# cwitkowitz/amt-tools

Measured on AMD Instinct MI355X. Metric: audio frames/sec (OnsetsFrames+Mel-229 inference), higher is better.
Workload: dtype bf16

## Files before the change

amt_tools_amd/csrc/amtx_kernels.h:

```cpp
#pragma once
#include "amtx_common.h"

enum { AMTX_T_BF16 = 0, AMTX_T_F32 = 1, AMTX_T_SPLIT = 2 };

static inline size_t amtx_tsize(int t) { return t == AMTX_T_BF16 ? 2 : 4; }

struct GemmArgs {
    const void* A; int64_t lda; int a_type;
    const bf16_t* W; int n_pad, k_pad, planes;
    const float* bias;
    void* C; int64_t ldc; int c_type;
    int64_t M; int N, K;
    int groups; int64_t a_gs, w_gs, bias_gs, c_gs;
    const int2* pair_map = nullptr; float* pair_out = nullptr; int64_t pair_gs = 0, pair_pitch = 0;
    int pair_rows[16] = {0, 0, 0, 0, 0, 0, 0, 0, 0, 0, 0, 0, 0, 0, 0, 0};
    float* pair_max = nullptr; int pair_nh = 0;
    float* roll_out = nullptr; int roll_T = 0; float roll_thr = 0.5f; int roll_group = 0;
    bf16_t* copy16 = nullptr; int64_t copy16_ld = 0; int copy16_col0 = 0, copy16_gs = 0, copy16_pad = 0;
    int64_t a_plane = 0;
    int64_t a_valid_lo = 0, a_valid_hi = 0;
    int64_t a_split = 0, c_split = 0;
};
constexpr int AMTX_GEMM_MULTI_MAX = 10;
struct GemmMulti { GemmArgs p[AMTX_GEMM_MULTI_MAX]; int n; };

struct ConvArgs {
    const void* in; int in_type;
    const bf16_t* wfrag; int planes;
    const float* shift;
    void* out; int out_type;
    int B, T, F, c_out;
    int groups; int64_t in_gs, w_gs, shift_gs, out_gs;
    const float* feats = nullptr; int64_t f_stride_b = 0, f_stride_c = 0, f_stride_t = 0, f_stride_f = 0;
    int c_in = 0;
    const bf16_t* w1frag = nullptr; const float* shift1 = nullptr;
    int64_t w1_gs = 0;
    const float* f_clip_max = nullptr; const float* f_ref = nullptr;
    const void* feats16 = nullptr;
    int64_t out_ts = 0;
    int64_t in_split = 0, out_split = 0;
};
int amtx_launch_convx3(const ConvArgs& c, hipStream_t stream);
int amtx_launch_convx12(const ConvArgs& c, hipStream_t stream);

static inline __host__ __device__ bool amtx_conv1g_tapk(int c_in, int planes) { return (planes == 1 || planes == 2) && c_in >= 2 && c_in <= 8; }

struct Conv1Args {
    const float* in; int64_t stride_b, stride_c, stride_t, stride_f;
    const float* w;
    const float* shift;
    void* out; int out_type;
    int B, T, F, c_in, c_out;
    int groups; int64_t w_gs, shift_gs, out_gs;
    int relu = 1;
};

struct LstmArgs {
    const void* xproj; int x_type;
    const bf16_t* whh; int planes;
    void* out; int out_type;
    int B, T;
    int groups; int64_t x_gs, w_gs, out_gs;
    int hidden = 128;
    float* save = nullptr;
};

namespace amtx_bf16 {
#include "amtx_kernels_fmt.h"
}
#ifdef AMTX_WITH_F16
namespace amtx_f16 {
#include "amtx_kernels_fmt.h"
}
#endif
using namespace AMTX_FMT_NS;

size_t amtx_bce_loss_partials(int B, int T, int keys);
int amtx_launch_bce_loss(const float* logits, int64_t ld, const float* labels, const float* weight, int B, int T, int keys, float* loss,
                         float* grad, float* partial, hipStream_t stream);
int amtx_launch_loss_reduce(const float* partial, int64_t n, float inv_bt, float* loss, hipStream_t stream);
int amtx_launch_pianoroll(const float* logits, int64_t ld, int col0, int B, int T, int keys, float threshold, float* out,
                          hipStream_t stream);

int amtx_launch_cvt_pad_bf16(const float* src, int64_t ld_src, int n_src, bf16_t* dst, int ld_dst, int64_t rows, hipStream_t stream,
                             bool f16 = false );
int amtx_launch_cvt_split(const float* src, int64_t ld_src, int n_src, bf16_t* dst, int ld_dst, int64_t split, int64_t rows, hipStream_t stream);
int amtx_launch_zero_cols(void* base, int64_t pitch_bytes, int width_bytes, int64_t rows, hipStream_t stream);

constexpr int DEC_HALF = 150;
constexpr int DEC_TAPS = 2 * DEC_HALF + 1;
constexpr int DEC_KW = 352;
constexpr int DEC_NKS = DEC_KW / 32;
int amtx_launch_cqt_decimate(const float* in, int64_t n_in, int64_t in_stride, int in_pad, float* out, int64_t n_out, int64_t out_stride, int pad,
                             const void* tfrag, int zero_pads, float* maxbuf, int n_harm, int batch, hipStream_t stream);
```

amt_tools_amd/csrc/amtx_kernels_fmt.h:

```cpp

bool amtx_gemm_has_roll_epilogue(const GemmArgs& g);
int amtx_launch_gemm(const GemmArgs& g, hipStream_t stream);
int amtx_launch_gemm_multi(const GemmArgs* gs, int n, hipStream_t stream);
void amtx_gemm_pack_dims(int N, int K, int* n_pad, int* k_pad);
void amtx_gemm_pack_host(const float* W, int64_t ldw, int N, int K, int planes, bf16_t* out);

int amtx_launch_conv3x3(const ConvArgs& c, hipStream_t stream);
size_t amtx_conv1_wfrag_elems(int c_in, int planes);
void amtx_conv1_pack_host(const float* w, const float* scale, int c_in, int planes, bf16_t* out);
size_t amtx_conv3x3_wfrag_elems(int c_out, int planes);
void amtx_conv3x3_pack_host(const float* w, const float* scale, int c_out, int planes, bf16_t* out);
int amtx_launch_conv1(const Conv1Args& c, hipStream_t stream);

bool amtx_conv_stack_fused_ok(int B, int T, int F, int groups);
int amtx_launch_conv_stack(const ConvArgs& c2, const bf16_t* w3frag, int64_t w3_gs, const float* shift3, void* out, int64_t out_gs,
                           int64_t out_plane, hipStream_t stream);

int amtx_conv3x3_gen_ntc(int c_in, int c_out);
size_t amtx_conv3x3_gen_wfrag_elems(int c_in, int c_out, int planes);
void amtx_conv3x3_gen_pack_host(const float* w , const float* scale, int c_in, int c_out, int planes, bf16_t* out);
int amtx_launch_conv3x3_gen(const ConvArgs& c, int c_in, hipStream_t stream);
size_t amtx_conv1g_wfrag_elems(int c_in, int c_mid, int planes);
void amtx_conv1g_pack_host(const float* w , const float* scale, int c_in, int c_mid, int planes, bf16_t* out);
bool amtx_conv3x3_gen_can_fuse1(int c_in, int c_mid, int c_out, int planes);

int amtx_launch_bilstm(const LstmArgs& l, hipStream_t stream);
size_t amtx_bilstm_wfrag_elems(int hidden, int planes);
void amtx_bilstm_pack_host(const float* whh_fwd, const float* whh_bwd, int hidden, int planes, bf16_t* out);
int amtx_launch_bilstm_pack_dev(const float* whh_fwd, const float* whh_bwd, int hidden, int planes, bf16_t* frag_fwd, bf16_t* frag_bwd, hipStream_t stream);
int amtx_launch_bilstm_bwd(const float* dout, const float* save, const bf16_t* whh_t, int hidden, int planes, float* dxproj, int B, int T, int groups,
                           hipStream_t stream);

int amtx_pack_bn_fold_dev(const float* conv_bias, const float* gamma, const float* beta, const float* mean, const float* var, int c_out, float* scale,
                          float* shift, hipStream_t s);
int amtx_pack_conv3x3_dev(const float* w, const float* scale, int c_out, int planes, bf16_t* out, hipStream_t s);
int amtx_pack_conv1_dev(const float* w, const float* scale, int planes, bf16_t* out, hipStream_t s);
int amtx_pack_conv_gen_dev(const float* w, const float* scale, int c_in, int c_out, int ntc, int planes, bf16_t* out, hipStream_t s);
int amtx_pack_conv1g_dev(const float* w, const float* scale, int c_in, int c_mid, int planes, bf16_t* out, hipStream_t s);
int amtx_pack_scale_rows_dev(const float* w, const float* scale, int rows, int cols, float* out, hipStream_t s);
int amtx_pack_linear_dev(const float* W, int64_t ldw, int N, int K, int planes, int n_pad, int k_pad, int row0, int rows_owned, int perm_c, int perm_f,
                         bf16_t* out, hipStream_t s);
void amtx_pack_linear_host(const float* W, int64_t ldw, int N, int K, int planes, int n_pad, int k_pad, int row0, int rows_owned, int perm_c, int perm_f,
                           bf16_t* out);
int amtx_pack_head_fold_dev(const float* w_out, const float* w_fc1, const float* b_fc1, const float* b_out, int n_out, int dim_am, int kfc, int kfc_pad,
                            int nf3, int fq, float* wfold, float* bfold, hipStream_t s);
int amtx_pack_vec_add_dev(const float* a, const float* b, int n, float* out, hipStream_t s);
```

amt_tools_amd/csrc/lstm.hip:

```cpp

#include "amtx_kernels.h"
#include "amtx_pack_layouts.h"

#include <type_traits>

namespace {

constexpr int H = 128;
constexpr int UB = 1;
constexpr int LWAVES = H / (16 * UB);
constexpr int LTHREADS = 64 * LWAVES;
constexpr int HP = H + 8;
constexpr int HBUF_BYTES = 16 * HP * 2;

template <bool FAST>
__device__ __forceinline__ float sigmoid_f(float x) {
    if (FAST) return __builtin_amdgcn_rcpf(1.0f + __builtin_amdgcn_exp2f(-1.4426950408889634f * x));
    return 1.0f / (1.0f + expf(-x));
}
template <bool FAST>
__device__ __forceinline__ float tanh_f(float x) {
    if (FAST) return fmaf(2.0f, __builtin_amdgcn_rcpf(1.0f + __builtin_amdgcn_exp2f(-2.8853900817779268f * x)), -1.0f);
    return tanhf(x);
}


struct Gates { float i, f, g, o; };
template <bool FAST>
__device__ __forceinline__ Gates lstm_gates(float ai, float af, float ag, float ao) {
    return {sigmoid_f<FAST>(ai), sigmoid_f<FAST>(af), tanh_f<FAST>(ag), sigmoid_f<FAST>(ao)};
}
template <bool FAST>
__device__ __forceinline__ float lstm_cell(const Gates& z, float& c) {
    c = z.f * c + z.i * z.g;
    return z.o * tanh_f<FAST>(c);
}

template <int NS>
__device__ __forceinline__ void split16(const float (&v)[4], uint2& hi, uint2& lo) {
    lo = make_uint2(0, 0);
    if (NS == 2) {
        split_bf16x2(v[0], v[1], hi.x, lo.x);
        split_bf16x2(v[2], v[3], hi.y, lo.y);
    } else {
        hi = make_uint2(pack_bf16x2(v[0], v[1]), pack_bf16x2(v[2], v[3]));
    }
}
template <int NS>
__device__ __forceinline__ void store16(char* tile, int plane_bytes, int off, uint2 hi, uint2 lo) {
    *reinterpret_cast<uint2*>(tile + off) = hi;
    if (NS == 2) *reinterpret_cast<uint2*>(tile + plane_bytes + off) = lo;
}

__device__ __forceinline__ int step_frame(int s, const int& T, const int& reverse) {
    s = s < T ? s : T - 1;
    return reverse == 0 ? s : T - 1 - s;
}

template <int SGK, int NS>
struct FragStream {
    typedef const __attribute__((address_space(1))) char* gchar_p;
    typedef __attribute__((ext_vector_type(4))) unsigned int u32x4_t;
    typedef __attribute__((address_space(1))) u32x4_t gu4_t;
    const char* base;
    gchar_p wb;
    unsigned wlane;
    __device__ __forceinline__ FragStream(const char* base_, int lane) : base(base_), wb((gchar_p)base_), wlane(lane * 16) {}
    __device__ __forceinline__ void rewind() {
        wb = (gchar_p)base;
        asm volatile("" : "+s"(wb));
    }
    __device__ __forceinline__ uint4 load(int gi, int k, int p) const {
        return __builtin_bit_cast(uint4, *reinterpret_cast<const gu4_t*>(wb + ((gi * SGK + k) * NS + p) * 1024 + wlane));
    }
    __device__ __forceinline__ void load_group(int gi, uint4 (&dst)[SGK][NS]) const {
        static_for<0, SGK>([&](auto kc) {
            static_for<0, NS>([&](auto pc) { dst[decltype(kc)::value][decltype(pc)::value] = load(gi, decltype(kc)::value, decltype(pc)::value); });
        });
    }
};

template <int X_TYPE> struct XRaw { typedef float4 type; };
template <> struct XRaw<AMTX_T_BF16> { typedef uint2 type; };

template <int X_TYPE>
__device__ __forceinline__ void load_x(const char* xbase, int64_t row_off, typename XRaw<X_TYPE>::type (&dst)[UB][4]) {
#pragma unroll
    for (int ub = 0; ub < UB; ++ub)
#pragma unroll
        for (int q = 0; q < 4; ++q) {
            const int64_t e = row_off + q * 128 + 16 * ub;
            dst[ub][q] = *reinterpret_cast<const typename XRaw<X_TYPE>::type*>(xbase + e * (X_TYPE == AMTX_T_F32 ? 4 : 2));
        }
}
__device__ __forceinline__ f32x4_t unpack_x(float4 v) { return (f32x4_t){v.x, v.y, v.z, v.w}; }
__device__ __forceinline__ f32x4_t unpack_x(uint2 v) {
    return (f32x4_t){unpack16_lo(v.x), unpack16_hi(v.x), unpack16_lo(v.y), unpack16_hi(v.y)};
}

__device__ __forceinline__ void lds_barrier() {
    asm volatile("s_waitcnt lgkmcnt(0)\n\ts_barrier" ::: "memory");
    __builtin_amdgcn_sched_barrier(0);
}

template <int NS, int X_TYPE, int OUT_TYPE, bool FAST>
__device__ __forceinline__ void lstm_step(char* smem, int cur, const uint4 (&wf)[UB][4][4][NS], const typename XRaw<X_TYPE>::type (&xcur)[UB][4],
                                          typename XRaw<X_TYPE>::type (&xnext)[UB][4], float (&c)[UB][4], const char* xbase, char* obase, int t, int tnext,
                                          int clip, int g, int wave, bool clip_ok) {
    const char* hb = smem + cur * NS * HBUF_BYTES;
    uint4 hf[4][NS];
#pragma unroll
    for (int ks = 0; ks < 4; ++ks)
#pragma unroll
        for (int p = 0; p < NS; ++p)
            hf[ks][p] = *reinterpret_cast<const uint4*>(hb + p * HBUF_BYTES + (clip * HP + 32 * ks + 8 * g) * 2);

    load_x<X_TYPE>(xbase, (int64_t)tnext * 1024, xnext);

    f32x4_t acc[UB][4];
#pragma unroll
    for (int ub = 0; ub < UB; ++ub)
#pragma unroll
        for (int q = 0; q < 4; ++q) acc[ub][q] = unpack_x(xcur[ub][q]);
#pragma unroll
    for (int ks = 0; ks < 4; ++ks)
#pragma unroll
        for (int ub = 0; ub < UB; ++ub)
#pragma unroll
            for (int q = 0; q < 4; ++q) {
                acc[ub][q] = mfma16(wf[ub][q][ks][0], hf[ks][0], acc[ub][q]);
                if (NS == 2) {
                    acc[ub][q] = mfma16(wf[ub][q][ks][0], hf[ks][1], acc[ub][q]);
                    acc[ub][q] = mfma16(wf[ub][q][ks][1], hf[ks][0], acc[ub][q]);
                }
            }

    char* hn = smem + (cur ^ 1) * NS * HBUF_BYTES;
#pragma unroll
    for (int ub = 0; ub < UB; ++ub) {
        float h[4];
#pragma unroll
        for (int r = 0; r < 4; ++r) {
            h[r] = lstm_cell<FAST>(lstm_gates<FAST>(acc[ub][0][r], acc[ub][1][r], acc[ub][2][r], acc[ub][3][r]), c[ub][r]);
        }
        uint2 hiw, low;
        split16<NS>(h, hiw, low);
        store16<NS>(hn, HBUF_BYTES, (clip * HP + 16 * UB * wave + 16 * ub + 4 * g) * 2, hiw, low);
        if (clip_ok) {
            const int64_t e = (int64_t)t * 256 + 16 * ub;
            if (OUT_TYPE == AMTX_T_BF16) *reinterpret_cast<uint2*>(obase + e * 2) = hiw;
            else *reinterpret_cast<float4*>(obase + e * 4) = make_float4(h[0], h[1], h[2], h[3]);
        }
    }
    lds_barrier();
}

template <int NS, int X_TYPE, int OUT_TYPE>
__global__ __launch_bounds__(LTHREADS) void bilstm_kernel(LstmArgs a) {
    extern __shared__ __attribute__((aligned(16))) char smem[];
    constexpr bool FAST = true;
    const int tid = threadIdx.x, lane = tid & 63, wave = tid >> 6;
    const int clip = lane & 15, g = lane >> 4;
    const int b0 = blockIdx.x * 16, dir = blockIdx.y, grp = blockIdx.z;
    const int b = b0 + clip;
    const bool clip_ok = b < a.B;
    const int T = a.T;

    uint4 wf[UB][4][4][NS];
    {
        const uint4* w = reinterpret_cast<const uint4*>(a.whh + (int64_t)grp * a.w_gs) + lane;
#pragma unroll
        for (int ub = 0; ub < UB; ++ub)
#pragma unroll
            for (int q = 0; q < 4; ++q)
#pragma unroll
                for (int ks = 0; ks < 4; ++ks)
#pragma unroll
                    for (int p = 0; p < NS; ++p)
                        wf[ub][q][ks][p] = w[((((((dir * LWAVES + wave) * UB + ub) * 4 + q) * 4 + ks) * NS) + p) * 64];
    }

    for (int i = tid; i < 2 * NS * HBUF_BYTES / 16; i += LTHREADS) reinterpret_cast<uint4*>(smem)[i] = make_uint4(0, 0, 0, 0);

    float c[UB][4];
#pragma unroll
    for (int ub = 0; ub < UB; ++ub)
#pragma unroll
        for (int r = 0; r < 4; ++r) c[ub][r] = 0.f;

    const char* xbase = reinterpret_cast<const char*>(a.xproj) +
                        ((int64_t)grp * a.x_gs + (int64_t)(clip_ok ? b : 0) * T * 1024 + dir * 512 + 16 * UB * wave + 4 * g) * (X_TYPE == AMTX_T_BF16 ? 2 : 4);
    char* obase = reinterpret_cast<char*>(a.out) +
                  ((int64_t)grp * a.out_gs + (int64_t)(clip_ok ? b : 0) * T * 256 + dir * 128 + 16 * UB * wave + 4 * g) * (OUT_TYPE == AMTX_T_BF16 ? 2 : 4);

    typename XRaw<X_TYPE>::type x0[UB][4], x1[UB][4], x2[UB][4], x3[UB][4];
    auto tidx = [&](int s) { return (int64_t)step_frame(s, T, dir); };
    load_x<X_TYPE>(xbase, tidx(0) * 1024, x0);
    load_x<X_TYPE>(xbase, tidx(1) * 1024, x1);
    load_x<X_TYPE>(xbase, tidx(2) * 1024, x2);
    __syncthreads();

    for (int s = 0; s < T; s += 4) {
        lstm_step<NS, X_TYPE, OUT_TYPE, FAST>(smem, 0, wf, x0, x3, c, xbase, obase, (int)tidx(s), (int)tidx(s + 3), clip, g, wave, clip_ok);
        lstm_step<NS, X_TYPE, OUT_TYPE, FAST>(smem, 1, wf, x1, x0, c, xbase, obase, (int)tidx(s + 1), (int)tidx(s + 4), clip, g, wave, clip_ok && s + 1 < T);
        lstm_step<NS, X_TYPE, OUT_TYPE, FAST>(smem, 0, wf, x2, x1, c, xbase, obase, (int)tidx(s + 2), (int)tidx(s + 5), clip, g, wave, clip_ok && s + 2 < T);
        lstm_step<NS, X_TYPE, OUT_TYPE, FAST>(smem, 1, wf, x3, x2, c, xbase, obase, (int)tidx(s + 3), (int)tidx(s + 6), clip, g, wave, clip_ok && s + 3 < T);
    }
}

template <int X_TYPE> struct XScalar { typedef float type; };
template <> struct XScalar<AMTX_T_BF16> { typedef unsigned int type; };
__device__ __forceinline__ float unpack_xs(float v, bool) { return v; }
__device__ __forceinline__ float unpack_xs(unsigned int v, bool odd) { return odd ? unpack16_hi(v) : unpack16_lo(v); }

template <int X_TYPE>
__device__ __forceinline__ void load_x4(const char* xbase, int64_t row_off, typename XScalar<X_TYPE>::type (&dst)[4]) {
#pragma unroll
    for (int q = 0; q < 4; ++q)
    {
        if (X_TYPE == AMTX_T_F32) dst[q] = *reinterpret_cast<const typename XScalar<X_TYPE>::type*>(xbase + (row_off + q * 128) * 4);
        else dst[q] = *reinterpret_cast<const unsigned int*>(xbase + (row_off + q * 128) * 2);
    }
}

template <int NS, int X_TYPE, int OUT_TYPE, bool FAST, int NC>
__device__ __forceinline__ void lstm4_step(char* smem, int cur, const uint4 (&wf)[4][4][NS], const typename XScalar<X_TYPE>::type (&xcur)[NC][4],
                                           typename XScalar<X_TYPE>::type (&xnext)[NC][4], float (&c)[NC], const char* const (&xbase)[NC],
                                           char* const (&obase)[NC], int t, int tnext, int lane, const int (&hwoff)[NC], const bool (&clip_ok)[NC],
                                           float* save) {
    constexpr int RSTEP = 4 / NC;
    const char* hb = smem + cur * NS * HBUF_BYTES;
    uint4 hf[4][NS];
#pragma unroll
    for (int ks = 0; ks < 4; ++ks)
#pragma unroll
        for (int p = 0; p < NS; ++p)
            hf[ks][p] = *reinterpret_cast<const uint4*>(hb + p * HBUF_BYTES + ((lane & 15) * HP + 32 * ks + 8 * (lane >> 4)) * 2);

#pragma unroll
    for (int j = 0; j < NC; ++j) load_x4<X_TYPE>(xbase[j], (int64_t)tnext * 1024, xnext[j]);

    f32x4_t acc[4];
#pragma unroll
    for (int q = 0; q < 4; ++q) {
        acc[q] = (f32x4_t){0.f, 0.f, 0.f, 0.f};
#pragma unroll
        for (int j = 0; j < NC; ++j) acc[q][RSTEP * j] = unpack_xs(xcur[j][q], lane & 1);
    }
#pragma unroll
    for (int ks = 0; ks < 4; ++ks) {
#pragma unroll
        for (int q = 0; q < 4; ++q) acc[q] = mfma16(hf[ks][0], wf[q][ks][0], acc[q]);
        if (NS == 2) {
#pragma unroll
            for (int q = 0; q < 4; ++q) acc[q] = mfma16(hf[ks][NS - 1], wf[q][ks][0], acc[q]);
#pragma unroll
            for (int q = 0; q < 4; ++q) acc[q] = mfma16(hf[ks][0], wf[q][ks][NS - 1], acc[q]);
        }
    }

    char* hn = smem + (cur ^ 1) * NS * HBUF_BYTES;
    Gates z[NC];
    float h[NC];
    uint32_t hiw[NC], low[NC];
#pragma unroll
    for (int j = 0; j < NC; ++j) z[j] = lstm_gates<FAST>(acc[0][RSTEP * j], acc[1][RSTEP * j], acc[2][RSTEP * j], acc[3][RSTEP * j]);
#pragma unroll
    for (int j = 0; j < NC; ++j) {
        h[j] = lstm_cell<FAST>(z[j], c[j]);
        low[j] = 0;
        if (NS == 2) split_bf16x2(h[j], 0.f, hiw[j], low[j]);
        else hiw[j] = pack_bf16x2(h[j], 0.f);
    }
#pragma unroll
    for (int j = 0; j < NC; ++j) {
        *reinterpret_cast<unsigned short*>(hn + hwoff[j]) = (unsigned short)hiw[j];
        if (NS == 2) *reinterpret_cast<unsigned short*>(hn + HBUF_BYTES + hwoff[j]) = (unsigned short)low[j];
    }
#pragma unroll
    for (int j = 0; j < NC; ++j) {
        if (NC == 1 && save && clip_ok[j]) {
            float* sv = save + (int64_t)t * (2 * 5 * H);
            sv[0] = z[j].i; sv[H] = z[j].f; sv[2 * H] = z[j].g; sv[3 * H] = z[j].o; sv[4 * H] = c[j];
        }
        if (clip_ok[j]) {
            if (OUT_TYPE == AMTX_T_BF16) *reinterpret_cast<unsigned short*>(obase[j] + (int64_t)t * 256 * 2) = (unsigned short)hiw[j];
            else *reinterpret_cast<float*>(obase[j] + (int64_t)t * 256 * 4) = h[j];
        }
    }
    lds_barrier();
}

template <int NS, int X_TYPE, int OUT_TYPE, int NC = 1>
__global__ __launch_bounds__(LTHREADS) void bilstm4_kernel(LstmArgs a) {
    extern __shared__ __attribute__((aligned(16))) char smem[];
    constexpr bool FAST = true;
    const int tid = threadIdx.x, lane = tid & 63, wave = tid >> 6;
    const int unit = 16 * wave + (lane & 15), cg = lane >> 4;
    const int dir = blockIdx.y, grp = blockIdx.z;
    const int T = a.T;

    uint4 wf[4][4][NS];
    {
        const uint4* w = reinterpret_cast<const uint4*>(a.whh + (int64_t)grp * a.w_gs) + lane;
#pragma unroll
        for (int q = 0; q < 4; ++q)
#pragma unroll
            for (int ks = 0; ks < 4; ++ks)
#pragma unroll
                for (int p = 0; p < NS; ++p) wf[q][ks][p] = w[(((((dir * LWAVES + wave) * 4 + q) * 4 + ks) * NS) + p) * 64];
    }
    for (int i = tid; i < 2 * NS * HBUF_BYTES / 16; i += LTHREADS) reinterpret_cast<uint4*>(smem)[i] = make_uint4(0, 0, 0, 0);

    float c[NC];
    bool clip_ok[NC];
    const char* xbase[NC];
    char* obase[NC];
    int hwoff[NC];
    float* save = nullptr;
#pragma unroll
    for (int j = 0; j < NC; ++j) {
        const int b = (blockIdx.x * 4 + cg) * NC + j;
        clip_ok[j] = b < a.B;
        c[j] = 0.f;
        xbase[j] = reinterpret_cast<const char*>(a.xproj) +
                   ((int64_t)grp * a.x_gs + (int64_t)(clip_ok[j] ? b : 0) * T * 1024 + dir * 512 + (X_TYPE == AMTX_T_BF16 ? (unit & ~1) : unit)) *
                       (X_TYPE == AMTX_T_BF16 ? 2 : 4);
        obase[j] = reinterpret_cast<char*>(a.out) +
                   ((int64_t)grp * a.out_gs + (int64_t)(clip_ok[j] ? b : 0) * T * 256 + dir * 128 + unit) * (OUT_TYPE == AMTX_T_BF16 ? 2 : 4);
        hwoff[j] = ((4 * cg + (4 / NC) * j) * HP + unit) * 2;
        if (NC == 1) save = a.save ? a.save + (((int64_t)grp * a.B + (clip_ok[j] ? b : 0)) * T * 2 + dir) * (5 * H) + unit : nullptr;
    }

    typename XScalar<X_TYPE>::type x0[NC][4], x1[NC][4], x2[NC][4], x3[NC][4];
    auto tidx = [&](int s) { return (int64_t)step_frame(s, T, dir); };
#pragma unroll
    for (int j = 0; j < NC; ++j) {
        load_x4<X_TYPE>(xbase[j], tidx(0) * 1024, x0[j]);
        load_x4<X_TYPE>(xbase[j], tidx(1) * 1024, x1[j]);
        load_x4<X_TYPE>(xbase[j], tidx(2) * 1024, x2[j]);
    }
    __syncthreads();

    for (int s = 0; s < T; s += 4) {
        bool ok1[NC], ok2[NC], ok3[NC];
#pragma unroll
        for (int j = 0; j < NC; ++j) { ok1[j] = clip_ok[j] && s + 1 < T; ok2[j] = clip_ok[j] && s + 2 < T; ok3[j] = clip_ok[j] && s + 3 < T; }
        lstm4_step<NS, X_TYPE, OUT_TYPE, FAST, NC>(smem, 0, wf, x0, x3, c, xbase, obase, (int)tidx(s), (int)tidx(s + 3), lane, hwoff, clip_ok, save);
        lstm4_step<NS, X_TYPE, OUT_TYPE, FAST, NC>(smem, 1, wf, x1, x0, c, xbase, obase, (int)tidx(s + 1), (int)tidx(s + 4), lane, hwoff, ok1, save);
        lstm4_step<NS, X_TYPE, OUT_TYPE, FAST, NC>(smem, 0, wf, x2, x1, c, xbase, obase, (int)tidx(s + 2), (int)tidx(s + 5), lane, hwoff, ok2, save);
        lstm4_step<NS, X_TYPE, OUT_TYPE, FAST, NC>(smem, 1, wf, x3, x2, c, xbase, obase, (int)tidx(s + 3), (int)tidx(s + 6), lane, hwoff, ok3, save);
    }
}

constexpr int GP = 4 * H + 8;
constexpr int GBUF_BYTES = 16 * GP * 2;

struct LstmBwdArgs {
    const float* dout;
    const float* save;
    const bf16_t* whh_t;
    int planes;
    float* dxproj;
    int B, T;
};

#ifdef AMTX_LSTM_TIMING
__device__ unsigned long long g_lstm_prof[4];
#define LT_TICK(SLOT) do { const unsigned long long n_ = __builtin_readcyclecounter(); lt_acc[SLOT] += n_ - lt_t; lt_t = n_; } while (0)
#else
#define LT_TICK(SLOT) do {} while (0)
#endif
template <int NS>
__global__ __launch_bounds__(LTHREADS) void bilstm4_bwd_kernel(LstmBwdArgs a) {
    extern __shared__ __attribute__((aligned(16))) char smem[];
    const int tid = threadIdx.x, lane = tid & 63, wave = tid >> 6;
    const int unit = 16 * wave + (lane & 15), cg = lane >> 4;
    const int dir = blockIdx.y;
    const int b = blockIdx.x * 4 + cg;
    const bool clip_ok = b < a.B;
    const int T = a.T;

    uint4 wt[16][NS];
    {
        const uint4* w = reinterpret_cast<const uint4*>(a.whh_t) + lane;
#pragma unroll
        for (int ks = 0; ks < 16; ++ks)
#pragma unroll
            for (int p = 0; p < NS; ++p) wt[ks][p] = w[((((dir * LWAVES + wave) * 16 + ks) * NS) + p) * 64];
    }
    for (int i = tid; i < 2 * NS * GBUF_BYTES / 16; i += LTHREADS) reinterpret_cast<uint4*>(smem)[i] = make_uint4(0, 0, 0, 0);
    __syncthreads();

    const int64_t bb = clip_ok ? b : 0;
    const float* sv0 = a.save + ((bb * T) * 2 + dir) * (5 * H) + unit;
    const float* do0 = a.dout + (bb * T) * 256 + dir * H + unit;
    float* dx0 = a.dxproj + (bb * T) * 1024 + dir * 512 + unit;
    const int gwoff = (4 * cg * GP + unit) * 2;

    float dh_rec = 0.f, dc_rec = 0.f;
    auto frame = [&](int s) { return step_frame(s, T, dir == 0); };
    float n_i, n_f, n_g, n_o, n_c, n_do;
    {
        const float* sv = sv0 + (int64_t)frame(0) * (2 * 5 * H);
        n_i = sv[0]; n_f = sv[H]; n_g = sv[2 * H]; n_o = sv[3 * H]; n_c = sv[4 * H];
        n_do = do0[(int64_t)frame(0) * 256];
    }
#ifdef AMTX_LSTM_TIMING
    unsigned long long lt_acc[4] = {0, 0, 0, 0}, lt_t = __builtin_readcyclecounter();
#endif
    for (int s = 0; s < T; ++s) {
        const int t = frame(s);
        const float ig = n_i, fg = n_f, gg = n_g, og = n_o, ct = n_c, dout_t = n_do;
        {
            const int tn = frame(s + 1);
            const float* sv = sv0 + (int64_t)tn * (2 * 5 * H);
            n_i = sv[0]; n_f = sv[H]; n_g = sv[2 * H]; n_o = sv[3 * H]; n_c = sv[4 * H];
            n_do = do0[(int64_t)tn * 256];
        }
        asm volatile("" : "+v"(n_c));
        const float cp = s + 1 < T ? n_c : 0.f;
        const float dh = dout_t + dh_rec;
        const float tc = tanh_f<true>(ct);
        const float d_o = dh * tc * og * (1.f - og);
        const float dc = dc_rec + dh * og * (1.f - tc * tc);
        const float d_i = dc * gg * ig * (1.f - ig);
        const float d_g = dc * ig * (1.f - gg * gg);
        const float d_f = dc * cp * fg * (1.f - fg);
        dc_rec = dc * fg;
        const float dgv[4] = {d_i, d_f, d_g, d_o};
        char* gt = smem + (s & 1) * NS * GBUF_BYTES;
#pragma unroll
        for (int q = 0; q < 4; ++q) {
            if (clip_ok) dx0[(int64_t)t * 1024 + q * H] = dgv[q];
            uint32_t hiw, low = 0;
            if (NS == 2) split_bf16x2(dgv[q], 0.f, hiw, low);
            else hiw = pack_bf16x2(dgv[q], 0.f);
            *reinterpret_cast<unsigned short*>(gt + gwoff + q * H * 2) = (unsigned short)hiw;
            if (NS == 2) *reinterpret_cast<unsigned short*>(gt + GBUF_BYTES + gwoff + q * H * 2) = (unsigned short)low;
        }
        LT_TICK(0);
        lds_barrier();
        LT_TICK(1);
        f32x4_t acc4[4];
#pragma unroll
        for (int i = 0; i < 4; ++i) acc4[i] = (f32x4_t){0.f, 0.f, 0.f, 0.f};
#pragma unroll
        for (int k4 = 0; k4 < 16; k4 += 4) {
            uint4 gf[4][NS];
#pragma unroll
            for (int i = 0; i < 4; ++i)
#pragma unroll
                for (int p = 0; p < NS; ++p)
                    gf[i][p] = *reinterpret_cast<const uint4*>(gt + p * GBUF_BYTES + ((lane & 15) * GP + 32 * (k4 + i) + 8 * (lane >> 4)) * 2);
#pragma unroll
            for (int i = 0; i < 4; ++i) acc4[i] = mfma16(gf[i][0], wt[k4 + i][0], acc4[i]);
            if (NS == 2) {
#pragma unroll
                for (int i = 0; i < 4; ++i) acc4[i] = mfma16(gf[i][NS - 1], wt[k4 + i][0], acc4[i]);
#pragma unroll
                for (int i = 0; i < 4; ++i) acc4[i] = mfma16(gf[i][0], wt[k4 + i][NS - 1], acc4[i]);
            }
        }
        dh_rec = (acc4[0][0] + acc4[1][0]) + (acc4[2][0] + acc4[3][0]);
#ifdef AMTX_LSTM_TIMING
        asm volatile("" ::"v"(dh_rec));
        LT_TICK(2);
        lt_acc[3] += 1;
#endif
    }
#ifdef AMTX_LSTM_TIMING
    if (tid == 0 && blockIdx.x == 0 && blockIdx.y == 0)
        for (int i = 0; i < 4; ++i) atomicAdd(&g_lstm_prof[i], lt_acc[i]);
#endif
}
#if defined(AMTX_LSTM_TIMING) && !defined(AMTX_F16)
extern "C" int amtxdbg_lstm_prof(unsigned long long* out4, int reset) {
    if (hipMemcpyFromSymbol(out4, HIP_SYMBOL(g_lstm_prof), 4 * sizeof(unsigned long long)) != hipSuccess) return -1;
    if (reset) {
        unsigned long long z[4] = {0, 0, 0, 0};
        if (hipMemcpyToSymbol(HIP_SYMBOL(g_lstm_prof), z, sizeof(z)) != hipSuccess) return -1;
    }
    return 0;
}
#endif

template <int HC>
__global__ void bilstm_pack_dev_kernel(const float* __restrict__ whh_fwd, const float* __restrict__ whh_bwd, int hidden, AmtxFragPut fwd, AmtxFragPut bwd) {
    if (HC) hidden = HC;
    for (int item = blockIdx.x * blockDim.x + threadIdx.x, n = amtx_layout_bilstm_items(hidden); item < n; item += gridDim.x * blockDim.x) {
        amtx_layout_bilstm(item, whh_fwd, whh_bwd, hidden, fwd);
        amtx_layout_bilstm_transposed(item, whh_fwd, whh_bwd, hidden, bwd);
    }
}

template <int HH, int NS, int X_TYPE, int OUT_TYPE>
__global__ __launch_bounds__(512) void bilstm_stream_kernel(LstmArgs a) {
    constexpr int NU = HH / 16, UPW = NU / 8, KSN = HH / 32;
    constexpr int SGK = NS == 2 ? 2 : 4;
    constexpr int NSUB = KSN / SGK;
    constexpr int NG = UPW * 4 * NSUB;
    constexpr int HPG = HH + 8;
    constexpr int HBG = 16 * HPG * 2;
    constexpr bool FAST = true;
    constexpr int RS = 4;
    constexpr bool PIN = NS == 1 && HH == 256;
    constexpr bool PINL = NS == 1 && HH == 384;
    constexpr int PER = NG / 4;
    constexpr int NPIN = PIN ? NG / 4 : (PINL ? 4 : 0);
    constexpr int NSG = NG - (PIN ? 2 : (PINL ? 1 : 0)) * NPIN;
    static_assert(NU % 8 == 0 && KSN % SGK == 0 && NG % 4 == 0 && NSG % RS == 0, "hidden size must be a multiple of 128");
    extern __shared__ __attribute__((aligned(16))) char smem[];
    const int tid = threadIdx.x, lane = tid & 63, wave = tid >> 6;
    const int clip = lane & 15, g = lane >> 4;
    const int b0 = blockIdx.x * 16, dir = blockIdx.y, grp = blockIdx.z;
    const int b = b0 + clip;
    const bool clip_ok = b < a.B;
    const int T = a.T;
    constexpr int XES = X_TYPE == AMTX_T_BF16 ? 2 : 4, OES = OUT_TYPE == AMTX_T_BF16 ? 2 : 4;

    for (int i = tid; i < 2 * NS * HBG / 16; i += 512) reinterpret_cast<uint4*>(smem)[i] = make_uint4(0, 0, 0, 0);

    const int wave_u = __builtin_amdgcn_readfirstlane(wave);
    const char* wbase = reinterpret_cast<const char*>(a.whh + (int64_t)grp * a.w_gs) + ((int64_t)(dir * NU + wave_u * UPW) * 4 * KSN * NS) * 1024;
    FragStream<SGK, NS> ws(wbase, lane);
    const char* xbase = reinterpret_cast<const char*>(a.xproj) +
                        ((int64_t)grp * a.x_gs + (int64_t)(clip_ok ? b : 0) * T * 8 * HH + dir * 4 * HH + 16 * UPW * wave + 4 * g) * XES;
    char* obase = reinterpret_cast<char*>(a.out) +
                  ((int64_t)grp * a.out_gs + (int64_t)(clip_ok ? b : 0) * T * 2 * HH + dir * HH + 16 * UPW * wave + 4 * g) * OES;

    float c[UPW][4];
#pragma unroll
    for (int ub = 0; ub < UPW; ++ub)
#pragma unroll
        for (int r = 0; r < 4; ++r) c[ub][r] = 0.f;

    typedef typename XRaw<X_TYPE>::type xraw_t;
    auto tidx = [&](int s) { return (int64_t)step_frame(s, T, dir); };
    auto load_xrow = [&](int64_t t, xraw_t (&dst)[UPW][4]) {
#pragma unroll
        for (int ub = 0; ub < UPW; ++ub)
#pragma unroll
            for (int q = 0; q < 4; ++q)
                dst[ub][q] = *reinterpret_cast<const xraw_t*>(xbase + (t * 8 * HH + q * HH + 16 * ub) * XES);
    };
    uint4 w[RS][SGK][NS];
    uint4 wpin[PIN ? NPIN : 1][SGK][NS];
    char* wlds = smem + 2 * NS * HBG + wave * (NPIN * SGK * NS * 1024);
    if constexpr (PIN || PINL) {
        static_for<0, NG>([&](auto ic) {
            constexpr int gi = decltype(ic)::value;
            constexpr int kind = PIN ? ((gi & 3) == 0 ? 0 : ((gi & 3) == 1 ? 1 : 2)) : (gi % PER == 0 ? 1 : 2);
            constexpr int pidx = PIN ? gi >> 2 : gi / PER;
            if constexpr (kind < 2) {
                static_for<0, SGK>([&](auto kc) {
                    constexpr int k = decltype(kc)::value;
                    static_for<0, NS>([&](auto pc) {
                        constexpr int p = decltype(pc)::value;
                        const uint4 v = ws.load(gi, k, p);
                        if constexpr (kind == 0) wpin[pidx][k][p] = v;
                        else *reinterpret_cast<uint4*>(wlds + ((pidx * SGK + k) * NS + p) * 1024 + ws.wlane) = v;
                    });
                });
            }
        });
    }

    xraw_t xn[UPW][4];
    load_xrow(tidx(0), xn);
    static_for<0, RS - 1>([&](auto sc) {
        constexpr int si = decltype(sc)::value;
        constexpr int gi = PIN ? (si >> 1) * 4 + 2 + (si & 1) : (PINL ? si + si / (PER - 1) + 1 : si);
        ws.load_group(gi, w[si % RS]);
    });
    __syncthreads();

    int cur = 0;
    for (int s = 0; s < T; ++s) {
        ws.rewind();
        const char* hb = smem + cur * NS * HBG;
        constexpr bool HF_REG = KSN * NS <= 16;
        uint4 hf[HF_REG ? KSN : 1][NS];
        if constexpr (HF_REG) {
#pragma unroll
            for (int ks = 0; ks < KSN; ++ks)
#pragma unroll
                for (int p = 0; p < NS; ++p) hf[ks][p] = *reinterpret_cast<const uint4*>(hb + p * HBG + (clip * HPG + 32 * ks + 8 * g) * 2);
        }

        f32x4_t acc[UPW][4];
#pragma unroll
        for (int ub = 0; ub < UPW; ++ub)
#pragma unroll
            for (int q = 0; q < 4; ++q) acc[ub][q] = unpack_x(xn[ub][q]);
        load_xrow(tidx(s + 1), xn);
        __builtin_amdgcn_sched_barrier(0);

        static_for<0, NG>([&](auto ic) {
            constexpr int gi = decltype(ic)::value;
            constexpr int ub = gi / (4 * NSUB), q = (gi / NSUB) & 3, sub = gi % NSUB;
            constexpr int kind = PIN ? ((gi & 3) == 0 ? 0 : ((gi & 3) == 1 ? 1 : 2)) : (PINL ? (gi % PER == 0 ? 1 : 2) : 2);
            constexpr int pidx = PIN ? gi >> 2 : gi / PER;
            constexpr int si = PIN ? (gi >> 2) * 2 + (gi & 3) - 2 : (PINL ? gi - gi / PER - 1 : gi);
            if constexpr (kind == 2) {
                constexpr int sn = (si + RS - 1) % NSG;
                constexpr int gn = PIN ? (sn >> 1) * 4 + 2 + (sn & 1) : (PINL ? sn + sn / (PER - 1) + 1 : sn);
                ws.load_group(gn, w[sn % RS]);
            }
            f32x4_t d = acc[ub][q];
            static_for<0, SGK>([&](auto kc) {
                constexpr int k = decltype(kc)::value;
                constexpr int ks = sub * SGK + k;
                uint4 w0, w1;
                if constexpr (kind == 0) {
                    w0 = wpin[pidx][k][0]; w1 = wpin[pidx][k][NS - 1];
                } else if constexpr (kind == 1) {
                    w0 = *reinterpret_cast<const uint4*>(wlds + ((pidx * SGK + k) * NS + 0) * 1024 + ws.wlane);
                    w1 = w0;
                } else {
                    w0 = w[si % RS][k][0]; w1 = w[si % RS][k][NS - 1];
                }
                uint4 h0, h1;
                if constexpr (HF_REG) {
                    h0 = hf[ks][0]; h1 = hf[ks][NS - 1];
                } else {
                    h0 = *reinterpret_cast<const uint4*>(hb + (clip * HPG + 32 * ks + 8 * g) * 2);
                    h1 = *reinterpret_cast<const uint4*>(hb + (NS - 1) * HBG + (clip * HPG + 32 * ks + 8 * g) * 2);
                }
                d = mfma16(w0, h0, d);
                if constexpr (NS == 2) {
                    d = mfma16(w0, h1, d);
                    d = mfma16(w1, h0, d);
                }
            });
            acc[ub][q] = d;
            __builtin_amdgcn_sched_barrier(0);
        });

        char* hn = smem + (cur ^ 1) * NS * HBG;
        const int64_t t = tidx(s);
#pragma unroll
        for (int ub = 0; ub < UPW; ++ub) {
            float h[4], sv[4][4];
#pragma unroll
            for (int r = 0; r < 4; ++r) {
                const Gates z = lstm_gates<FAST>(acc[ub][0][r], acc[ub][1][r], acc[ub][2][r], acc[ub][3][r]);
                h[r] = lstm_cell<FAST>(z, c[ub][r]);
                sv[0][r] = z.i; sv[1][r] = z.f; sv[2][r] = z.g; sv[3][r] = z.o;
            }
            if (a.save && clip_ok) {
                float* sp = a.save + ((((int64_t)grp * a.B + b) * T + t) * 2 + dir) * (5 * HH) + 16 * UPW * wave + 16 * ub + 4 * g;
#pragma unroll
                for (int q = 0; q < 4; ++q) *reinterpret_cast<float4*>(sp + q * HH) = make_float4(sv[q][0], sv[q][1], sv[q][2], sv[q][3]);
                *reinterpret_cast<float4*>(sp + 4 * HH) = make_float4(c[ub][0], c[ub][1], c[ub][2], c[ub][3]);
            }
            uint2 hiw, low;
            split16<NS>(h, hiw, low);
            store16<NS>(hn, HBG, (clip * HPG + 16 * UPW * wave + 16 * ub + 4 * g) * 2, hiw, low);
            if (clip_ok) {
                const int64_t e = t * 2 * HH + 16 * ub;
                if (OUT_TYPE == AMTX_T_BF16) *reinterpret_cast<uint2*>(obase + e * 2) = hiw;
                else *reinterpret_cast<float4*>(obase + e * 4) = make_float4(h[0], h[1], h[2], h[3]);
            }
        }
        cur ^= 1;
        lds_barrier();
    }
}

struct LstmBwdHArgs {
    const float* dout; const float* save; const bf16_t* whh_t; float* dxproj; int B, T;
    int64_t w_gs;
};

template <int HH, int NS>
__global__ __launch_bounds__(512) void bilstm_stream_bwd_kernel(LstmBwdHArgs a) {
    constexpr int UT = HH / 128;
    constexpr int KSN = 4 * HH / 32;
    constexpr int SGK = NS == 2 ? 2 : 4;
    constexpr int NG = UT * KSN / SGK;
    constexpr int RS = 4;
    constexpr bool PINB = HH == 256;
    constexpr int NPINB = PINB ? NG / 4 : 0, NSGB = NG - NPINB;
    constexpr int GPH = 4 * HH + 8;
    constexpr int GBH = 5 * GPH * 2;
    static_assert(NG % 4 == 0 && NSGB % RS == 0, "hidden size must be a multiple of 128");
    extern __shared__ __attribute__((aligned(16))) char smem[];
    const int tid = threadIdx.x, lane = tid & 63, wave = tid >> 6;
    const int cg = lane >> 4;
    const int dir = blockIdx.y;
    const int b = blockIdx.x * 4 + cg;
    const bool clip_ok = b < a.B;
    const int T = a.T;
    const int unit0 = 16 * UT * wave + (lane & 15);

    for (int i = tid; i < 2 * NS * GBH / 16; i += 512) reinterpret_cast<uint4*>(smem)[i] = make_uint4(0, 0, 0, 0);

    const int wave_u = __builtin_amdgcn_readfirstlane(wave);
    const int grp = blockIdx.z;
    const char* wbase = reinterpret_cast<const char*>(a.whh_t + (int64_t)grp * a.w_gs) + ((int64_t)(dir * 8 + wave_u) * UT * KSN * NS) * 1024;
    FragStream<SGK, NS> ws(wbase, lane);
    uint4 w[RS][SGK][NS];

    const int64_t bb = (int64_t)grp * a.B + (clip_ok ? b : 0);
    const float* sv0 = a.save + ((bb * T) * 2 + dir) * (5 * HH) + unit0;
    const float* do0 = a.dout + (bb * T) * (2 * HH) + dir * HH + unit0;
    float* dx0 = a.dxproj + (bb * T) * (8 * HH) + dir * 4 * HH + unit0;
    const int gwoff = (cg * GPH + unit0) * 2;
    const int groff = ((((lane & 15) & 3) == 0 ? (lane & 15) >> 2 : 4) * GPH + 8 * (lane >> 4)) * 2;

    float dh_rec[UT], dc_rec[UT];
#pragma unroll
    for (int ut = 0; ut < UT; ++ut) { dh_rec[ut] = 0.f; dc_rec[ut] = 0.f; }
    auto frame = [&](int s) { return step_frame(s, T, dir == 0); };
    float nv[UT][6];
    auto load_next = [&](int tn) {
#pragma unroll
        for (int ut = 0; ut < UT; ++ut) {
            const float* sv = sv0 + (int64_t)tn * (2 * 5 * HH) + 16 * ut;
#pragma unroll
            for (int q = 0; q < 5; ++q) nv[ut][q] = sv[q * HH];
            nv[ut][5] = do0[(int64_t)tn * (2 * HH) + 16 * ut];
        }
    };
    load_next(frame(0));
    uint4 wpin[PINB ? NPINB : 1][SGK][NS];
    static_for<0, NPINB>([&](auto gc) { ws.load_group(4 * decltype(gc)::value, wpin[decltype(gc)::value]); });
    static_for<0, RS - 1>([&](auto sc) {
        constexpr int si = decltype(sc)::value;
        constexpr int gi = PINB ? (si / 3) * 4 + 1 + si % 3 : si;
        ws.load_group(gi, w[si % RS]);
    });
    __syncthreads();

    for (int s = 0; s < T; ++s) {
        ws.rewind();
        const int t = frame(s);
        float cur[UT][6];
#pragma unroll
        for (int ut = 0; ut < UT; ++ut)
#pragma unroll
            for (int q = 0; q < 6; ++q) cur[ut][q] = nv[ut][q];
        load_next(frame(s + 1));
        char* gt = smem + (s & 1) * NS * GBH;
#pragma unroll
        for (int ut = 0; ut < UT; ++ut) {
            asm volatile("" : "+v"(nv[ut][4]));
            const float cp = s + 1 < T ? nv[ut][4] : 0.f;
            const float ig = cur[ut][0], fg = cur[ut][1], gg = cur[ut][2], og = cur[ut][3], ct = cur[ut][4];
            const float dh = cur[ut][5] + dh_rec[ut];
            const float tc = tanh_f<true>(ct);
            const float d_o = dh * tc * og * (1.f - og);
            const float dc = dc_rec[ut] + dh * og * (1.f - tc * tc);
            const float d_i = dc * gg * ig * (1.f - ig);
            const float d_g = dc * ig * (1.f - gg * gg);
            const float d_f = dc * cp * fg * (1.f - fg);
            dc_rec[ut] = dc * fg;
            const float dgv[4] = {d_i, d_f, d_g, d_o};
#pragma unroll
            for (int q = 0; q < 4; ++q) {
                if (clip_ok) dx0[(int64_t)t * (8 * HH) + q * HH + 16 * ut] = dgv[q];
                uint32_t hiw, low = 0;
                if (NS == 2) split_bf16x2(dgv[q], 0.f, hiw, low);
                else hiw = pack_bf16x2(dgv[q], 0.f);
                *reinterpret_cast<unsigned short*>(gt + gwoff + (q * HH + 16 * ut) * 2) = (unsigned short)hiw;
                if (NS == 2) *reinterpret_cast<unsigned short*>(gt + GBH + gwoff + (q * HH + 16 * ut) * 2) = (unsigned short)low;
            }
        }
        lds_barrier();
        f32x4_t acc[UT];
#pragma unroll
        for (int ut = 0; ut < UT; ++ut) acc[ut] = (f32x4_t){0.f, 0.f, 0.f, 0.f};
        static_for<0, NG>([&](auto ic) {
            constexpr int gi = decltype(ic)::value;
            constexpr int ut = gi / (KSN / SGK), sub = gi % (KSN / SGK);
            constexpr bool pinned = PINB && (gi & 3) == 0;
            constexpr int si = PINB ? (gi >> 2) * 3 + (gi & 3) - 1 : gi;
            if constexpr (!pinned) {
                constexpr int sn = (si + RS - 1) % NSGB;
                constexpr int gn = PINB ? (sn / 3) * 4 + 1 + sn % 3 : sn;
                ws.load_group(gn, w[sn % RS]);
            }
            static_for<0, SGK>([&](auto kc) {
                constexpr int k = decltype(kc)::value;
                constexpr int ks = sub * SGK + k;
                uint4 gf[NS];
#pragma unroll
                for (int p = 0; p < NS; ++p)
                    gf[p] = *reinterpret_cast<const uint4*>(gt + p * GBH + groff + 32 * ks * 2);
                uint4 w0, w1;
                if constexpr (pinned) { w0 = wpin[gi >> 2][k][0]; w1 = wpin[gi >> 2][k][NS - 1]; }
                else { w0 = w[si % RS][k][0]; w1 = w[si % RS][k][NS - 1]; }
                acc[ut] = mfma16(gf[0], w0, acc[ut]);
                if constexpr (NS == 2) {
                    acc[ut] = mfma16(gf[NS - 1], w0, acc[ut]);
                    acc[ut] = mfma16(gf[0], w1, acc[ut]);
                }
            });
            __builtin_amdgcn_sched_barrier(0);
        });
#pragma unroll
        for (int ut = 0; ut < UT; ++ut) dh_rec[ut] = acc[ut][0];
    }
}


struct LstmSwitches { bool no8; };
const LstmSwitches& lstm_switches() {
    static const LstmSwitches sw = {getenv("AMTX_LSTM_NO8") != nullptr};
    return sw;
}

enum LstmFamily { LSTM_CLIPS4, LSTM_CLIPS8, LSTM_CLIPS16, LSTM_STREAM, LSTM_ERROR };
enum LstmInst { LSTM_BF16, LSTM_BF16_F32IO, LSTM_X3, LSTM_NO_INST };
struct LstmRouted { LstmFamily family; LstmInst inst; dim3 grid; size_t lds; int code; const char* error; };

LstmRouted lstm_route(const LstmArgs& a, const LstmSwitches& sw) {
    const bool io16 = a.x_type == AMTX_T_BF16 && a.out_type == AMTX_T_BF16, io32 = a.x_type == AMTX_T_F32 && a.out_type == AMTX_T_F32;
    const LstmInst inst = a.planes == 1 && io16 ? LSTM_BF16 : (a.planes == 1 && io32 ? LSTM_BF16_F32IO : (a.planes == 2 && io32 ? LSTM_X3 : LSTM_NO_INST));
    auto error = [](int code, const char* msg) { return LstmRouted{LSTM_ERROR, LSTM_NO_INST, dim3(), 0, code, msg}; };
    auto on = [&](LstmFamily family, int clips, size_t lds) {
        return LstmRouted{family, inst, dim3((unsigned)((a.B + clips - 1) / clips), 2, (unsigned)a.groups), lds, AMTX_OK, nullptr};
    };
    if (a.hidden != H) {
        if (a.save && a.planes != 2) return error(AMTX_ERR_ARG, "bilstm: the training forward (save) is built for the two-plane precision");
        if (a.hidden != 256 && a.hidden != 384 && a.hidden != 512) return error(AMTX_ERR_UNSUPPORTED, "bilstm: unsupported hidden size (128, 256, 384 and 512 are built)");
        if (inst != LSTM_BF16 && inst != LSTM_X3) return error(AMTX_ERR_UNSUPPORTED, "bilstm: unsupported precision/type combination");
        return on(LSTM_STREAM, 16, 2 * (size_t)a.planes * 16 * (a.hidden + 8) * 2 + (a.planes == 1 && a.hidden <= 384 ? (size_t)8 * 4 * 4096 : 0));
    }
    if (inst == LSTM_NO_INST) return error(AMTX_ERR_UNSUPPORTED, "bilstm: unsupported precision/type combination");
    const size_t lds = 2 * (size_t)a.planes * HBUF_BYTES;
    const int64_t blocks4 = (int64_t)((a.B + 3) / 4) * 2 * a.groups;
    if (a.save) return on(LSTM_CLIPS4, 4, lds);
    if (blocks4 > 1024) return on(LSTM_CLIPS16, 16, lds);
    if (!sw.no8 && a.planes == 1 && blocks4 > 256) return on(LSTM_CLIPS8, 8, lds);
    return on(LSTM_CLIPS4, 4, lds);
}

template <typename F>
int with_hidden(int hidden, F&& f) {
    switch (hidden) {
        case 256: return f(std::integral_constant<int, 256>{});
        case 384: return f(std::integral_constant<int, 384>{});
        case 512: return f(std::integral_constant<int, 512>{});
    }
    amtx_set_error("bilstm: unsupported hidden size %d (128, 256, 384 and 512 are built)", hidden);
    return AMTX_ERR_UNSUPPORTED;
}

template <typename K, typename A>
int launch_kernel(K kern, dim3 grid, size_t lds, hipStream_t stream, const A& a) {
    AMTX_GRANT_LDS(kern, lds);
    hipLaunchKernelGGL(kern, grid, dim3(LTHREADS), lds, stream, a);
    AMTX_CHECK_LAUNCH();
    return AMTX_OK;
}

template <int NS, int XT>
int launch_routed(const LstmRouted& r, const LstmArgs& a, hipStream_t stream) {
    switch (r.family) {
        case LSTM_CLIPS4: return launch_kernel(bilstm4_kernel<NS, XT, XT>, r.grid, r.lds, stream, a);
        case LSTM_CLIPS8: return launch_kernel(bilstm4_kernel<NS, XT, XT, 2>, r.grid, r.lds, stream, a);
        case LSTM_CLIPS16: return launch_kernel(bilstm_kernel<NS, XT, XT>, r.grid, r.lds, stream, a);
        case LSTM_STREAM:
            if constexpr (NS == 2 || XT == AMTX_T_BF16)
                return with_hidden(a.hidden, [&](auto hh) { return launch_kernel(bilstm_stream_kernel<decltype(hh)::value, NS, XT, XT>, r.grid, r.lds, stream, a); });
            break;
        case LSTM_ERROR: break;
    }
    amtx_set_error("bilstm: route without a kernel");
    return AMTX_ERR_UNSUPPORTED;
}

}

namespace AMTX_FMT_NS {

size_t amtx_bilstm_wfrag_elems(int hidden, int planes) { return (size_t)2 * 4 * hidden * hidden * planes; }

static_assert(16 * UB * LWAVES == H && LWAVES == AMTX_LSTM_BWD_WAVES, "W_hh fragment layouts");

void amtx_bilstm_pack_host(const float* whh_fwd, const float* whh_bwd, int hidden, int planes, bf16_t* out) {
    const AmtxFragPut put{out, planes};
    for (int item = 0, n = amtx_layout_bilstm_items(hidden); item < n; ++item) amtx_layout_bilstm(item, whh_fwd, whh_bwd, hidden, put);
}

int amtx_launch_bilstm(const LstmArgs& a, hipStream_t stream) {
    AMTX_REQUIRE(a.xproj && a.whh && a.out, "bilstm: null pointer");
    AMTX_REQUIRE(a.B > 0 && a.T > 0 && a.groups > 0, "bilstm: bad sizes");
    AMTX_REQUIRE(a.planes == 1 || a.planes == 2, "bilstm: planes must be 1 or 2");
    const LstmRouted r = lstm_route(a, lstm_switches());
    switch (r.inst) {
        case LSTM_BF16: return launch_routed<1, AMTX_T_BF16>(r, a, stream);
        case LSTM_BF16_F32IO: return launch_routed<1, AMTX_T_F32>(r, a, stream);
        case LSTM_X3: return launch_routed<2, AMTX_T_F32>(r, a, stream);
        case LSTM_NO_INST: break;
    }
    amtx_set_error("%s (hidden %d)", r.error, a.hidden);
    return r.code;
}

int amtx_launch_bilstm_pack_dev(const float* whh_fwd, const float* whh_bwd, int hidden, int planes, bf16_t* frag_fwd, bf16_t* frag_bwd, hipStream_t stream) {
    AMTX_REQUIRE(whh_fwd && whh_bwd && frag_fwd && frag_bwd && (planes == 1 || planes == 2), "bilstm pack: bad argument");
    AMTX_REQUIRE(hidden == H || hidden == 256 || hidden == 384 || hidden == 512, "bilstm pack: hidden size %d is not built (128, 256, 384, 512)", hidden);
    const AmtxFragPut fwd{frag_fwd, planes}, bwd{frag_bwd, planes};
    if (hidden == H) hipLaunchKernelGGL(bilstm_pack_dev_kernel<H>, dim3(64), dim3(256), 0, stream, whh_fwd, whh_bwd, H, fwd, bwd);
    else hipLaunchKernelGGL(bilstm_pack_dev_kernel<0>, dim3(256), dim3(256), 0, stream, whh_fwd, whh_bwd, hidden, fwd, bwd);
    AMTX_CHECK_LAUNCH();
    return AMTX_OK;
}

int amtx_launch_bilstm_bwd(const float* dout, const float* save, const bf16_t* whh_t, int hidden, int planes, float* dxproj, int B, int T, int groups,
                           hipStream_t stream) {
    AMTX_REQUIRE(groups >= 1, "bilstm backward: bad group count");
    AMTX_REQUIRE(dout && save && whh_t && dxproj, "bilstm backward: null pointer");
    AMTX_REQUIRE(B > 0 && T > 0 && (planes == 1 || planes == 2), "bilstm backward: bad sizes");
    const int64_t w_gs = (int64_t)amtx_bilstm_wfrag_elems(hidden, planes), bt = (int64_t)B * T;
    const dim3 grid((unsigned)((B + 3) / 4), 2);
    if (hidden == H) {
        for (int g = 0; g < groups; ++g) {
            const LstmBwdArgs a{dout + g * bt * 2 * H, save + g * bt * 2 * 5 * H, whh_t + g * w_gs, planes, dxproj + g * bt * 8 * H, B, T};
            const size_t lds = 2 * (size_t)planes * GBUF_BYTES;
            const int rc = planes == 2 ? launch_kernel(bilstm4_bwd_kernel<2>, grid, lds, stream, a) : launch_kernel(bilstm4_bwd_kernel<1>, grid, lds, stream, a);
            if (rc != AMTX_OK) return rc;
        }
        return AMTX_OK;
    }
    AMTX_REQUIRE(planes == 2 && (hidden == 256 || hidden == 384 || hidden == 512),
                 "bilstm backward: hidden 256 / 384 / 512 are built for the two-plane precision only (got hidden %d, planes %d)", hidden, planes);
    const LstmBwdHArgs a{dout, save, whh_t, dxproj, B, T, w_gs};
    return with_hidden(hidden, [&](auto hh) {
        return launch_kernel(bilstm_stream_bwd_kernel<decltype(hh)::value, 2>, dim3(grid.x, 2, (unsigned)groups), 2 * (size_t)planes * 5 * (4 * hidden + 8) * 2, stream, a);
    });
}

}
```

amt_tools_amd/csrc/ofmodel.hip:

```cpp

#include "amtx_kernels.h"
#include "amtx_model_common.h"
#include "amtx_pack_layouts.h"

#include <cmath>
#include <cstdlib>
#include <thread>

namespace {

struct LinearPack { DevBuf w, b; int N = 0, K = 0, n_pad = 0, k_pad = 0, groups = 0; };

#define AMTX_FMT_KERNELS(X, ns)                                                                                                    \
    X(ns, pack_linear_host) X(ns, bilstm_pack_host) X(ns, conv1_pack_host) X(ns, conv1g_pack_host) X(ns, conv3x3_pack_host)     \
    X(ns, conv3x3_gen_pack_host) X(ns, pack_conv1_dev) X(ns, pack_conv1g_dev) X(ns, pack_conv3x3_dev) X(ns, pack_conv_gen_dev)    \
    X(ns, pack_linear_dev) X(ns, launch_bilstm_pack_dev) X(ns, launch_conv1) X(ns, launch_conv3x3) X(ns, launch_conv3x3_gen)    \
    X(ns, launch_conv_stack) X(ns, launch_gemm) X(ns, launch_bilstm)
#define AMTX_KERNEL_FIELD(ns, name) decltype(&ns::amtx_##name) name;
#define AMTX_KERNEL_ENTRY(ns, name) &ns::amtx_##name,
struct KernelSet { AMTX_FMT_KERNELS(AMTX_KERNEL_FIELD, amtx_bf16) };
const KernelSet kKernelsBf16 = {AMTX_FMT_KERNELS(AMTX_KERNEL_ENTRY, amtx_bf16)};
#ifdef AMTX_WITH_F16
const KernelSet kKernelsF16 = {AMTX_FMT_KERNELS(AMTX_KERNEL_ENTRY, amtx_f16)};
#endif

enum ConvFamily { K_CONV1,
                  K_CONV,
                  K_CONVG };
struct ConvLayer { const char* name; int c_in, c_out; ConvFamily fam; size_t frag_per; };

struct ConvSwitches { bool no_convg_mc2, no_conv_fuse, x3_no_split, no_convx12m, rowmajor_a3, no_roll_epilogue; };
ConvSwitches switches_from_env() {
    auto on = [](const char* name) { return getenv(name) != nullptr; };
    return {on("AMTX_NO_CONVG_MC2"), on("AMTX_NO_CONV_FUSE"), on("AMTX_X3_NO_SPLIT"), on("AMTX_NO_CONVX12M"), on("AMTX_OF_ROWMAJOR_A3"), on("AMTX_OF_NO_ROLL_EPILOGUE")};
}

struct ConvPlan {
    ConvLayer layer[3];
    bool conv1_fused;
    bool stack;
    bool two_plane_acts;
    bool convx12; size_t c2x_per;
    bool rowmajor_a3, no_roll_epilogue;
    bool device_resync;
    int fuses_db_scale, takes_feats16;
};

ConvPlan make_conv_plan(int in_channels, int model_complexity, int precision, const ConvSwitches& sw) {
    const int ic = in_channels, nf1 = 16 * model_complexity, nf3 = 2 * nf1, pl = precision == AMTX_PREC_X3 ? 2 : 1;
    ConvPlan p{};
    const ConvFamily f3 = nf1 != 32 ? K_CONVG : K_CONV;
    const bool g_fuse1 = amtx_conv3x3_gen_can_fuse1(ic, nf1, nf1, pl);
    const ConvFamily f2 = f3 == K_CONVG || (ic > 1 && !sw.no_convg_mc2 && g_fuse1) ? K_CONVG : K_CONV;
    p.conv1_fused = f2 == K_CONVG ? g_fuse1 : 9 * ic <= 64;
    auto frag3x3 = [pl](ConvFamily f, int c_in, int c_out) { return f == K_CONVG ? amtx_conv3x3_gen_wfrag_elems(c_in, c_out, pl) : amtx_conv3x3_wfrag_elems(c_out, pl); };
    p.layer[0] = {"layer1", ic, nf1, p.conv1_fused ? f2 : K_CONV1,
                  !p.conv1_fused ? 0 : f2 == K_CONVG ? amtx_conv1g_wfrag_elems(ic, nf1, pl) : amtx_conv1_wfrag_elems(ic, pl)};
    p.layer[1] = {"layer2", nf1, nf1, f2, frag3x3(f2, nf1, nf1)};
    p.layer[2] = {"layer3", nf1, nf3, f3, frag3x3(f3, nf1, nf3)};
    p.stack = f2 == K_CONV && p.conv1_fused && ic == 1 && pl == 1 && !sw.no_conv_fuse;
    p.two_plane_acts = pl == 2 && f3 == K_CONV && p.conv1_fused && !sw.x3_no_split && (f2 == K_CONV ? ic == 1 : ic > 1 && (9 * ic + 31) / 32 <= 2);
    p.convx12 = p.two_plane_acts && f2 == K_CONVG && ic >= 2 && ic <= 8 && amtx_conv1g_tapk(ic, 2) && !sw.no_convx12m;
    p.c2x_per = frag3x3(K_CONV, nf1, nf1);
    p.rowmajor_a3 = sw.rowmajor_a3; p.no_roll_epilogue = sw.no_roll_epilogue;
    p.device_resync = f2 == K_CONVG || ic == 1;
    p.fuses_db_scale = p.conv1_fused && f2 == K_CONV && ic == 1;
    p.takes_feats16 = !(p.conv1_fused && f2 == K_CONVG && precision != AMTX_PREC_F16) ? 0 : p.convx12 ? 2 : pl == 1 && nf1 == 32 && amtx_conv1g_tapk(ic, pl);
    return p;
}

}

struct amtx_of_model {
    int dim_in, in_channels, mc, n_out, has_offsets, precision;
    int planes, act_type;
    bool f16 = false;
    const KernelSet* k = &kKernelsBf16;
    int nf1, nf2, nf3, dim_am, dim_lm, fq, kfc;
    int kfc_pad;
    int hid, xw;
    size_t hh_elems;
    ConvPlan plan;
    int n_heads;
    int n_rec;
    std::vector<std::string> head_names;
    TensorStore store{"of_model", "was not provided"};
    DevBuf pack_scratch;
    bool finalized = false;
    bool packed_once = false;
    DevBuf conv_w[3], conv_s[3];
    DevBuf conv1_w;
    DevBuf conv2_wx;
    LinearPack fc1;
    LinearPack rec_ih;
    DevBuf rec_hh;
    LinearPack rec_out;
    LinearPack pitch_out;
    LinearPack adj_ih;
    DevBuf adj_hh;
    LinearPack adj_out;
    int dim_aj;
    mutable bool prof = false;
    mutable std::vector<std::vector<hipEvent_t>> prof_events;
};

enum { ST_CONV1 = 0, ST_CONV2, ST_CONV3, ST_FC1, ST_REC_XPROJ, ST_REC_LSTM, ST_REC_HEAD, ST_PITCH_HEAD, ST_ADJ_XPROJ, ST_ADJ_LSTM,
       ST_ADJ_HEAD, ST_PIANOROLL, ST_COUNT };
static const char* kStageNames[ST_COUNT] = {"conv1", "conv2_pool", "conv3_pool", "fc1_gemm", "rec_xproj_gemm", "rec_bilstm", "rec_head_gemm",
                                            "pitch_head_gemm", "adj_xproj_gemm", "adj_bilstm", "adj_head_gemm", "pianoroll"};

namespace {

struct Workspace {
    char *a1, *a2, *a3, *e, *xp, *l1, *joint, *joint16, *xp2, *l2, *mp;
    size_t total;
};

enum ConvPath { PATH_STACK,
                PATH_CONVX12,
                PATH_CONV12, PATH_CONVG12,
                PATH_CONV1 };
struct ConvCall { ConvPath path; bool a2_in_hbm; int64_t a3_plane; };

ConvCall resolve_conv(const amtx_of_model* m, int B, int T, bool feats16) {
    const ConvPlan& p = m->plan;
    if (p.stack && amtx_conv_stack_fused_ok(B, T, m->dim_in, m->n_heads))
        return {PATH_STACK, false, p.rowmajor_a3 ? 0 : (int64_t)B * T * 64};
    return {feats16 && p.convx12 ? PATH_CONVX12 : !p.conv1_fused ? PATH_CONV1 : p.layer[1].fam == K_CONVG ? PATH_CONVG12 : PATH_CONV12, true, 0};
}

Workspace carve(const amtx_of_model* m, int B, int T, char* base) {
    Workspace w;
    const size_t es = amtx_tsize(m->act_type);
    const size_t BT = (size_t)B * T;
    const int F = m->dim_in, F2 = F / 2;
    WorkspaceCarver ws{base};
    w.a1 = ws.take(m->plan.conv1_fused ? 256 : BT * F * m->nf1 * es * m->n_heads);
    w.a2 = ws.take(resolve_conv(m, B, T, false).a2_in_hbm ? BT * F2 * m->nf2 * es * m->n_heads : 256);
    w.a3 = ws.take(BT * m->kfc_pad * es * m->n_heads);
    w.e = ws.take(BT * m->dim_am * es * m->n_heads);
    w.xp = ws.take(BT * m->xw * es * m->n_rec);
    w.l1 = ws.take(BT * m->dim_lm * es * m->n_rec);
    w.joint = ws.take(BT * m->dim_aj * sizeof(float));
    w.joint16 = ws.take(BT * (size_t)((m->dim_aj + 63) / 64 * 64) * 2 * (m->plan.two_plane_acts ? 2 : 1));
    w.xp2 = ws.take(BT * m->xw * es);
    w.l2 = ws.take(BT * m->dim_lm * es);
    w.mp = ws.take(BT * m->n_out * sizeof(float));
    w.total = ws.off;
    return w;
}

}

extern "C" int amtx_has_f16(void) {
#ifdef AMTX_WITH_F16
    return 1;
#else
    return 0;
#endif
}

extern "C" int amtx_of_model_create(amtx_of_model** out, int dim_in, int in_channels, int model_complexity, int n_out,
                                    int has_offsets, int precision) {
    AMTX_REQUIRE(out, "amtx_of_model_create: null model pointer");
    *out = nullptr;
    AMTX_REQUIRE(precision == AMTX_PREC_BF16 || precision == AMTX_PREC_X3 || precision == AMTX_PREC_F16, "amtx_of_model_create: bad precision");
    AMTX_REQUIRE(dim_in >= 4 && in_channels >= 1 && n_out > 0 && n_out % 4 == 0, "amtx_of_model_create: bad dims");
    if (precision == AMTX_PREC_F16 && !amtx_has_f16()) {
        amtx_set_error("amtx_of_model_create: precision f16 needs a library built with the half-operand kernel twins (AMTX_BUILD_F16=1 python -m amt_tools_amd.build)");
        return AMTX_ERR_UNSUPPORTED;
    }
    if (model_complexity < 2 || model_complexity > 5) {
        amtx_set_error("amtx_of_model_create: model_complexity 2 (32/32/64-channel convolutions, LSTM hidden 128), 3 (48/48/96, hidden 256) and "
                       "4 (64/64/128, hidden 384), 5 (80/80/160, hidden 512) are implemented, with or without the OnsetsFrames2 offset head (got model_complexity=%d)", model_complexity);
        return AMTX_ERR_UNSUPPORTED;
    }
    amtx_of_model* m = new amtx_of_model();
    m->dim_in = dim_in; m->in_channels = in_channels; m->mc = model_complexity; m->n_out = n_out;
    m->has_offsets = has_offsets; m->precision = precision;
    m->planes = precision == AMTX_PREC_X3 ? 2 : 1;
    m->act_type = precision == AMTX_PREC_X3 ? AMTX_T_F32 : AMTX_T_BF16;
    m->f16 = precision == AMTX_PREC_F16;
#ifdef AMTX_WITH_F16
    if (m->f16) m->k = &kKernelsF16;
#endif
    m->nf1 = 16 * model_complexity; m->nf2 = m->nf1; m->nf3 = 32 * model_complexity;
    m->dim_am = 256 * model_complexity; m->dim_lm = 256 * (model_complexity - 1);
    m->fq = dim_in / 4;
    m->kfc = m->nf3 * m->fq;
    m->kfc_pad = (m->kfc + 63) / 64 * 64;
    m->hid = m->dim_lm / 2; m->xw = 8 * m->hid;
    m->hh_elems = amtx_bilstm_wfrag_elems(m->hid, m->planes);
    m->plan = make_conv_plan(in_channels, model_complexity, precision, switches_from_env());
    m->head_names = {"onset_head"};
    if (has_offsets) m->head_names.push_back("offset_head");
    m->n_rec = (int)m->head_names.size();
    m->head_names.push_back("pitch_head");
    m->n_heads = (int)m->head_names.size();
    m->dim_aj = (m->n_rec + 1) * n_out;
    *out = m;
    return AMTX_OK;
}

extern "C" int amtx_of_model_destroy(amtx_of_model* m) {
    if (!m) return AMTX_OK;
    DevBuf* bufs[] = {&m->conv1_w, &m->conv_w[0], &m->conv_w[1], &m->conv_w[2], &m->conv_s[0], &m->conv_s[1], &m->conv_s[2], &m->conv2_wx, &m->fc1.w, &m->fc1.b,
                      &m->rec_ih.w, &m->rec_ih.b, &m->rec_hh, &m->rec_out.w, &m->rec_out.b, &m->pitch_out.w, &m->pitch_out.b,
                      &m->adj_ih.w, &m->adj_ih.b, &m->adj_hh, &m->adj_out.w, &m->adj_out.b, &m->pack_scratch};
    for (DevBuf* b : bufs) b->release();
    delete m;
    return AMTX_OK;
}

extern "C" int amtx_of_model_set_tensor(amtx_of_model* m, const char* name, const float* host_data, int64_t numel) {
    AMTX_REQUIRE(m && name && host_data && numel > 0, "amtx_of_model_set_tensor: bad argument");
    m->store.set(name, host_data, numel);
    m->finalized = false;
    return AMTX_OK;
}

namespace {

struct HostPack {
    amtx_of_model* m;
    std::map<DevBuf*, std::vector<char>> image;
    std::vector<float> scratch_;

    int need(const std::string& name, size_t numel, const float** p) { return m->store.need(name, numel, p); }
    template <class T> T* dst(DevBuf& b, size_t elems) {
        std::vector<char>& v = image[&b];
        v.resize(elems * sizeof(T));
        return (T*)v.data();
    }
    int scratch(size_t floats, float** p) { scratch_.resize(floats); *p = scratch_.data(); return AMTX_OK; }
    int bn_fold(const float* cb, const float* g, const float* be, const float* mu, const float* var, int c_out, float* scale, float* shift) {
        for (int c = 0; c < c_out; ++c) amtx_bn_fold(cb, g, be, mu, var, c, scale, shift);
        return AMTX_OK;
    }
    int scale_rows(const float* w, const float* scale, int rows, int cols, float* out) {
        for (int item = 0; item < rows * cols; ++item) amtx_layout_scale_rows(item, w, scale, cols, out);
        return AMTX_OK;
    }
    int conv1(const float* w, const float* scale, int c_in, bf16_t* out) { m->k->conv1_pack_host(w, scale, c_in, m->planes, out); return AMTX_OK; }
    int conv1g(const float* w, const float* scale, int c_in, int c_mid, bf16_t* out) { m->k->conv1g_pack_host(w, scale, c_in, c_mid, m->planes, out); return AMTX_OK; }
    int conv3x3(const float* w, const float* scale, int c_out, bf16_t* out) { m->k->conv3x3_pack_host(w, scale, c_out, m->planes, out); return AMTX_OK; }
    int conv_gen(const float* w, const float* scale, int c_in, int c_out, bf16_t* out) { m->k->conv3x3_gen_pack_host(w, scale, c_in, c_out, m->planes, out); return AMTX_OK; }
    int linear(const float* W, int64_t ldw, int N, int K, const LinearPack& lp, int row0, int rows, int perm_c, int perm_f, bf16_t* out) {
        m->k->pack_linear_host(W, ldw, N, K, m->planes, lp.n_pad, lp.k_pad, row0, rows, perm_c, perm_f, out);
        return AMTX_OK;
    }
    int vec_add(const float* a, const float* b, int n, float* out) { for (int i = 0; i < n; ++i) out[i] = a[i] + b[i]; return AMTX_OK; }
    int copy(float* out, const float* src, size_t n) { memcpy(out, src, n * sizeof(float)); return AMTX_OK; }
    int bilstm(const float* whh_fwd, const float* whh_bwd, bf16_t* out) { m->k->bilstm_pack_host(whh_fwd, whh_bwd, m->hid, m->planes, out); return AMTX_OK; }
    int head_fold(const float* w_out, const float* w_fc1, const float* b_fc1, const float* b_out, float* wfold, float* bfold) {
        const int n_out = m->n_out, dim_am = m->dim_am, kfc = m->kfc, kfc_pad = m->kfc_pad, nf3 = m->nf3, fq = m->fq;
        auto fold_rows = [=](int o0, int o1) {
            std::vector<double> rowacc(kfc);
            for (int o = o0; o < o1; ++o) {
                std::fill(rowacc.begin(), rowacc.end(), 0.0);
                double bacc = b_out[o];
                for (int j = 0; j < dim_am; ++j) {
                    const double wo = w_out[(size_t)o * dim_am + j];
                    const float* frow = w_fc1 + (size_t)j * kfc;
                    for (int ks = 0; ks < kfc; ++ks) rowacc[ks] += wo * frow[ks];
                    bacc += wo * b_fc1[j];
                }
                for (int k = 0; k < kfc_pad; ++k) wfold[(size_t)o * kfc_pad + k] = k < kfc ? (float)rowacc[amtx_fc1_col(k, nf3, fq)] : 0.0f;
                bfold[o] = (float)bacc;
            }
        };
        const int nthreads = (int)std::max(1u, std::min(8u, std::thread::hardware_concurrency()));
        std::vector<std::thread> pool;
        const int per = (n_out + nthreads - 1) / nthreads;
        for (int t = 1; t < nthreads; ++t)
            if (t * per < n_out) pool.emplace_back(fold_rows, t * per, std::min(n_out, (t + 1) * per));
        fold_rows(0, std::min(n_out, per));
        for (auto& th : pool) th.join();
        return AMTX_OK;
    }
};

struct DevicePack {
    amtx_of_model* m;
    hipStream_t s;
    bool dry;

    int need(const std::string& name, size_t numel, const float** p) { return m->store.need_device(name, numel, p); }
    template <class T> T* dst(DevBuf& b, size_t) { return (T*)b.p; }
    bf16_t* hh_bwd = nullptr;
    int scratch(size_t floats, float** p) {
        const size_t bytes = floats * sizeof(float) + m->hh_elems * sizeof(bf16_t) + 256;
        if (!m->pack_scratch.p || m->pack_scratch.bytes < bytes) {
            m->pack_scratch.release();
            AMTX_CHECK_HIP(hipMalloc(&m->pack_scratch.p, bytes));
            m->pack_scratch.bytes = bytes;
        }
        *p = (float*)m->pack_scratch.p;
        hh_bwd = (bf16_t*)(((uintptr_t)(*p + floats) + 255) & ~(uintptr_t)255);
        return AMTX_OK;
    }
    int bn_fold(const float* cb, const float* g, const float* be, const float* mu, const float* var, int c_out, float* scale, float* shift) {
        return dry ? AMTX_OK : amtx_pack_bn_fold_dev(cb, g, be, mu, var, c_out, scale, shift, s);
    }
    int scale_rows(const float* w, const float* scale, int rows, int cols, float* out) { return dry ? AMTX_OK : amtx_pack_scale_rows_dev(w, scale, rows, cols, out, s); }
    int conv1(const float* w, const float* scale, int c_in, bf16_t* out) {
        AMTX_REQUIRE(c_in == 1, "amtx_of_model_finalize_device: internal: no device packer for a multi-channel first conv on conv.hip");
        return dry ? AMTX_OK : m->k->pack_conv1_dev(w, scale, m->planes, out, s);
    }
    int conv1g(const float* w, const float* scale, int c_in, int c_mid, bf16_t* out) { return dry ? AMTX_OK : m->k->pack_conv1g_dev(w, scale, c_in, c_mid, m->planes, out, s); }
    int conv3x3(const float* w, const float* scale, int c_out, bf16_t* out) { return dry ? AMTX_OK : m->k->pack_conv3x3_dev(w, scale, c_out, m->planes, out, s); }
    int conv_gen(const float* w, const float* scale, int c_in, int c_out, bf16_t* out) {
        return dry ? AMTX_OK : m->k->pack_conv_gen_dev(w, scale, c_in, c_out, amtx_conv3x3_gen_ntc(c_in, c_out), m->planes, out, s);
    }
    int linear(const float* W, int64_t ldw, int N, int K, const LinearPack& lp, int row0, int rows, int perm_c, int perm_f, bf16_t* out) {
        return dry ? AMTX_OK : m->k->pack_linear_dev(W, ldw, N, K, m->planes, lp.n_pad, lp.k_pad, row0, rows, perm_c, perm_f, out, s);
    }
    int vec_add(const float* a, const float* b, int n, float* out) { return dry ? AMTX_OK : amtx_pack_vec_add_dev(a, b, n, out, s); }
    int copy(float* out, const float* src, size_t n) {
        if (!dry) AMTX_CHECK_HIP(hipMemcpyAsync(out, src, n * sizeof(float), hipMemcpyDeviceToDevice, s));
        return AMTX_OK;
    }
    int bilstm(const float* whh_fwd, const float* whh_bwd, bf16_t* out) {
        return dry ? AMTX_OK : m->k->launch_bilstm_pack_dev(whh_fwd, whh_bwd, m->hid, m->planes, out, hh_bwd, s);
    }
    int head_fold(const float* w_out, const float* w_fc1, const float* b_fc1, const float* b_out, float* wfold, float* bfold) {
        return dry ? AMTX_OK : amtx_pack_head_fold_dev(w_out, w_fc1, b_fc1, b_out, m->n_out, m->dim_am, m->kfc, m->kfc_pad, m->nf3, m->fq, wfold, bfold, s);
    }
};

#define NEED(name, numel, ptr)                                         \
    do {                                                               \
        int _rc = x.need(name, numel, &(ptr));                         \
        if (_rc != AMTX_OK) return _rc;                                \
    } while (0)
#define STEP(expr)                                                     \
    do {                                                               \
        int _rc = (expr);                                              \
        if (_rc != AMTX_OK) return _rc;                                \
    } while (0)

template <class X>
int pack_model(amtx_of_model* m, X& x) {
    const int nh = m->n_heads, pl = m->planes, G = 4 * m->hid, ic = m->in_channels;
    const ConvPlan& p = m->plan;
    auto size_linear = [](LinearPack& lp, int N, int K, int groups) {
        lp.N = N; lp.K = K; lp.groups = groups;
        amtx_gemm_pack_dims(N, K, &lp.n_pad, &lp.k_pad);
    };
    size_linear(m->fc1, m->dim_am, m->kfc_pad, m->n_rec);
    size_linear(m->rec_ih, m->xw, m->dim_am, m->n_rec);
    size_linear(m->rec_out, m->n_out, m->dim_lm, m->n_rec);
    size_linear(m->pitch_out, m->n_out, m->kfc_pad, 1);
    size_linear(m->adj_ih, m->xw, m->dim_aj, 1);
    size_linear(m->adj_out, m->n_out, m->dim_lm, 1);
    auto linear = [&](LinearPack& lp, int grp, const float* W, int N, int K, int row0, int rows, int perm_c, int perm_f) {
        const size_t per = (size_t)lp.n_pad * lp.k_pad * pl;
        return x.linear(W, K, N, K, lp, row0, rows, perm_c, perm_f, x.template dst<bf16_t>(lp.w, per * lp.groups) + per * grp);
    };
    auto bias = [&](LinearPack& lp, int grp) { return x.template dst<float>(lp.b, (size_t)lp.N * lp.groups) + (size_t)lp.N * grp; };
    auto need_fc1 = [&](int h, const float*& w, const float*& b) {
        NEED(m->head_names[h] + ".0.fc1.0.weight", (size_t)m->dim_am * m->kfc, w);
        NEED(m->head_names[h] + ".0.fc1.0.bias", (size_t)m->dim_am, b);
        return (int)AMTX_OK;
    };
    auto need_bank = [&](const std::string& bank, int K, const float*& w, const float*& b) {
        NEED(bank + ".output_layer.weight", (size_t)m->n_out * K, w);
        NEED(bank + ".output_layer.bias", (size_t)m->n_out, b);
        return (int)AMTX_OK;
    };
    AMTX_REQUIRE(m->nf3 <= 256, "of_model: internal: scale scratch");
    float* scale;
    STEP(x.scratch(256 + (size_t)m->n_out * m->kfc_pad + m->n_out, &scale));
    float* wfold = scale + 256;
    float* bfold = wfold + (size_t)m->n_out * m->kfc_pad;

    for (int h = 0; h < nh; ++h) {
        const std::string am = m->head_names[h] + ".0";
        const float *w, *cb, *g, *be, *mu, *var;
        for (int l = 0; l < 3; ++l) {
            const ConvLayer& y = p.layer[l];
            const std::string conv = am + "." + y.name + ".0", bn = am + "." + y.name + ".1";
            NEED(conv + ".weight", (size_t)y.c_out * y.c_in * 9, w);
            NEED(conv + ".bias", (size_t)y.c_out, cb); NEED(bn + ".weight", (size_t)y.c_out, g); NEED(bn + ".bias", (size_t)y.c_out, be);
            NEED(bn + ".running_mean", (size_t)y.c_out, mu); NEED(bn + ".running_var", (size_t)y.c_out, var);
            STEP(x.bn_fold(cb, g, be, mu, var, y.c_out, scale, x.template dst<float>(m->conv_s[l], (size_t)nh * y.c_out) + (size_t)h * y.c_out));
            bf16_t* frag = x.template dst<bf16_t>(m->conv_w[l], y.frag_per * nh) + y.frag_per * h;
            if (l == 0) {
                const size_t per = (size_t)y.c_out * ic * 9;
                STEP(x.scale_rows(w, scale, y.c_out, ic * 9, x.template dst<float>(m->conv1_w, per * nh) + per * h));
                if (y.fam == K_CONVG) STEP(x.conv1g(w, scale, ic, y.c_out, frag));
                else if (y.fam == K_CONV) STEP(x.conv1(w, scale, ic, frag));
            } else if (y.fam == K_CONVG) STEP(x.conv_gen(w, scale, y.c_in, y.c_out, frag));
            else STEP(x.conv3x3(w, scale, y.c_out, frag));
            if (l == 1 && p.convx12) STEP(x.conv3x3(w, scale, y.c_out, x.template dst<bf16_t>(m->conv2_wx, p.c2x_per * nh) + p.c2x_per * h));
        }
        if (h < m->n_rec) {
            const float* fb;
            STEP(need_fc1(h, w, fb));
            STEP(linear(m->fc1, h, w, m->dim_am, m->kfc, 0, m->fc1.n_pad, m->nf3, m->fq));
            STEP(x.copy(bias(m->fc1, h), fb, m->dim_am));
        }
    }
    auto pack_rec = [&](const std::string& lstm, const std::string& bank, int dim_in, LinearPack& ih, DevBuf& hh, LinearPack& outp, int grp) {
        const float *wif, *wib, *whf, *whb, *bif, *bib, *bhf, *bhb, *wo, *bo;
        const std::string q = lstm + ".mlm.";
        NEED(q + "weight_ih_l0", (size_t)G * dim_in, wif); NEED(q + "weight_ih_l0_reverse", (size_t)G * dim_in, wib);
        NEED(q + "weight_hh_l0", (size_t)G * m->hid, whf); NEED(q + "weight_hh_l0_reverse", (size_t)G * m->hid, whb);
        NEED(q + "bias_ih_l0", (size_t)G, bif); NEED(q + "bias_ih_l0_reverse", (size_t)G, bib);
        NEED(q + "bias_hh_l0", (size_t)G, bhf); NEED(q + "bias_hh_l0_reverse", (size_t)G, bhb);
        STEP(linear(ih, grp, wif, G, dim_in, 0, G, 0, 0));
        STEP(linear(ih, grp, wib, G, dim_in, G, ih.n_pad - G, 0, 0));
        STEP(x.vec_add(bif, bhf, G, bias(ih, grp)));
        STEP(x.vec_add(bib, bhb, G, bias(ih, grp) + G));
        STEP(x.bilstm(whf, whb, x.template dst<bf16_t>(hh, m->hh_elems * ih.groups) + m->hh_elems * grp));
        STEP(need_bank(bank, m->dim_lm, wo, bo));
        STEP(linear(outp, grp, wo, m->n_out, m->dim_lm, 0, outp.n_pad, 0, 0));
        STEP(x.copy(bias(outp, grp), bo, m->n_out));
        return (int)AMTX_OK;
    };
    for (int r = 0; r < m->n_rec; ++r) STEP(pack_rec(m->head_names[r] + ".1", m->head_names[r] + ".2", m->dim_am, m->rec_ih, m->rec_hh, m->rec_out, r));
    {
        const float *wo, *bo, *w1, *b1;
        STEP(need_bank("pitch_head.1", m->dim_am, wo, bo));
        STEP(need_fc1(nh - 1, w1, b1));
        STEP(x.head_fold(wo, w1, b1, bo, wfold, bfold));
        STEP(linear(m->pitch_out, 0, wfold, m->n_out, m->kfc_pad, 0, m->pitch_out.n_pad, 0, 0));
        STEP(x.copy(bias(m->pitch_out, 0), bfold, m->n_out));
    }
    return pack_rec("adjoin.0", "adjoin.1", m->dim_aj, m->adj_ih, m->adj_hh, m->adj_out, 0);
}

}

extern "C" int amtx_of_model_finalize(amtx_of_model* m) {
    AMTX_REQUIRE(m, "amtx_of_model_finalize: null model");
    STEP(amtx_quiesce_before_resync(m->packed_once));
    if (m->plan.layer[2].fam == K_CONVG && (!amtx_conv3x3_gen_ntc(m->nf1, m->nf2) || !amtx_conv3x3_gen_ntc(m->nf2, m->nf3))) {
        amtx_set_error("of_model: no convolution kernel for %d -> %d -> %d channels", m->nf1, m->nf2, m->nf3);
        return AMTX_ERR_UNSUPPORTED;
    }
    HostPack x{m};
    STEP(pack_model(m, x));
    DevBuf* order[] = {&m->conv1_w, &m->conv_s[0], &m->conv_w[0], &m->conv_w[1], &m->conv2_wx, &m->conv_s[1], &m->conv_w[2], &m->conv_s[2],
                       &m->fc1.w, &m->fc1.b, &m->rec_ih.w, &m->rec_ih.b, &m->rec_hh, &m->rec_out.w, &m->rec_out.b, &m->pitch_out.w, &m->pitch_out.b,
                       &m->adj_ih.w, &m->adj_ih.b, &m->adj_hh, &m->adj_out.w, &m->adj_out.b};
    for (DevBuf* b : order) {
        const std::vector<char>& v = x.image[b];
        if (!v.empty()) STEP(b->upload(v.data(), v.size()));
    }
    m->store.host.clear();
    m->finalized = true;
    m->packed_once = true;
    return AMTX_OK;
}

extern "C" int amtx_of_model_set_tensor_device(amtx_of_model* m, const char* name, const float* device_data, int64_t numel) {
    AMTX_REQUIRE(m && name && device_data && numel > 0, "amtx_of_model_set_tensor_device: bad argument");
    m->store.set_device(name, device_data, numel);
    return AMTX_OK;
}

extern "C" int amtx_of_model_finalize_device(amtx_of_model* m, void* stream_) {
    AMTX_REQUIRE(m, "amtx_of_model_finalize_device: null model");
    struct Clear {
        amtx_of_model* m;
        ~Clear() { m->store.device.clear(); }
    } clear{m};
    AMTX_REQUIRE(m->finalized, "amtx_of_model_finalize_device: the first sync goes through amtx_of_model_finalize (it allocates the packed buffers)");
    if (!m->plan.device_resync) {
        amtx_set_error("amtx_of_model_finalize_device: no device packer for conv.hip's multi-channel first conv; use amtx_of_model_finalize");
        return AMTX_ERR_UNSUPPORTED;
    }
    DevicePack x{m, (hipStream_t)stream_, true};
    STEP(pack_model(m, x));
    STEP(amtx_quiesce_before_resync(m->packed_once));
    x.dry = false;
    const int rc = pack_model(m, x);
    if (rc != AMTX_OK) m->finalized = false;
    return rc;
}

extern "C" size_t amtx_of_workspace_bytes(const amtx_of_model* m, int batch, int num_frames) {
    if (!m || batch <= 0 || num_frames <= 0) return 0;
    return carve(m, batch, num_frames, nullptr).total;
}

static GemmArgs gemm_args(const void* A, int64_t lda, int a_type, const LinearPack& lp, int planes, void* C, int64_t ldc, int c_type,
                          int64_t M, int groups, int64_t a_gs, int64_t c_gs) {
    GemmArgs g;
    g.A = A; g.lda = lda; g.a_type = a_type;
    g.W = (const bf16_t*)lp.w.p; g.n_pad = lp.n_pad; g.k_pad = lp.k_pad; g.planes = planes;
    g.bias = (const float*)lp.b.p;
    g.C = C; g.ldc = ldc; g.c_type = c_type;
    g.M = M; g.N = lp.N; g.K = lp.K;
    g.groups = groups; g.a_gs = a_gs; g.w_gs = (int64_t)lp.n_pad * lp.k_pad * planes; g.bias_gs = lp.N; g.c_gs = c_gs;
    return g;
}

struct FeatsIn { const float* feats; const void* feats16; int64_t stride_b, stride_c, stride_t, stride_f; const float *clip_max, *ref; };

template <class Mark>
static int run_convs(const amtx_of_model* m, const ConvCall& call, const FeatsIn& in, const Workspace& w, int B, int T, hipStream_t s, Mark&& mark) {
    const ConvPlan& p = m->plan;
    const KernelSet* k = m->k;
    const int64_t BT = (int64_t)B * T;
    const int F = m->dim_in, F2 = F / 2, at = m->act_type, pl = m->planes, nh = m->n_heads;
    int rc;
    if (call.path == PATH_CONV1) {
        Conv1Args c1;
        c1.in = in.feats; c1.stride_b = in.stride_b; c1.stride_c = in.stride_c; c1.stride_t = in.stride_t; c1.stride_f = in.stride_f;
        c1.w = (const float*)m->conv1_w.p; c1.shift = (const float*)m->conv_s[0].p; c1.out = w.a1; c1.out_type = at;
        c1.B = B; c1.T = T; c1.F = F; c1.c_in = m->in_channels; c1.c_out = m->nf1;
        c1.groups = nh; c1.w_gs = (int64_t)m->nf1 * m->in_channels * 9; c1.shift_gs = m->nf1; c1.out_gs = BT * F * m->nf1;
        if ((rc = k->launch_conv1(c1, s)) != AMTX_OK) return rc;
    }
    mark();
    ConvArgs c2;
    c2.in = w.a1; c2.in_type = at; c2.wfrag = (const bf16_t*)m->conv_w[1].p; c2.planes = pl; c2.shift = (const float*)m->conv_s[1].p;
    c2.out = w.a2; c2.out_type = at; c2.B = B; c2.T = T; c2.F = F; c2.c_out = m->nf2;
    c2.groups = nh; c2.in_gs = BT * F * m->nf1; c2.shift_gs = m->nf2; c2.w_gs = (int64_t)p.layer[1].frag_per; c2.out_gs = BT * F2 * m->nf2;
    const int64_t a2_split = BT * F2 * m->nf2 * nh, a3_split = BT * m->kfc_pad * nh;
    if (p.two_plane_acts) { c2.out_type = AMTX_T_SPLIT; c2.out_split = a2_split; }
    if (p.conv1_fused) {
        c2.in = nullptr;
        c2.feats = in.feats; c2.f_stride_b = in.stride_b; c2.f_stride_c = in.stride_c; c2.f_stride_t = in.stride_t; c2.f_stride_f = in.stride_f;
        c2.c_in = m->in_channels; c2.w1frag = (const bf16_t*)m->conv_w[0].p; c2.shift1 = (const float*)m->conv_s[0].p; c2.w1_gs = (int64_t)p.layer[0].frag_per;
        c2.f_clip_max = in.clip_max; c2.f_ref = in.ref;
        if (in.feats16) { c2.feats = nullptr; c2.feats16 = in.feats16; }
    }
    if (call.path == PATH_CONVX12) { c2.in_split = BT * F * 8; c2.wfrag = (const bf16_t*)m->conv2_wx.p; c2.w_gs = (int64_t)p.c2x_per; }
    if (call.path == PATH_STACK)
        rc = k->launch_conv_stack(c2, (const bf16_t*)m->conv_w[2].p, (int64_t)p.layer[2].frag_per, (const float*)m->conv_s[2].p, w.a3, BT * m->kfc_pad, call.a3_plane, s);
    else if (call.path == PATH_CONVX12) rc = amtx_launch_convx12(c2, s);
    else rc = p.layer[1].fam == K_CONVG ? k->launch_conv3x3_gen(c2, m->nf1, s) : k->launch_conv3x3(c2, s);
    if (rc != AMTX_OK) return rc;
    mark();
    ConvArgs c3 = c2;
    c3.feats = nullptr; c3.feats16 = nullptr; c3.w1frag = nullptr; c3.shift1 = nullptr; c3.c_in = 0;
    c3.in = w.a2; c3.wfrag = (const bf16_t*)m->conv_w[2].p; c3.shift = (const float*)m->conv_s[2].p; c3.out = w.a3;
    c3.F = F2; c3.c_out = m->nf3; c3.in_gs = BT * F2 * m->nf2; c3.w_gs = (int64_t)p.layer[2].frag_per; c3.shift_gs = m->nf3; c3.out_gs = BT * m->kfc_pad;
    if (p.two_plane_acts) { c3.in_type = AMTX_T_SPLIT; c3.in_split = a2_split; c3.out_type = AMTX_T_SPLIT; c3.out_split = a3_split; }
    if (m->kfc_pad != m->kfc) {
        AMTX_REQUIRE(p.layer[2].fam == K_CONVG, "amtx_of_forward: internal: padded fc1 rows need the general conv kernel");
        c3.out_ts = m->kfc_pad;
        const size_t es = amtx_tsize(at);
        if ((rc = amtx_launch_zero_cols(w.a3 + (size_t)m->kfc * es, (int64_t)m->kfc_pad * es, (int)((m->kfc_pad - m->kfc) * es), BT * nh, s)) != AMTX_OK) return rc;
    }
    if (call.path != PATH_STACK && (rc = p.layer[2].fam == K_CONVG ? k->launch_conv3x3_gen(c3, m->nf2, s) : k->launch_conv3x3(c3, s)) != AMTX_OK) return rc;
    mark();
    return AMTX_OK;
}

static int of_forward_impl(const amtx_of_model* m, const FeatsIn& in, int B, int T, void* workspace, size_t workspace_bytes, float* out_onsets,
                           float* out_multi_pitch, float* logits_onsets, float* logits_multi_pitch, float* logits_pitch_head, void* stream_) {
    AMTX_REQUIRE(m && m->finalized, "amtx_of_forward: model not finalized");
    AMTX_REQUIRE(!in.clip_max || m->plan.fuses_db_scale, "amtx_of_forward_power: this model does not stage its features in the conv kernel");
    AMTX_REQUIRE(!in.feats16 || m->plan.takes_feats16, "amtx_of_forward_feats16: this model does not stage 16-bit channels-last features");
    AMTX_REQUIRE((in.feats || in.feats16) && workspace, "amtx_of_forward: null pointer");
    AMTX_REQUIRE(B > 0 && T > 0, "amtx_of_forward: bad batch/num_frames");
    Workspace w = carve(m, B, T, (char*)workspace);
    AMTX_REQUIRE(workspace_bytes >= w.total, "amtx_of_forward: workspace too small (%zu < %zu)", workspace_bytes, w.total);
    AMTX_REQUIRE(((uintptr_t)workspace % 256) == 0, "amtx_of_forward: workspace must be 256-byte aligned");
    hipStream_t s = (hipStream_t)stream_;
    const int64_t BT = (int64_t)B * T;
    const int at = m->act_type, pl = m->planes;
    const KernelSet* k = m->k;
    int rc;
    std::vector<hipEvent_t>* evs = nullptr;
    if (m->prof) {
        m->prof_events.emplace_back();
        evs = &m->prof_events.back();
    }
    auto mark = [&]() {
        if (!evs) return;
        hipEvent_t e;
        if (hipEventCreate(&e) == hipSuccess) { (void)hipEventRecord(e, s); evs->push_back(e); }
    };
    mark();

    const ConvCall call = resolve_conv(m, B, T, in.feats16 != nullptr);
    if ((rc = run_convs(m, call, in, w, B, T, s, mark)) != AMTX_OK) return rc;
    const bool sp = m->plan.two_plane_acts, no_roll_epi = m->plan.no_roll_epilogue;
    const int64_t a3_plane = call.a3_plane, a3_split = BT * m->kfc_pad * m->n_heads, e_split = BT * m->dim_am * m->n_heads;

    const int at_d = sp ? AMTX_T_SPLIT : at;
    GemmArgs g = gemm_args(w.a3, m->kfc_pad, at_d, m->fc1, pl, w.e, m->dim_am, at_d, BT, m->n_rec, BT * m->kfc_pad, BT * m->dim_am);
    g.a_plane = a3_plane; g.a_split = a3_split; g.c_split = e_split;
    if ((rc = k->launch_gemm(g, s)) != AMTX_OK) return rc;
    mark();

    g = gemm_args(w.e, m->dim_am, at_d, m->rec_ih, pl, w.xp, m->xw, at, BT, m->n_rec, BT * m->dim_am, BT * m->xw);
    g.a_split = e_split;
    if ((rc = k->launch_gemm(g, s)) != AMTX_OK) return rc;
    mark();
    LstmArgs l;
    l.xproj = w.xp; l.x_type = at; l.whh = (const bf16_t*)m->rec_hh.p; l.planes = pl; l.out = w.l1; l.out_type = at;
    l.B = B; l.T = T; l.groups = m->n_rec; l.x_gs = BT * m->xw; l.w_gs = (int64_t)m->hh_elems; l.out_gs = BT * m->dim_lm;
    l.hidden = m->hid;
    if ((rc = k->launch_bilstm(l, s)) != AMTX_OK) return rc;
    mark();
    g = gemm_args(w.l1, m->dim_lm, at, m->rec_out, pl, w.joint, m->dim_aj, AMTX_T_F32, BT, m->n_rec, BT * m->dim_lm, m->n_out);
    const bool roll_on = out_onsets && !no_roll_epi && amtx_gemm_has_roll_epilogue(g);
    if (roll_on) { g.roll_out = out_onsets; g.roll_T = T; g.roll_thr = 0.5f; g.roll_group = 0; }
    const int kp = (m->dim_aj + 63) / 64 * 64;
    GemmArgs gp = gemm_args(w.a3 + (size_t)(m->n_heads - 1) * BT * m->kfc_pad * (sp ? 2 : amtx_tsize(at)), m->kfc_pad, at_d, m->pitch_out, pl,
                            w.joint + (size_t)m->n_rec * m->n_out * sizeof(float), m->dim_aj, AMTX_T_F32, BT, 1, 0, 0);
    gp.a_plane = a3_plane; gp.a_split = a3_split;
    const bool copy_on = pl == 1 && !no_roll_epi && amtx_gemm_has_roll_epilogue(g) && amtx_gemm_has_roll_epilogue(gp) && m->n_out % 4 == 0 &&
                         (kp - m->dim_aj) % 4 == 0 && gp.N + (kp - m->dim_aj) <= gp.n_pad;
    if (copy_on) {
        g.copy16 = (bf16_t*)w.joint16; g.copy16_ld = kp; g.copy16_col0 = 0; g.copy16_gs = m->n_out; g.copy16_pad = 0;
        gp.copy16 = (bf16_t*)w.joint16; gp.copy16_ld = kp; gp.copy16_col0 = m->n_rec * m->n_out; gp.copy16_gs = 0; gp.copy16_pad = kp - m->dim_aj;
        if (roll_on && !logits_onsets && !logits_pitch_head && !m->has_offsets) { g.C = nullptr; gp.C = nullptr; }
    }
    if ((rc = k->launch_gemm(g, s)) != AMTX_OK) return rc;
    mark();
    if ((rc = k->launch_gemm(gp, s)) != AMTX_OK) return rc;
    mark();

    if (pl == 1) {
        if (!copy_on && (rc = amtx_launch_cvt_pad_bf16((const float*)w.joint, m->dim_aj, m->dim_aj, (bf16_t*)w.joint16, kp, BT, s, m->f16)) != AMTX_OK) return rc;
        g = gemm_args(w.joint16, kp, AMTX_T_BF16, m->adj_ih, pl, w.xp2, m->xw, at, BT, 1, 0, 0);
        g.K = kp;
    } else if (sp) {
        if ((rc = amtx_launch_cvt_split((const float*)w.joint, m->dim_aj, m->dim_aj, (bf16_t*)w.joint16, kp, BT * kp, BT, s)) != AMTX_OK) return rc;
        g = gemm_args(w.joint16, kp, AMTX_T_SPLIT, m->adj_ih, pl, w.xp2, m->xw, at, BT, 1, 0, 0);
        g.K = kp; g.a_split = BT * kp;
    } else {
        g = gemm_args(w.joint, m->dim_aj, AMTX_T_F32, m->adj_ih, pl, w.xp2, m->xw, at, BT, 1, 0, 0);
    }
    if ((rc = k->launch_gemm(g, s)) != AMTX_OK) return rc;
    mark();
    l.xproj = w.xp2; l.whh = (const bf16_t*)m->adj_hh.p; l.out = w.l2; l.groups = 1;
    if ((rc = k->launch_bilstm(l, s)) != AMTX_OK) return rc;
    mark();
    g = gemm_args(w.l2, m->dim_lm, at, m->adj_out, pl, w.mp, m->n_out, AMTX_T_F32, BT, 1, 0, 0);
    const bool roll_mp = out_multi_pitch && !no_roll_epi && amtx_gemm_has_roll_epilogue(g);
    if (roll_mp) {
        g.roll_out = out_multi_pitch; g.roll_T = T; g.roll_thr = 0.5f; g.roll_group = 0;
        if (!logits_multi_pitch) g.C = nullptr;
    }
    if ((rc = k->launch_gemm(g, s)) != AMTX_OK) return rc;
    mark();

    if (out_onsets && !roll_on && (rc = amtx_launch_pianoroll((const float*)w.joint, m->dim_aj, 0, B, T, m->n_out, 0.5f, out_onsets, s)) != AMTX_OK) return rc;
    if (out_multi_pitch && !roll_mp && (rc = amtx_launch_pianoroll((const float*)w.mp, m->n_out, 0, B, T, m->n_out, 0.5f, out_multi_pitch, s)) != AMTX_OK) return rc;

    mark();
    const size_t row = (size_t)m->n_out * sizeof(float);
    if (logits_onsets)
        AMTX_CHECK_HIP(hipMemcpy2DAsync(logits_onsets, row, w.joint, (size_t)m->dim_aj * 4, row, BT, hipMemcpyDeviceToDevice, s));
    if (logits_pitch_head)
        AMTX_CHECK_HIP(hipMemcpy2DAsync(logits_pitch_head, row, w.joint + (size_t)m->n_rec * row, (size_t)m->dim_aj * 4, row, BT,
                                        hipMemcpyDeviceToDevice, s));
    if (logits_multi_pitch)
        AMTX_CHECK_HIP(hipMemcpyAsync(logits_multi_pitch, w.mp, row * BT, hipMemcpyDeviceToDevice, s));
    return AMTX_OK;
}

extern "C" int amtx_of_fuses_db_scale(const amtx_of_model* m) { return m && m->finalized && m->plan.fuses_db_scale; }
extern "C" int amtx_of_conv_stack_fused(const amtx_of_model* m, int batch, int num_frames) { return m && resolve_conv(m, batch, num_frames, false).path == PATH_STACK; }

extern "C" int amtx_of_forward(const amtx_of_model* m, const float* feats, int64_t stride_b, int64_t stride_c, int64_t stride_t,
                               int64_t stride_f, int batch, int num_frames, void* workspace, size_t workspace_bytes,
                               float* out_onsets, float* out_multi_pitch, float* logits_onsets, float* logits_multi_pitch,
                               float* logits_pitch_head, void* stream_) {
    return of_forward_impl(m, {feats, nullptr, stride_b, stride_c, stride_t, stride_f, nullptr, nullptr}, batch, num_frames, workspace, workspace_bytes,
                           out_onsets, out_multi_pitch, logits_onsets, logits_multi_pitch, logits_pitch_head, stream_);
}

extern "C" int amtx_of_forward_power(const amtx_of_model* m, const float* power, int64_t stride_b, int64_t stride_t, int64_t stride_f,
                                     const float* clip_max, const float* ref, int batch, int num_frames, void* workspace,
                                     size_t workspace_bytes, float* out_onsets, float* out_multi_pitch, float* logits_onsets,
                                     float* logits_multi_pitch, float* logits_pitch_head, void* stream_) {
    AMTX_REQUIRE(clip_max, "amtx_of_forward_power: clip_max is null");
    return of_forward_impl(m, {power, nullptr, stride_b, 0, stride_t, stride_f, clip_max, ref}, batch, num_frames, workspace, workspace_bytes,
                           out_onsets, out_multi_pitch, logits_onsets, logits_multi_pitch, logits_pitch_head, stream_);
}

extern "C" int amtx_of_takes_feats16(const amtx_of_model* m) { return m && m->finalized ? m->plan.takes_feats16 : 0; }

extern "C" int amtx_of_forward_feats16(const amtx_of_model* m, const void* feats16, int batch, int num_frames, void* workspace, size_t workspace_bytes,
                                       float* out_onsets, float* out_multi_pitch, float* logits_onsets, float* logits_multi_pitch,
                                       float* logits_pitch_head, void* stream_) {
    AMTX_REQUIRE(feats16, "amtx_of_forward_feats16: feats16 is null");
    return of_forward_impl(m, {nullptr, feats16, 0, 0, 0, 0, nullptr, nullptr}, batch, num_frames, workspace, workspace_bytes, out_onsets, out_multi_pitch,
                           logits_onsets, logits_multi_pitch, logits_pitch_head, stream_);
}

extern "C" int amtx_of_offsets(const amtx_of_model* m, void* workspace, size_t workspace_bytes, int batch, int num_frames, float* out_offsets,
                               float* logits_offsets, void* stream_) {
    AMTX_REQUIRE(m && m->finalized, "amtx_of_offsets: model not finalized");
    AMTX_REQUIRE(m->has_offsets, "amtx_of_offsets: the model has no offset head");
    AMTX_REQUIRE(workspace && batch > 0 && num_frames > 0, "amtx_of_offsets: bad argument");
    Workspace w = carve(m, batch, num_frames, (char*)workspace);
    AMTX_REQUIRE(workspace_bytes >= w.total, "amtx_of_offsets: workspace too small");
    hipStream_t s = (hipStream_t)stream_;
    const int64_t BT = (int64_t)batch * num_frames;
    int rc;
    if (out_offsets && (rc = amtx_launch_pianoroll((const float*)w.joint, m->dim_aj, m->n_out, batch, num_frames, m->n_out, -1.0f, out_offsets, s)) != AMTX_OK)
        return rc;
    const size_t row = (size_t)m->n_out * sizeof(float);
    if (logits_offsets)
        AMTX_CHECK_HIP(hipMemcpy2DAsync(logits_offsets, row, w.joint + row, (size_t)m->dim_aj * 4, row, BT, hipMemcpyDeviceToDevice, s));
    return AMTX_OK;
}

extern "C" int amtx_of_num_stages(void) { return ST_COUNT; }
extern "C" const char* amtx_of_stage_name(int i) { return (i >= 0 && i < ST_COUNT) ? kStageNames[i] : ""; }

extern "C" int amtx_of_profile_enable(amtx_of_model* m, int enable) {
    AMTX_REQUIRE(m, "amtx_of_profile_enable: null model");
    for (auto& v : m->prof_events)
        for (hipEvent_t e : v) (void)hipEventDestroy(e);
    m->prof_events.clear();
    m->prof = enable != 0;
    return AMTX_OK;
}

extern "C" int amtx_of_profile_read(amtx_of_model* m, double* stage_ms, int* num_forwards) {
    AMTX_REQUIRE(m && stage_ms && num_forwards, "amtx_of_profile_read: null argument");
    for (int i = 0; i < ST_COUNT; ++i) stage_ms[i] = 0.0;
    *num_forwards = 0;
    for (auto& v : m->prof_events) {
        if ((int)v.size() != ST_COUNT + 1) continue;
        AMTX_CHECK_HIP(hipEventSynchronize(v.back()));
        for (int i = 0; i < ST_COUNT; ++i) {
            float ms = 0.f;
            AMTX_CHECK_HIP(hipEventElapsedTime(&ms, v[i], v[i + 1]));
            stage_ms[i] += ms;
        }
        ++*num_forwards;
    }
    return AMTX_OK;
}
```

amt_tools_amd/models.py:

```python

import ctypes as C

import numpy as np
import os

import torch
import torch.nn.functional as F
from torch import nn

from . import _lib, tools

__all__ = ['TranscriptionModel', 'OutputLayer', 'LogisticBank', 'AcousticModel', 'LanguageModel', 'OnsetsFrames',
           'SpectralFrontend']


class TranscriptionModel(nn.Module):

    def __init__(self, dim_in, profile, in_channels=1, model_complexity=1, frame_width=1, device='cpu'):
        nn.Module.__init__(self)
        self.dim_in = dim_in
        self.profile = profile
        self.in_channels = in_channels
        self.model_complexity = model_complexity
        self.frame_width = frame_width
        self.device = device
        self.iter = 0
        self.frontend = nn.Sequential()

    _engine_class = None
    _transient = ('_engine',)

    def __getstate__(self):
        state = dict(self.__dict__)
        for key in self._transient:
            state.pop(key, None)
        return state

    def _get_engine(self, device):
        eng = self.__dict__.get('_engine')
        if eng is None or eng.device != device:
            eng = self._engine_class(self, device)
            self.__dict__['_engine'] = eng
        eng.sync_weights(self)
        return eng

    def change_device(self, device=None):
        if device is None:
            device = self.device
        if isinstance(device, int):
            device = torch.device(f'cuda:{device}' if torch.cuda.is_available() else 'cpu')
        self.device = device
        self.to(self.device)
        if torch.device(self.device).type == 'cuda':
            self.to(memory_format=torch.channels_last)
        for m in self.frontend:
            mod = getattr(m, 'module', None)
            if mod is not None and hasattr(mod, 'change_device'):
                mod.change_device(self.device)

    def pre_proc(self, batch):
        batch = tools.dict_to_device(batch, self.device)
        audio = tools.unpack_dict(batch, tools.KEY_AUDIO)
        feats = tools.unpack_dict(batch, tools.KEY_FEATS)
        from .tracks import TrackClips
        if isinstance(audio, TrackClips):
            frontend_feats = self._clips_module(audio).process_clips(audio, model_layout=True).transpose(-1, -2)
            feats = frontend_feats if feats is None else torch.cat((feats, frontend_feats), dim=1)
        elif audio is not None and len(self.frontend):
            frontend_feats = self.frontend(audio.unsqueeze(-2))
            feats = frontend_feats if feats is None else torch.cat((feats, frontend_feats), dim=1)
        batch[tools.KEY_FEATS] = feats
        return batch

    def _clips_module(self, clips):
        from .features import _SpecPlanOwner, _index_of
        module = self.frontend[0].module if len(self.frontend) == 1 and isinstance(self.frontend[0], SpectralFrontend) else None
        if not isinstance(module, _SpecPlanOwner):
            raise TypeError('a TrackClips batch needs a model whose frontend is exactly one SpectralFrontend over an STFT / MelSpec module')
        if torch.device(self.device).type != 'cuda' or _index_of(self.device) != clips.device.index:
            raise ValueError(f'the clips live on {clips.device}, the model on {self.device}')
        return module

    def forward(self, feats):
        raise NotImplementedError

    def post_proc(self, batch):
        raise NotImplementedError

    def run_on_batch(self, batch):
        batch = self.pre_proc(batch)
        batch[tools.KEY_OUTPUT] = self(batch[tools.KEY_FEATS])
        output = self.post_proc(batch)
        if tools.query_dict(batch, tools.KEY_TIMES):
            output[tools.KEY_TIMES] = batch[tools.KEY_TIMES]
        return output

    @classmethod
    def model_name(cls):
        return cls.__name__


class OutputLayer(nn.Module):
    def __init__(self, dim_in, dim_out, weights=None):
        super().__init__()
        self.dim_in = dim_in
        self.dim_out = dim_out
        self.weights = None
        if weights is not None:
            self.set_weights(np.asarray(weights).flatten())

    def set_weights(self, weights, device='cpu'):
        if isinstance(device, int):
            device = torch.device(f'cuda:{device}' if torch.cuda.is_available() else 'cpu')
        self.weights = torch.Tensor(weights).to(device)


class LogisticBank(OutputLayer):

    def __init__(self, dim_in, dim_out, weights=None):
        super().__init__(dim_in, dim_out, weights)
        self.output_layer = nn.Linear(self.dim_in, self.dim_out)

    def forward(self, feats):
        if feats.is_cuda and torch.is_grad_enabled():
            from .autograd import linear, linear_supported, note_fallback
            if linear_supported(feats, self.output_layer.weight):
                return linear(feats, self.output_layer.weight, self.output_layer.bias)
            note_fallback('LogisticBank.output_layer', f'Linear {self.dim_in} -> {self.dim_out}, {feats.dtype}')
        return self.output_layer(feats)

    def get_loss(self, estimated, reference):
        if (estimated.is_cuda and estimated.dtype == torch.float32 and estimated.dim() == 3 and reference.dim() == 3
                and reference.shape == (estimated.shape[0], estimated.shape[2], estimated.shape[1])):
            from .autograd import bce_logits_loss
            return bce_logits_loss(estimated, reference, self.weights)
        if estimated.is_cuda and torch.is_grad_enabled() and estimated.requires_grad:
            from .autograd import note_fallback
            note_fallback('LogisticBank.get_loss', f'logits {tuple(estimated.shape)} {estimated.dtype} vs labels {tuple(reference.shape)}')
        est = estimated.transpose(-2, -1)
        weight = self.weights.unsqueeze(-1) if self.weights is not None else None
        loss = F.binary_cross_entropy_with_logits(est.float(), reference.float(), weight=weight, reduction='none')
        return loss.mean(dim=-1).sum(dim=-1).mean()

    def finalize_output(self, raw_output, threshold=None):
        final = torch.sigmoid(raw_output.clone().detach()).transpose(-2, -1)
        if threshold is not None:
            final = tools.threshold_activations(final.contiguous(), threshold)
        return final


class AcousticModel(nn.Module):

    def __init__(self, dim_in, dim_out, in_channels=1, model_complexity=2):
        super().__init__()
        nf1 = nf2 = 16 * model_complexity
        nf3 = 32 * model_complexity
        self.layer1 = nn.Sequential(nn.Conv2d(in_channels, nf1, (3, 3), padding=1), nn.BatchNorm2d(nf1), nn.ReLU())
        self.layer2 = nn.Sequential(nn.Conv2d(nf1, nf2, (3, 3), padding=1), nn.BatchNorm2d(nf2), nn.ReLU(),
                                    nn.MaxPool2d((1, 2)), nn.Dropout(0.25))
        self.layer3 = nn.Sequential(nn.Conv2d(nf2, nf3, (3, 3), padding=1), nn.BatchNorm2d(nf3), nn.ReLU(),
                                    nn.MaxPool2d((1, 2)), nn.Dropout(0.25))
        self.fc1 = nn.Sequential(nn.Linear(nf3 * (dim_in // 4), dim_out), nn.Dropout(0.50))

    use_hip_bn = True

    def _stage(self, layer, x):
        mods = list(layer)
        if self.training and self.use_hip_bn and x.is_cuda and not isinstance(mods[1], nn.SyncBatchNorm):
            from .autograd import bn_relu_pool, bn_relu_pool_supported, conv3x3, conv3x3_supported, note_fallback
            if conv3x3_supported(x, mods[0]):
                y = conv3x3(x, mods[0])
            else:
                note_fallback('AcousticModel conv', f'Conv2d {mods[0].in_channels} -> {mods[0].out_channels} on {x.dtype}')
                y = mods[0](x)
            if bn_relu_pool_supported(y, mods[1]):
                pool = len(mods) > 3 and isinstance(mods[3], nn.MaxPool2d)
                y = bn_relu_pool(y, mods[1], pool)
                for m in mods[(4 if pool else 3):]:
                    y = m(y)
                return y
            note_fallback('AcousticModel BatchNorm+ReLU+MaxPool', f'{y.shape[1]} channels, {y.dtype}, channels_last={y.is_contiguous(memory_format=torch.channels_last)}')
            for m in mods[1:]:
                y = m(y)
            return y
        if self.training and x.is_cuda:
            from .autograd import note_fallback
            note_fallback('AcousticModel stage', 'use_hip_bn off' if not self.use_hip_bn else 'SyncBatchNorm (stock modules by design: its statistics are a collective)')
        return layer(x)

    def forward(self, in_feats):
        x = self._stage(self.layer3, self._stage(self.layer2, self._stage(self.layer1, in_feats)))
        if (self.training and x.is_cuda and x.dim() == 4 and x.is_contiguous(memory_format=torch.channels_last)
                and not x.is_contiguous()):
            lin = self.fc1[0]
            B, C, T, F = x.shape
            w = lin.weight.view(lin.out_features, C, F).transpose(1, 2).reshape(lin.out_features, F * C)
            from .autograd import linear, linear_supported, note_fallback
            xin = x.permute(0, 2, 3, 1).reshape(B, T, F * C)
            if linear_supported(xin, w):
                y = linear(xin, w, lin.bias)
            else:
                note_fallback('AcousticModel.fc1', f'Linear {w.shape[1]} -> {w.shape[0]}, {xin.dtype}')
                y = torch.nn.functional.linear(xin, w, lin.bias)
            for m in list(self.fc1)[1:]:
                y = m(y)
            return y
        if self.training and x.is_cuda:
            from .autograd import note_fallback
            note_fallback('AcousticModel.fc1', 'conv map not in channels-last layout')
        x = x.transpose(-3, -2).flatten(-2)
        return self.fc1(x)


class LanguageModel(nn.Module):

    def __init__(self, dim_in, dim_out, chunk_len=512, bidirectional=True):
        super().__init__()
        self.dim_in = dim_in
        self.dim_out = dim_out
        self.chunk_len = chunk_len
        self.num_directions = int(bidirectional) + 1
        self.hidden_size = self.dim_out // self.num_directions
        self.mlm = nn.LSTM(input_size=self.dim_in, hidden_size=self.hidden_size, batch_first=True, bidirectional=bidirectional)
        self.use_hip_autograd = True

    def forward(self, in_feats):
        from .autograd import HIDDEN_SIZES
        if (in_feats.is_cuda and in_feats.dtype == torch.float32 and self.num_directions == 2 and self.hidden_size in HIDDEN_SIZES
                and self.mlm.num_layers == 1 and self.use_hip_autograd):
            from .autograd import bilstm
            return bilstm(in_feats, self.mlm)
        if in_feats.is_cuda and torch.is_grad_enabled():
            from .autograd import note_fallback
            note_fallback('LanguageModel', f'nn.LSTM hidden {self.hidden_size} x {self.num_directions} directions, {in_feats.dtype}, '
                                           f'use_hip_autograd={self.use_hip_autograd}')
        return self.mlm(in_feats)[0]


class SpectralFrontend(nn.Module):

    def __init__(self, module):
        super().__init__()
        self.module = module

    def forward(self, audio):
        assert audio.dim() == 3 and audio.shape[1] == 1
        from .features import _SpecPlanOwner
        if isinstance(self.module, _SpecPlanOwner):
            feats = self.module.process_batch(audio[:, 0].float(), model_layout=True)
            return feats.transpose(-1, -2)
        return self.module.process_batch(audio[:, 0].float())


def _pick_side_stream(device, candidates=6, spins=20, spin_cycles=20000):
    import time
    sleep = getattr(torch.cuda, '_sleep', None)
    main = torch.cuda.current_stream(device)
    first = None
    try:
        with torch.cuda.device(device):
            def chains(streams):
                torch.cuda.synchronize(device)
                t0 = time.perf_counter()
                for st in streams:
                    with torch.cuda.stream(st):
                        for _ in range(spins):
                            sleep(spin_cycles)
                for st in streams:
                    st.synchronize()
                return time.perf_counter() - t0
            for _ in range(candidates):
                s = torch.cuda.Stream(device=device)
                first = first or s
                if sleep is None:
                    return s
                chains((main, s))
                one = min(chains((main,)) for _ in range(2))
                if min(chains((main, s)) for _ in range(2)) < 1.7 * one:
                    return s
    except Exception:
        pass
    return first or torch.cuda.Stream(device=device)


class PendingFeatures(object):

    def __init__(self, module, power, clip_max, ref=None):
        self.module, self.power, self.clip_max, self.ref = module, power, clip_max, ref

    @property
    def device(self):
        return self.power.device

    def materialize(self):
        return self.module.scale_batch(self.power, self.clip_max, self.ref, model_layout=True)


class PendingFeatures16(PendingFeatures):

    def __init__(self, module, feats16, audio):
        self.module, self.feats16, self.audio = module, feats16, audio

    @property
    def device(self):
        return self.feats16.device

    def materialize(self):
        return self.module.process_batch(self.audio).transpose(-1, -2)


class _EngineBase(object):

    ABI = None

    def __init__(self, device, *create_args):
        self.device = device
        self.handle = C.c_void_p()
        _lib.call(self.ABI + '_create', C.byref(self.handle), *create_args, device=device)
        self.version = None
        self.workspace = None

    def sync_weights(self, model):
        items = [(k, v) for k, v in model.state_dict().items() if v.dtype.is_floating_point and not k.startswith('frontend.') and v.numel() > 0]
        version = tuple((k, v._version, v.data_ptr()) for k, v in items)
        if version == self.version:
            return
        if self.version is None or not self._resync_on_device(items):
            flat = torch.cat([v.detach().reshape(-1).to(torch.float32) for _, v in items]).cpu().numpy()
            off = 0
            for k, v in items:
                n = v.numel()
                _lib.call(self.ABI + '_set_tensor', self.handle, k.encode(), flat[off:off + n], n)
                off += n
            _lib.call(self.ABI + '_finalize', self.handle, device=self.device)
        self.version = version

    def _resync_on_device(self, items):
        return False

    def _grow_workspace(self, need, device):
        if self.workspace is None or self.workspace.numel() < need:
            self.workspace = None
            self.workspace = _lib.alloc_workspace(need, device)

    def __del__(self):
        try:
            _lib.call(self.ABI + '_destroy', self.handle)
        except Exception:
            pass


class _OFEngine(_EngineBase):

    ABI = 'amtx_of_model'

    def __init__(self, model, device):
        self.n_out = model.profile.get_range_len()
        super().__init__(device, int(model.dim_in), int(model.in_channels), int(model.model_complexity), int(self.n_out),
                         int(model.has_offsets), {'bf16': 0, 'x3': 1, 'f16': 2}[model.precision])
        self.device_sync = os.environ.get('AMTX_HOST_WEIGHT_SYNC') is None
        self.device_syncs = 0

    def _resync_on_device(self, items):
        if not (self.device_sync and all(v.is_cuda and v.device == torch.device(self.device) and v.dtype == torch.float32 for _, v in items)):
            return False
        keep = []
        for k, v in items:
            t = v.detach()
            t = t if t.is_contiguous() else t.contiguous()
            keep.append(t)
            _lib.call('amtx_of_model_set_tensor_device', self.handle, k.encode(), t, t.numel())
        with torch.cuda.device(self.device):
            rc = _lib.lib().amtx_of_model_finalize_device(self.handle, _lib.current_stream(self.device))
            if keep and rc == 0:
                torch.cuda.current_stream(self.device).synchronize()
        del keep
        if rc == 0:
            self.device_syncs += 1
            return True
        if rc != _lib.ERR_UNSUPPORTED:
            _lib.check(rc, 'amtx_of_model_finalize_device')
        self.device_sync = False
        return False

    def fuses_db_scale(self):
        return bool(_lib.call('amtx_of_fuses_db_scale', self.handle))

    def takes_feats16(self):
        return int(_lib.call('amtx_of_takes_feats16', self.handle))

    def conv_stack_fused(self, batch, num_frames):
        return bool(_lib.call('amtx_of_conv_stack_fused', self.handle, int(batch), int(num_frames)))

    def forward(self, feats, want_logits=True):
        pending = feats if isinstance(feats, PendingFeatures) else None
        pending16 = isinstance(pending, PendingFeatures16)
        if pending16:
            feats = pending.feats16
            B, T = feats.shape[-4], feats.shape[-3]
        elif pending is not None:
            feats = pending.power.unsqueeze(1)
        if not pending16:
            B, Cc, T, Fd = feats.shape
        self._grow_workspace(_lib.call('amtx_of_workspace_bytes', self.handle, B, T), feats.device)
        n_out = self.n_out
        opts = dict(dtype=torch.float32, device=feats.device)
        onsets = torch.empty((B, n_out, T), **opts)
        multi_pitch = torch.empty((B, n_out, T), **opts)
        lo = torch.empty((B, T, n_out), **opts) if want_logits else None
        lm = torch.empty((B, T, n_out), **opts) if want_logits else None
        lp = torch.empty((B, T, n_out), **opts) if want_logits else None
        sb, sc, st, sf = (0, 0, 0, 0) if pending16 else feats.stride()
        ws, outs = self.workspace, (onsets, multi_pitch, lo, lm, lp)
        if pending16:
            _lib.call('amtx_of_forward_feats16', self.handle, feats, B, T, ws, ws.numel(), *outs, device=feats.device)
        elif pending is not None:
            _lib.call('amtx_of_forward_power', self.handle, feats, sb, st, sf, pending.clip_max, pending.ref, B, T, ws, ws.numel(), *outs,
                      device=feats.device)
        else:
            _lib.call('amtx_of_forward', self.handle, feats, sb, sc, st, sf, B, T, ws, ws.numel(), *outs, device=feats.device)
        self._last = (B, T)
        return onsets, multi_pitch, lo, lm, lp

    def offsets(self, device, want_logits=True):
        B, T = self._last
        opts = dict(dtype=torch.float32, device=device)
        prob = torch.empty((B, self.n_out, T), **opts)
        logits = torch.empty((B, T, self.n_out), **opts) if want_logits else None
        _lib.call('amtx_of_offsets', self.handle, self.workspace, self.workspace.numel(), B, T, prob, logits, device=device)
        return prob, logits


class OnsetsFrames(TranscriptionModel):

    has_offsets = False

    def __init__(self, dim_in, profile, in_channels=1, model_complexity=2, detach_heads=False, device='cpu',
                 precision='x3'):
        super().__init__(dim_in, profile, in_channels, model_complexity, 1, device)
        assert precision in ('bf16', 'x3', 'f16')
        self.detach_heads = detach_heads
        self.precision = precision
        self.dim_am = 256 * self.model_complexity
        self.dim_lm = 256 * (self.model_complexity - 1)
        dim_out = self.profile.get_range_len()
        self.onset_head = nn.Sequential(AcousticModel(self.dim_in, self.dim_am, self.in_channels, self.model_complexity),
                                        LanguageModel(self.dim_am, self.dim_lm), LogisticBank(self.dim_lm, dim_out))
        self.pitch_head = nn.Sequential(AcousticModel(self.dim_in, self.dim_am, self.in_channels, self.model_complexity),
                                        LogisticBank(self.dim_am, dim_out))
        self.dim_aj = 2 * dim_out
        self.adjoin = nn.Sequential(LanguageModel(self.dim_aj, self.dim_lm), LogisticBank(self.dim_lm, dim_out))

    _engine_class = _OFEngine
    _transient = TranscriptionModel._transient + ('_engine_out', '_engine_offsets', '_side_stream', '_overlap_armed', '_fb_last_forward',
                                                  '_overlap_latched_off')

    def pre_proc(self, batch):
        pending = self._deferred_scale(batch) if self.__dict__.get('_in_run_on_batch') else None
        if pending is not None:
            return pending
        batch = super().pre_proc(batch)
        batch[tools.KEY_FEATS] = batch[tools.KEY_FEATS].transpose(-1, -2)
        return batch

    def _deferred_scale(self, batch):
        if self.training or len(self.frontend) != 1 or not isinstance(self.frontend[0], SpectralFrontend):
            return None
        if os.environ.get('AMTX_DEFER_DB_SCALE', '1') == '0':
            return None
        from .features import _SpecPlanOwner, _CqtPlanOwner
        module = self.frontend[0].module
        cqt = isinstance(module, _CqtPlanOwner)
        if cqt:
            if os.environ.get('AMTX_CQT_FEATS16', '1') == '0':
                return None
        elif not isinstance(module, _SpecPlanOwner) or not getattr(module, 'decibels', False):
            return None
        if tools.query_dict(batch, tools.KEY_FEATS) or not tools.query_dict(batch, tools.KEY_AUDIO):
            return None
        if torch.device(self.device).type != 'cuda':
            return None
        batch = tools.dict_to_device(batch, self.device)
        audio = batch[tools.KEY_AUDIO]
        from .tracks import TrackClips
        if isinstance(audio, TrackClips):
            if cqt or not self._get_engine(audio.device).fuses_db_scale():
                return None
            power, track_max = self._clips_module(audio).power_clips(audio)
            batch[tools.KEY_FEATS] = PendingFeatures(module, power, clip_max=track_max)
            return batch
        if not (torch.is_tensor(audio) and audio.is_cuda and audio.dim() == 2):
            return None
        if cqt:
            form = self._get_engine(audio.device).takes_feats16()
            if not form:
                return None
            if int(getattr(module, 'n_bins', -1)) != int(self.dim_in) or int(module.get_num_channels()) != int(self.in_channels):
                return None
            audio = audio.float()
            batch[tools.KEY_FEATS] = PendingFeatures16(module, module.process_batch16(audio, split=(form == 2)), audio)
            return batch
        if not self._get_engine(audio.device).fuses_db_scale():
            return None
        power, clip_max = module.power_batch(audio.float())
        batch[tools.KEY_FEATS] = PendingFeatures(module, power, clip_max)
        return batch

    def run_on_batch(self, batch):
        labelled = any(tools.query_dict(batch, k) for k in (tools.KEY_MULTIPITCH, tools.KEY_ONSETS, tools.KEY_OFFSETS))
        self.__dict__['_logits_wanted'] = labelled
        self.__dict__['_in_run_on_batch'] = True
        try:
            return super().run_on_batch(batch)
        finally:
            self.__dict__.pop('_logits_wanted', None)
            self.__dict__.pop('_in_run_on_batch', None)

    def forward(self, feats):
        pending = isinstance(feats, PendingFeatures)
        if pending and self.training:
            feats, pending = feats.materialize(), False
        if pending or (feats.is_cuda and not self.training):
            eng = self._get_engine(feats.device)
            if not pending and feats.dtype != torch.float32:
                feats = feats.float()
            want = self.__dict__.get('_logits_wanted', True)
            onsets_bin, mp_bin, lo, lm, lp = eng.forward(feats if pending else feats.detach(), want_logits=want)
            if not want:
                lo, lm = onsets_bin, mp_bin
            output = {tools.KEY_ONSETS: lo, tools.KEY_MULTIPITCH: lm}
            self.__dict__['_engine_out'] = (lo, lm, onsets_bin, mp_bin, lp)
            if self.has_offsets:
                prob, logits = eng.offsets(feats.device, want_logits=want)
                output[tools.KEY_OFFSETS] = logits if want else prob
                self.__dict__['_engine_offsets'] = (output[tools.KEY_OFFSETS], prob)
            return output
        self.__dict__.pop('_engine_out', None)
        self.__dict__.pop('_engine_offsets', None)
        output = dict()
        fb0 = None
        if feats.is_cuda and self.training and torch.is_grad_enabled():
            from . import autograd as _ag
            fb0 = _ag.fallback_total()
        if self._overlap_heads(feats):
            main = torch.cuda.current_stream(feats.device)
            side = self.__dict__.get('_side_stream')
            if side is None or side.device != feats.device:
                side = _pick_side_stream(feats.device)
                self.__dict__['_side_stream'] = side
            side.wait_stream(main)
            feats.record_stream(side)
            with torch.cuda.stream(side):
                multi_pitch = self.pitch_head(feats)
            onsets, offsets = self._recurrent_heads(feats)
            main.wait_stream(side)
            multi_pitch.record_stream(main)
        else:
            multi_pitch = self.pitch_head(feats)
            onsets, offsets = self._recurrent_heads(feats)
        output[tools.KEY_ONSETS] = onsets
        heads = [onsets]
        if self.has_offsets:
            output[tools.KEY_OFFSETS] = offsets
            heads.append(offsets)
        if self.detach_heads:
            heads = [h.clone().detach() for h in heads]
        joint = torch.cat(heads + [multi_pitch], -1)
        output[tools.KEY_MULTIPITCH] = self.adjoin(joint)
        if fb0 is not None:
            self.__dict__['_fb_last_forward'] = _ag.fallback_total() - fb0
            if self.__dict__['_fb_last_forward']:
                self.__dict__['_overlap_latched_off'] = True
        return output

    def _overlap_heads(self, feats):
        if not (feats.is_cuda and self.training and torch.is_grad_enabled()):
            return False
        if os.environ.get('AMTX_TRAIN_OVERLAP', '1') == '0' or not self.__dict__.get('overlap_heads', True):
            return False
        from . import autograd as ag
        if not ag.USE_HIP_DENSE:
            return False
        if self.__dict__.get('_overlap_latched_off', False):
            return False
        if self.__dict__.get('_fb_last_forward', None) != 0:
            return False
        return True

    def _recurrent_heads(self, feats):
        if self._grouped_recurrences(feats):
            from .autograd import bilstm_multi
            (am_on, lm_on, lb_on), (am_off, lm_off, lb_off) = self.onset_head, self.offset_head
            l_on, l_off = bilstm_multi([am_on(feats), am_off(feats)], [lm_on.mlm, lm_off.mlm])
            return lb_on(l_on), lb_off(l_off)
        onsets = self.onset_head(feats)
        offsets = self.offset_head(feats) if self.has_offsets else None
        return onsets, offsets

    def _grouped_recurrences(self, feats):
        if not (self.has_offsets and feats.is_cuda and self.training and feats.dtype == torch.float32):
            return False
        from .autograd import HIDDEN_SIZES
        lms = (self.onset_head[1], self.offset_head[1])
        return all(isinstance(lm, LanguageModel) and lm.use_hip_autograd and lm.num_directions == 2 and lm.mlm.num_layers == 1
                   and lm.hidden_size in HIDDEN_SIZES for lm in lms) and lms[0].hidden_size == lms[1].hidden_size

    def post_proc(self, batch):
        output = batch[tools.KEY_OUTPUT]
        onset_layer, pitch_layer = self.onset_head[-1], self.adjoin[-1]
        onsets_est, multi_pitch_est = output[tools.KEY_ONSETS], output[tools.KEY_MULTIPITCH]
        if tools.KEY_MULTIPITCH in batch.keys():
            loss = dict()
            multi_pitch_ref = batch[tools.KEY_MULTIPITCH]
            loss[tools.KEY_LOSS_PITCH] = pitch_layer.get_loss(multi_pitch_est, multi_pitch_ref)
            if tools.KEY_ONSETS in batch.keys():
                onsets_ref = batch[tools.KEY_ONSETS]
            else:
                onsets_ref = tools.multi_pitch_to_onsets(multi_pitch_ref)
            loss[tools.KEY_LOSS_ONSETS] = onset_layer.get_loss(onsets_est, onsets_ref)
            loss[tools.KEY_LOSS_TOTAL] = loss[tools.KEY_LOSS_PITCH] + loss[tools.KEY_LOSS_ONSETS]
            output[tools.KEY_LOSS] = loss
        cached = self.__dict__.pop('_engine_out', None)
        if cached is not None and cached[0] is onsets_est and cached[1] is multi_pitch_est:
            output[tools.KEY_ONSETS], output[tools.KEY_MULTIPITCH] = cached[2], cached[3]
        else:
            output[tools.KEY_ONSETS] = onset_layer.finalize_output(onsets_est, 0.5)
            output[tools.KEY_MULTIPITCH] = pitch_layer.finalize_output(multi_pitch_est, 0.5)
        return output

    def engine_logits(self, feats_bcft):
        feats = feats_bcft.transpose(-1, -2)
        eng = self._get_engine(feats.device)
        onsets_bin, mp_bin, lo, lm, lp = eng.forward(feats.float())
        return {'onsets': lo, 'multi_pitch': lm, 'pitch_head': lp, 'onsets_bin': onsets_bin, 'multi_pitch_bin': mp_bin}


class OnsetsFrames2(OnsetsFrames):

    has_offsets = True

    def __init__(self, dim_in, profile, in_channels=1, model_complexity=3, detach_heads=True, device='cpu', precision='x3'):
        super().__init__(dim_in, profile, in_channels, model_complexity, detach_heads, device, precision)
        dim_out = self.profile.get_range_len()
        self.offset_head = nn.Sequential(AcousticModel(self.dim_in, self.dim_am, self.in_channels, self.model_complexity),
                                         LanguageModel(self.dim_am, self.dim_lm), LogisticBank(self.dim_lm, dim_out))
        self.dim_aj += dim_out
        self.adjoin[0] = LanguageModel(self.dim_aj, self.dim_lm)

    def post_proc(self, batch):
        output = super().post_proc(batch)
        offset_layer = self.offset_head[-1]
        offsets_est = output[tools.KEY_OFFSETS]
        if tools.KEY_LOSS in output.keys():
            if tools.KEY_OFFSETS in batch.keys():
                offsets_ref = batch[tools.KEY_OFFSETS]
            else:
                offsets_ref = tools.multi_pitch_to_offsets(batch[tools.KEY_MULTIPITCH])
            loss = output[tools.KEY_LOSS]
            offsets_loss = offset_layer.get_loss(offsets_est, offsets_ref)
            loss[tools.KEY_LOSS_OFFSETS] = offsets_loss
            loss[tools.KEY_LOSS_TOTAL] += offsets_loss
            output[tools.KEY_LOSS] = loss
        cached = self.__dict__.pop('_engine_offsets', None)
        if cached is not None and cached[0] is offsets_est:
            output[tools.KEY_OFFSETS] = cached[1]
        else:
            output[tools.KEY_OFFSETS] = offset_layer.finalize_output(offsets_est)
        return output

    def engine_logits(self, feats_bcft):
        out = super().engine_logits(feats_bcft)
        prob, logits = self._get_engine(feats_bcft.device).offsets(feats_bcft.device)
        out['offsets'], out['offsets_prob'] = logits, prob
        return out


class SoftmaxGroups(OutputLayer):

    def __init__(self, dim_in, num_groups, num_classes, weights=None):
        self.num_groups = num_groups
        self.num_classes = num_classes
        super().__init__(dim_in, num_groups * num_classes, weights)
        self.output_layer = nn.Linear(self.dim_in, self.dim_out)

    def forward(self, feats):
        return self.output_layer(feats)

    def _grouped(self, logits):
        return logits.reshape(logits.shape[0], -1, self.num_groups, self.num_classes)

    def get_loss(self, estimated, reference):
        log_prob = torch.log_softmax(self._grouped(estimated).float(), dim=-1)
        target = reference.transpose(-2, -1).long()
        target = torch.where(target < 0, torch.full_like(target, self.num_classes - 1), target)
        nll = -log_prob.gather(-1, target.unsqueeze(-1)).squeeze(-1)
        if self.weights is not None:
            per_class = self.weights.to(nll.device).reshape(self.num_groups, self.num_classes)
            group_idx = torch.arange(self.num_groups, device=nll.device).expand_as(target)
            nll = nll * per_class[group_idx, target]
        return nll.sum(dim=-1).mean(dim=-1).mean()

    def finalize_output(self, raw_output, last_negative=True):
        winners = torch.softmax(self._grouped(raw_output.detach()), dim=-1).argmax(dim=-1)
        if last_negative:
            winners = torch.where(winners == self.num_classes - 1, torch.full_like(winners, -1), winners)
        return winners.transpose(-2, -1)


def tab_window_view(feats, frame_width=9):
    if not torch.is_tensor(feats) or feats.dim() != 5 or feats.shape[-1] != frame_width or feats.dtype != torch.float32:
        return None
    B, T, Cc, Fd, W = feats.shape
    sb, st, sc, sf, sw = feats.stride()
    if st != sw or st <= 0 or min(sb, sc, sf) < 0 or min(B, T, Cc, Fd) <= 0:
        return None
    ncols = T + W - 1
    off = feats.storage_offset()
    last = off + (B - 1) * sb + (Cc - 1) * sc + (Fd - 1) * sf + (ncols - 1) * st
    if off < 0 or (last + 1) * feats.element_size() > feats.untyped_storage().nbytes():
        return None
    return dict(offset=off, num_windows=T, num_cols=ncols, strides=(sb, sc, sf, st))


class _TabEngine(_EngineBase):

    ABI = 'amtx_tab_model'
    WORKSPACE_CAP = 1 << 30

    def __init__(self, model, device):
        self.G = int(model.profile.get_num_dofs())
        self.C = int(model.profile.num_pitches + 1)
        super().__init__(device, int(model.dim_in), int(model.in_channels), int(model.model_complexity), self.G, self.C,
                         {'bf16': 0, 'x3': 1}[model.precision])
        self.forwards = 0

    def workspace_bytes(self, batch, num_windows):
        return int(_lib.call('amtx_tab_workspace_bytes', self.handle, int(batch), int(num_windows)))

    def _chunks(self, B, T):
        cap = self.WORKSPACE_CAP
        if self.workspace_bytes(B, T) <= cap:
            return [(0, B, 0, T)]
        bc = B
        while bc > 1 and self.workspace_bytes(bc, 1) > cap:
            bc = (bc + 1) // 2
        lo, hi = 1, T
        while lo < hi:
            mid = (lo + hi + 1) // 2
            if self.workspace_bytes(bc, mid) <= cap:
                lo = mid
            else:
                hi = mid - 1
        return [(b0, min(B, b0 + bc), t0, min(T, t0 + lo)) for b0 in range(0, B, bc) for t0 in range(0, T, lo)]

    def forward(self, feats, view):
        B, T = feats.shape[:2]
        sb, sc, sf, st = view['strides']
        G, Cn = self.G, self.C
        logits = torch.empty((B, T, G * Cn), dtype=torch.float32, device=feats.device)
        tab = torch.empty((B, G, T), dtype=torch.int64, device=feats.device)
        chunks = self._chunks(B, T)
        self._grow_workspace(max(self.workspace_bytes(b1 - b0, t1 - t0) for b0, b1, t0, t1 in chunks), feats.device)
        base = feats.data_ptr()
        esz = feats.element_size()
        for b0, b1, t0, t1 in chunks:
            whole = len(chunks) == 1
            lg = logits if whole else torch.empty((b1 - b0, t1 - t0, G * Cn), dtype=torch.float32, device=feats.device)
            tb = tab if whole else torch.empty((b1 - b0, G, t1 - t0), dtype=torch.int64, device=feats.device)
            ptr = base + (b0 * sb + t0 * st) * esz
            _lib.call('amtx_tab_forward', self.handle, ptr, sb, sc, sf, st, b1 - b0, t1 - t0, self.workspace, self.workspace.numel(), lg, tb,
                      device=feats.device)
            if not whole:
                logits[b0:b1, t0:t1] = lg
                tab[b0:b1, :, t0:t1] = tb
        self.forwards += 1
        return logits, tab


class TabCNN(TranscriptionModel):

    CONTEXT = 9
    use_hip_train = True

    def __init__(self, dim_in, profile, in_channels=1, model_complexity=1, device='cpu', precision='x3'):
        super().__init__(dim_in, profile, in_channels, model_complexity, self.CONTEXT, device)
        assert precision in ('bf16', 'x3')
        self.precision = precision
        self.online = False
        widths = (32 * model_complexity, 64 * model_complexity, 64 * model_complexity)
        layers, c_prev = [], self.in_channels
        for c in widths:
            layers += [nn.Conv2d(c_prev, c, (3, 3)), nn.ReLU()]
            c_prev = c
        self.conv = nn.Sequential(*layers, nn.MaxPool2d((2, 2)), nn.Dropout(0.25))
        self.conv_embedding_size = widths[-1] * ((self.dim_in - 6) // 2) * ((self.frame_width - 6) // 2)
        self.fc_embedding_size = 128 * model_complexity
        self.dense = nn.Sequential(nn.Linear(self.conv_embedding_size, self.fc_embedding_size), nn.ReLU(), nn.Dropout(0.50),
                                   SoftmaxGroups(self.fc_embedding_size, self.profile.get_num_dofs(), self.profile.num_pitches + 1))

    _engine_class = _TabEngine
    _transient = TranscriptionModel._transient + ('_engine_tab',)

    def engine_unsupported(self):
        C_ = self.profile.num_pitches + 1
        G = self.profile.get_num_dofs()
        if self.model_complexity != 1:
            return f'model_complexity={self.model_complexity} (1 is built)'
        if not 1 <= self.in_channels <= 8:
            return f'in_channels={self.in_channels} (1 to 8 are built)'
        if not 9 <= self.dim_in <= 2048:
            return f'dim_in={self.dim_in} (9 to 2048 are built)'
        if C_ > 32 or G * C_ > 256:
            return f'num_classes={C_}, num_groups={G} (num_classes <= 32 and num_groups x num_classes <= 256 are built)'
        return None

    def _engine_view(self, feats):
        if not (torch.is_tensor(feats) and feats.is_cuda and feats.dtype == torch.float32 and not self.training):
            return None
        if torch.is_grad_enabled() and (feats.requires_grad or any(p.requires_grad for p in self.parameters())):
            return None
        view = tab_window_view(feats, self.frame_width)
        if view is None or tuple(feats.shape[2:4]) != (self.in_channels, self.dim_in):
            return None
        why = self.engine_unsupported()
        if why is not None:
            from . import autograd
            autograd.note_fallback('TabCNN.forward', f'no HIP engine for {why}')
            return None
        return view

    def toggle_online(self):
        self.online = not self.online

    def pre_proc(self, batch):
        batch = super().pre_proc(batch)
        feats = batch[tools.KEY_FEATS]
        W = self.frame_width
        if not self.online:
            feats = F.pad(feats, (W // 2, W // 2))
        elif feats.shape[-1] < W:
            feats = F.pad(feats, ((W - feats.shape[-1]) // 2, W - feats.shape[-1] - (W - feats.shape[-1]) // 2))
        windows = feats.unfold(-1, W, 1)
        batch[tools.KEY_FEATS] = windows.permute(0, 3, 1, 2, 4)
        return batch

    def train_unsupported(self, feats):
        from . import autograd
        if not self.use_hip_train:
            return 'TabCNN.use_hip_train is off'
        if not autograd.USE_HIP_DENSE:
            return 'autograd.USE_HIP_DENSE is off'
        if feats.dtype != torch.float32:
            return f'{feats.dtype} features'
        if tab_window_view(feats, self.frame_width) is None:
            return 'the windows are not a shared-window view (a contiguous copy?)'
        if tuple(feats.shape[2:4]) != (self.in_channels, self.dim_in):
            return f'feature shape {tuple(feats.shape[2:4])} is not ({self.in_channels}, {self.dim_in})'
        if self.dim_in < 8:
            return f'dim_in={self.dim_in}'
        for i, idx in enumerate((0, 2, 4)):
            if not autograd.tab_conv_supported(self.conv[idx], i > 0 or feats.requires_grad):
                return f'conv.{idx} ({self.conv[idx]})'
        if not isinstance(self.conv[6], nn.MaxPool2d) or self.conv[6].kernel_size not in (2, (2, 2)):
            return 'conv.6 is not MaxPool2d((2, 2))'
        fc, out = self.dense[0], self.dense[-1].output_layer
        if fc.weight.dtype != torch.float32 or fc.in_features % 4 or fc.out_features % 4 or out.in_features % 4:
            return f'dense layers {fc.in_features} -> {fc.out_features} -> {out.out_features}'
        return None

    def _forward_hip_train(self, feats):
        from . import autograd
        view = tab_window_view(feats, self.frame_width)
        B, T = feats.shape[:2]
        sb, sc, sf, st = view['strides']
        seq = feats.as_strided((B, self.in_channels, view['num_cols'], self.dim_in), (sb, sc, st, sf), view['offset'])
        y = torch.relu(autograd.tab_conv3x3(seq, self.conv[0]))
        y = torch.relu(autograd.tab_conv3x3(y, self.conv[2]))
        y = autograd.tab_conv3x3(y, self.conv[4])
        x = self.conv[-1](autograd.tab_window_pool(y, T))
        fc = self.dense[0]
        x = self.dense[2](torch.relu(autograd.linear(x, fc.weight, fc.bias)))
        head = self.dense[-1].output_layer
        n = head.out_features
        pad = (-n) % 4
        w = F.pad(head.weight, (0, 0, 0, pad)) if pad else head.weight
        b = F.pad(head.bias, (0, pad)) if pad else head.bias
        logits = autograd.linear(x, w, b)[:, :n]
        return logits.reshape(B, T, n)

    def forward(self, feats):
        self.__dict__.pop('_engine_tab', None)
        if self.training and torch.is_tensor(feats) and feats.is_cuda:
            from . import autograd
            why = self.train_unsupported(feats)
            if why is None:
                return {tools.KEY_TABLATURE: self._forward_hip_train(feats)}
            autograd.note_fallback('TabCNN.train', why)
        view = self._engine_view(feats)
        if view is not None:
            logits, tab = self._get_engine(feats.device).forward(feats.detach(), view)
            self.__dict__['_engine_tab'] = (logits, tab)
            return {tools.KEY_TABLATURE: logits}
        B, T = feats.shape[:2]
        embeddings = self.conv(feats.reshape(B * T, self.in_channels, self.dim_in, self.frame_width))
        return {tools.KEY_TABLATURE: self.dense(embeddings.reshape(B, T, -1))}

    def post_proc(self, batch):
        output = batch[tools.KEY_OUTPUT]
        head = self.dense[-1]
        logits = output[tools.KEY_TABLATURE]
        if tools.KEY_TABLATURE in batch:
            labels = batch[tools.KEY_TABLATURE]
            if (self.training and self.use_hip_train and logits.is_cuda and logits.dtype == torch.float32 and logits.dim() == 3
                    and tuple(labels.shape) == (logits.shape[0], head.num_groups, logits.shape[1])):
                from .autograd import softmax_groups_loss
                loss = softmax_groups_loss(logits, labels, head.num_groups, head.num_classes, head.weights)
            else:
                loss = head.get_loss(logits, labels)
            output[tools.KEY_LOSS] = {tools.KEY_LOSS_TOTAL: loss}
        engine = self.__dict__.pop('_engine_tab', None)
        if engine is not None and engine[0] is logits:
            output[tools.KEY_TABLATURE] = engine[1]
        else:
            output[tools.KEY_TABLATURE] = head.finalize_output(logits)
        return output
```

include/amtx.h:

```cpp
#ifndef AMTX_H
#define AMTX_H

#include <stddef.h>
#include <stdint.h>

#ifdef __cplusplus
extern "C" {
#endif

#define AMTX_OK 0
#define AMTX_ERR_ARG (-1)
#define AMTX_ERR_HIP (-2)
#define AMTX_ERR_UNSUPPORTED (-3)

#define AMTX_PREC_BF16 0
#define AMTX_PREC_X3 1
#define AMTX_PREC_F16 2

const char* amtx_last_error(void);
int amtx_version(void);

typedef struct amtx_spec_plan amtx_spec_plan;

#define AMTX_PAD_CONSTANT 0
#define AMTX_PAD_REFLECT 1

int amtx_spec_plan_create(amtx_spec_plan** plan, int sample_rate, int n_fft, int hop_length, int win_length,
                          int n_mels, int htk, int center, int pad_mode);
int amtx_spec_mel_layout(int sample_rate, int n_fft, int n_mels, int htk, int32_t* slot_row, int32_t* slot_start, int32_t* round_max);
int amtx_spec_plan_destroy(amtx_spec_plan* plan);
int amtx_spec_num_bins(const amtx_spec_plan* plan);
int64_t amtx_spec_num_frames(const amtx_spec_plan* plan, int64_t num_samples);
int amtx_spec_filterbank(const amtx_spec_plan* plan, float* host_out);

int amtx_spec_power(const amtx_spec_plan* plan, const float* audio, int64_t num_samples, int64_t audio_stride,
                    int batch, float* power, float* clip_max, void* stream);

#define AMTX_LAYOUT_BFT_F32 0
#define AMTX_LAYOUT_BTF_F32 1
#define AMTX_SCALE_DB 0
#define AMTX_SCALE_POWER 1
#define AMTX_SCALE_MAGNITUDE 2
int amtx_spec_scale(const amtx_spec_plan* plan, const float* power, const float* clip_max, const float* ref,
                    int batch, int64_t num_frames, int transform, int layout, float* out, void* stream);

typedef struct amtx_of_model amtx_of_model;

int amtx_of_model_create(amtx_of_model** model, int dim_in, int in_channels, int model_complexity, int n_out,
                         int has_offsets, int precision );
int amtx_has_f16(void);
int amtx_of_model_destroy(amtx_of_model* model);
int amtx_of_model_set_tensor(amtx_of_model* model, const char* name, const float* host_data, int64_t numel);
int amtx_of_model_finalize(amtx_of_model* model);
size_t amtx_of_workspace_bytes(const amtx_of_model* model, int batch, int num_frames);
int amtx_of_forward(const amtx_of_model* model, const float* feats, int64_t stride_b, int64_t stride_c, int64_t stride_t,
                    int64_t stride_f, int batch, int num_frames, void* workspace, size_t workspace_bytes,
                    float* out_onsets, float* out_multi_pitch, float* logits_onsets, float* logits_multi_pitch,
                    float* logits_pitch_head, void* stream);

int amtx_of_fuses_db_scale(const amtx_of_model* model);
int amtx_of_forward_power(const amtx_of_model* model, const float* power, int64_t stride_b, int64_t stride_t, int64_t stride_f,
                          const float* clip_max, const float* ref, int batch, int num_frames, void* workspace, size_t workspace_bytes,
                          float* out_onsets, float* out_multi_pitch, float* logits_onsets, float* logits_multi_pitch,
                          float* logits_pitch_head, void* stream);

int amtx_of_takes_feats16(const amtx_of_model* model);
int amtx_of_forward_feats16(const amtx_of_model* model, const void* feats16, int batch, int num_frames, void* workspace, size_t workspace_bytes,
                            float* out_onsets, float* out_multi_pitch, float* logits_onsets, float* logits_multi_pitch,
                            float* logits_pitch_head, void* stream);

int amtx_of_model_set_tensor_device(amtx_of_model* model, const char* name, const float* device_data, int64_t numel);
int amtx_of_model_finalize_device(amtx_of_model* model, void* stream);

int amtx_of_conv_stack_fused(const amtx_of_model* model, int batch, int num_frames);

int amtx_of_offsets(const amtx_of_model* model, void* workspace, size_t workspace_bytes, int batch, int num_frames, float* out_offsets,
                    float* logits_offsets, void* stream);

int amtx_of_num_stages(void);
const char* amtx_of_stage_name(int stage);
int amtx_of_profile_enable(amtx_of_model* model, int enable);
int amtx_of_profile_read(amtx_of_model* model, double* stage_ms , int* num_forwards);

int64_t amtx_linear_packed_elems(int n, int k, int planes);
int amtx_linear_pack(const float* host_w, int n, int k, int planes, uint16_t* host_out);
int amtx_linear_fwd(const void* a, int64_t lda, int a_type, const uint16_t* w_packed, int planes, const float* bias, void* c,
                    int64_t ldc, int c_type, int64_t m, int n, int k, void* stream);
int amtx_split_planes(const float* src, int64_t ld_src, int n, uint16_t* dst, int ld_dst, int64_t split, int64_t rows, void* stream);
int amtx_linear_fwd_split(const void* a, int64_t lda, int64_t a_split, const uint16_t* w_packed, const float* bias, void* c, int64_t ldc,
                          int c_type, int64_t c_split, int64_t m, int n, int k, void* stream);
int64_t amtx_conv3x3_packed_elems(int c_out, int planes);
int amtx_conv3x3_pack(const float* host_w , const float* host_scale , int c_out, int planes,
                      uint16_t* host_out);
int amtx_conv3x3_fwd(const void* in, int elem_type, const uint16_t* w_packed, int planes, const float* shift, void* out, int batch,
                     int num_frames, int num_bins, int c_out, void* stream);
int64_t amtx_conv3x3g_packed_elems(int c_in, int c_out, int planes);
int amtx_conv3x3g_pack(const float* host_w , const float* host_scale , int c_in, int c_out, int planes,
                       uint16_t* host_out);
int amtx_conv3x3g_fwd(const void* in, int elem_type, const uint16_t* w_packed, int planes, const float* shift, void* out, int batch,
                      int num_frames, int num_bins, int c_in, int c_out, void* stream);
int amtx_conv1_fwd(const float* feats, int64_t stride_b, int64_t stride_c, int64_t stride_t, int64_t stride_f, const float* w,
                   const float* shift, void* out, int out_type, int batch, int num_frames, int num_bins, int c_in, int c_out,
                   void* stream);
int64_t amtx_bilstm_packed_elems(int planes);
int amtx_bilstm_pack(const float* host_whh_fwd, const float* host_whh_bwd , int planes, uint16_t* host_out);
int amtx_bilstm_fwd(const void* xproj , const uint16_t* whh_packed, int planes, int elem_type, void* out ,
                    int batch, int num_frames, void* stream);
int64_t amtx_bilstm_h_packed_elems(int hidden, int planes);
int amtx_bilstm_h_pack(const float* host_whh_fwd, const float* host_whh_bwd, int hidden, int planes, uint16_t* host_out);
int amtx_bilstm_h_fwd(const void* xproj, const uint16_t* whh_packed, int hidden, int planes, int elem_type, void* out, int batch,
                      int num_frames, void* stream);
int amtx_bilstm_pack_device(const float* whh_fwd, const float* whh_bwd, int planes, uint16_t* frag_fwd, uint16_t* frag_bwd, void* stream);
int amtx_bilstm_train_fwd(const float* xproj, const uint16_t* whh_packed, int planes, float* out, float* save, int batch, int num_frames,
                          void* stream);
int amtx_bilstm_train_bwd(const float* dout, const float* save, const uint16_t* whh_t_packed, int planes, float* dxproj, int batch,
                          int num_frames, void* stream);
int amtx_bilstm_h_pack_device(const float* whh_fwd, const float* whh_bwd, int hidden, int planes, uint16_t* frag_fwd, uint16_t* frag_bwd,
                              void* stream);
int amtx_bilstm_h_train_fwd(const float* xproj, const uint16_t* whh_packed, int hidden, int planes, float* out, float* save, int batch,
                            int num_frames, int groups, void* stream);
int amtx_bilstm_h_train_bwd(const float* dout, const float* save, const uint16_t* whh_t_packed, int hidden, int planes, float* dxproj,
                            int batch, int num_frames, int groups, void* stream);
size_t amtx_bn_train_workspace_bytes(int channels);
int amtx_bn_relu_pool_train_fwd(const float* x, int64_t rows, int num_bins, int channels, int pool, const float* gamma, const float* beta,
                                float eps, float momentum, float* running_mean, float* running_var, float* y, float* stats,
                                void* workspace, size_t workspace_bytes, void* stream);
int amtx_bn_relu_pool_train_bwd(const float* x, int64_t rows, int num_bins, int channels, int pool, const float* stats, const float* dy,
                                float* dx, float* dgamma, float* dbeta, void* workspace, size_t workspace_bytes, void* stream);
size_t amtx_bce_logits_loss_workspace_bytes(int batch, int num_frames, int keys);
int amtx_bce_logits_loss(const float* logits, int64_t ld, const float* labels, const float* weight, int batch, int num_frames, int keys,
                         float* loss, float* grad, void* workspace, size_t workspace_bytes, void* stream);
size_t amtx_matmul_workspace_bytes(int64_t m, int64_t n, int64_t k);
int amtx_matmul_f32(const float* a, int64_t lda, int a_trans, const float* b, int64_t ldb, int b_trans, const float* bias, float* c, int64_t ldc,
                    int64_t m, int64_t n, int64_t k, void* workspace, size_t workspace_bytes, void* stream);
int amtx_linear_train_fwd(const float* x, int64_t ldx, const float* w, int64_t ldw, const float* bias, float* y, int64_t ldy, int64_t m, int n,
                          int k, void* stream);
size_t amtx_linear_bwd_workspace_bytes(int64_t m, int n, int k);
int amtx_linear_bwd(const float* dy, int64_t lddy, const float* x, int64_t ldx, const float* w, int64_t ldw, float* dx, int64_t lddx, float* dw,
                    float* db, int64_t m, int n, int k, void* workspace, size_t workspace_bytes, void* stream);
size_t amtx_conv3x3_train_workspace_bytes(int64_t rows, int num_bins, int c_in, int c_out);
int amtx_conv3x3_train_fwd(const float* x, const float* w, const float* bias, float* y, int64_t rows, int frames_per_clip, int num_bins, int c_in,
                           int c_out, void* workspace, size_t workspace_bytes, void* stream);
int amtx_conv3x3_bwd(const float* dy, const float* x, const float* w, float* dx, float* dw, float* db, int64_t rows, int frames_per_clip,
                     int num_bins, int c_in, int c_out, void* workspace, size_t workspace_bytes, void* stream);
int amtx_pianoroll_fwd(const float* logits, int64_t ld, int col0, int batch, int num_frames, int keys, float threshold, float* out,
                       void* stream);

typedef struct amtx_cqt_plan amtx_cqt_plan;
int amtx_cqt_plan_create(amtx_cqt_plan** plan, int sample_rate, int hop_length, double fmin, int n_bins, int bins_per_octave,
                         double gamma, const double* harmonics, int n_harmonics, int truncate_to_expected, int librosa09);
int amtx_cqt_plan_destroy(amtx_cqt_plan* plan);
int amtx_cqt_num_harmonics(const amtx_cqt_plan* plan);
int64_t amtx_cqt_num_frames(const amtx_cqt_plan* plan, int64_t num_samples);
size_t amtx_cqt_workspace_bytes(const amtx_cqt_plan* plan, int batch, int64_t num_samples);
int amtx_cqt_forward(const amtx_cqt_plan* plan, const float* audio, int64_t num_samples, int64_t audio_stride, int batch, int decibels,
                     void* workspace, size_t workspace_bytes, float* out, void* stream);
int amtx_cqt_forward16(const amtx_cqt_plan* plan, const float* audio, int64_t num_samples, int64_t audio_stride, int batch, int decibels,
                       void* workspace, size_t workspace_bytes, void* out16, void* stream);
int amtx_cqt_forward16_split(const amtx_cqt_plan* plan, const float* audio, int64_t num_samples, int64_t audio_stride, int batch, int decibels,
                             void* workspace, size_t workspace_bytes, void* out16, int64_t plane_elems, void* stream);

size_t amtx_rms_norm_workspace_bytes(int batch, int64_t num_samples);
int amtx_rms_norm(const float* audio, int64_t num_samples, int64_t audio_stride, int batch, float* out, int64_t out_stride,
                  void* workspace, size_t workspace_bytes, void* stream);

int amtx_notes_decode(const float* onsets, const float* multi_pitch, int batch, int keys, int num_frames, int capacity,
                      int32_t* pairs, int32_t* counts, void* stream);

int amtx_notes_rows(const int32_t* pairs, const int32_t* counts, int batch, int keys, int capacity, const double* times_ext,
                    int64_t times_stride, int low_pitch, double* rows, double* onset_col, int64_t rows_capacity, int32_t* clip_offsets,
                    void* stream);

int amtx_tab_expand(const int64_t* tablature, int batch, int strings, int num_frames, const int32_t* dof_start, int num_classes,
                    int num_pitches, float* stacked, float* collapsed, void* stream);

int amtx_tab_notes(const int64_t* tablature, int batch, int strings, int num_frames, const int32_t* tuning, int num_classes,
                   const double* times_ext, int64_t times_stride, const int32_t* release, int64_t release_stride, int has_minimum_duration,
                   double minimum_duration, double* rows, int64_t rows_capacity, int32_t* row_offsets, void* stream);

int amtx_eval_multipitch_counts(const float* est, const float* ref, int batch, int slices, int keys, int num_frames, int64_t* counts,
                                void* stream);

int amtx_eval_tab_counts(const int64_t* est, const int64_t* ref, int batch, int strings, int num_frames, const int32_t* tuning, int num_classes,
                         int64_t* counts, void* stream);

#define AMTX_EVAL_MATCH_MAX_WINDOW 128
size_t amtx_eval_notes_match_workspace_bytes(int64_t est_rows, int64_t ref_rows);
int amtx_eval_notes_match(const double* est, const int32_t* est_offsets, int64_t est_rows, const double* ref, const int32_t* ref_offsets,
                          int64_t ref_rows, int groups, double onset_tolerance, double offset_ratio, double offset_min_tolerance, int decimals,
                          void* workspace, size_t workspace_bytes, int32_t* matched, int32_t* status, int wait, void* stream);

typedef struct amtx_tab_model amtx_tab_model;
int amtx_tab_model_create(amtx_tab_model** model, int dim_in, int in_channels, int model_complexity, int num_groups, int num_classes,
                          int precision );
int amtx_tab_model_destroy(amtx_tab_model* model);
int amtx_tab_model_set_tensor(amtx_tab_model* model, const char* name, const float* host, int64_t numel);
int amtx_tab_model_finalize(amtx_tab_model* model);
size_t amtx_tab_workspace_bytes(const amtx_tab_model* model, int batch, int num_windows);
int amtx_tab_forward(const amtx_tab_model* model, const float* feats, int64_t stride_b, int64_t stride_c, int64_t stride_f, int64_t stride_t,
                     int batch, int num_windows, void* workspace, size_t workspace_bytes, float* logits, int64_t* tablature, void* stream);

int amtx_tab_pool_train_fwd(const float* map, int64_t stride_b, int64_t stride_c, int64_t stride_col, int64_t stride_f, int batch,
                            int channels, int num_bins, int num_windows, float* x, uint8_t* record, void* stream);
int amtx_tab_pool_train_bwd(const float* dx, const uint8_t* record, int batch, int channels, int num_bins, int num_windows, float* dmap,
                            void* stream);
size_t amtx_softmax_groups_loss_workspace_bytes(int batch, int num_frames, int num_groups, int num_classes);
int amtx_softmax_groups_loss(const float* logits, int64_t ld, const int64_t* targets, const float* weight, int batch, int num_frames,
                             int num_groups, int num_classes, float* loss, float* grad, void* workspace, size_t workspace_bytes, void* stream);

#ifdef __cplusplus
}
#endif
#endif
```

Baseline: 41.46 million.

## Fuse adjacency LSTM input projection into the bidirectional recurrence kernel

```diff
diff --git a/amt_tools_amd/csrc/amtx_kernels.h b/amt_tools_amd/csrc/amtx_kernels.h
--- a/amt_tools_amd/csrc/amtx_kernels.h
+++ b/amt_tools_amd/csrc/amtx_kernels.h
@@ -63,6 +63,8 @@
     int groups; int64_t x_gs, w_gs, out_gs;
     int hidden = 128;
     float* save = nullptr;
+    const bf16_t* x = nullptr; int64_t ldx = 0; int kx = 0;
+    const bf16_t* wih = nullptr; int64_t ldw = 0; const float* bias = nullptr;
 };
 
 namespace amtx_bf16 {
diff --git a/amt_tools_amd/csrc/amtx_kernels_fmt.h b/amt_tools_amd/csrc/amtx_kernels_fmt.h
--- a/amt_tools_amd/csrc/amtx_kernels_fmt.h
+++ b/amt_tools_amd/csrc/amtx_kernels_fmt.h
@@ -25,6 +25,7 @@
 bool amtx_conv3x3_gen_can_fuse1(int c_in, int c_mid, int c_out, int planes);
 
 int amtx_launch_bilstm(const LstmArgs& l, hipStream_t stream);
+bool amtx_bilstm_takes_input(int hidden, int B, int kx, int64_t ldx, int64_t ldw);
 size_t amtx_bilstm_wfrag_elems(int hidden, int planes);
 void amtx_bilstm_pack_host(const float* whh_fwd, const float* whh_bwd, int hidden, int planes, bf16_t* out);
 int amtx_launch_bilstm_pack_dev(const float* whh_fwd, const float* whh_bwd, int hidden, int planes, bf16_t* frag_fwd, bf16_t* frag_bwd, hipStream_t stream);
diff --git a/amt_tools_amd/csrc/lstm.hip b/amt_tools_amd/csrc/lstm.hip
--- a/amt_tools_amd/csrc/lstm.hip
+++ b/amt_tools_amd/csrc/lstm.hip
@@ -30,9 +30,9 @@
 __device__ __forceinline__ Gates lstm_gates(float ai, float af, float ag, float ao) {
     return {sigmoid_f<FAST>(ai), sigmoid_f<FAST>(af), tanh_f<FAST>(ag), sigmoid_f<FAST>(ao)};
 }
-template <bool FAST>
+template <bool FAST, bool PIN = false>
 __device__ __forceinline__ float lstm_cell(const Gates& z, float& c) {
-    c = z.f * c + z.i * z.g;
+    c = PIN ? fmaf(c, z.f, z.i * z.g) : z.f * c + z.i * z.g;
     return z.o * tanh_f<FAST>(c);
 }
 
@@ -141,7 +141,7 @@
         float h[4];
 #pragma unroll
         for (int r = 0; r < 4; ++r) {
-            h[r] = lstm_cell<FAST>(lstm_gates<FAST>(acc[ub][0][r], acc[ub][1][r], acc[ub][2][r], acc[ub][3][r]), c[ub][r]);
+            h[r] = lstm_cell<FAST, NS == 1 && X_TYPE == AMTX_T_BF16 && OUT_TYPE == AMTX_T_BF16>(lstm_gates<FAST>(acc[ub][0][r], acc[ub][1][r], acc[ub][2][r], acc[ub][3][r]), c[ub][r]);
         }
         uint2 hiw, low;
         split16<NS>(h, hiw, low);
@@ -208,6 +208,21 @@
     }
 }
 
+#ifdef AMTX_LSTM_FWD_TIMING
+__device__ unsigned long long g_lstm_fwd_prof[5];
+#define LF_PARAM , unsigned long long (&lf_acc)[5], unsigned long long& lf_t
+#define LF_ARG , lf_acc, lf_t
+#define LF_TICK(SLOT) do { const unsigned long long n_ = __builtin_readcyclecounter(); lf_acc[SLOT] += n_ - lf_t; lf_t = n_; } while (0)
+#define LF_BEGIN unsigned long long lf_acc[5] = {0, 0, 0, 0, 0}, lf_t = __builtin_readcyclecounter()
+#define LF_END do { if (threadIdx.x == 0 && blockIdx.x == 0 && blockIdx.y == 0 && blockIdx.z == 0) for (int i_ = 0; i_ < 5; ++i_) atomicAdd(&g_lstm_fwd_prof[i_], lf_acc[i_]); } while (0)
+#else
+#define LF_PARAM
+#define LF_ARG
+#define LF_TICK(SLOT) do {} while (0)
+#define LF_BEGIN do {} while (0)
+#define LF_END do {} while (0)
+#endif
+
 template <int X_TYPE> struct XScalar { typedef float type; };
 template <> struct XScalar<AMTX_T_BF16> { typedef unsigned int type; };
 __device__ __forceinline__ float unpack_xs(float v, bool) { return v; }
@@ -227,7 +242,7 @@
 __device__ __forceinline__ void lstm4_step(char* smem, int cur, const uint4 (&wf)[4][4][NS], const typename XScalar<X_TYPE>::type (&xcur)[NC][4],
                                            typename XScalar<X_TYPE>::type (&xnext)[NC][4], float (&c)[NC], const char* const (&xbase)[NC],
                                            char* const (&obase)[NC], int t, int tnext, int lane, const int (&hwoff)[NC], const bool (&clip_ok)[NC],
-                                           float* save) {
+                                           float* save LF_PARAM) {
     constexpr int RSTEP = 4 / NC;
     const char* hb = smem + cur * NS * HBUF_BYTES;
     uint4 hf[4][NS];
@@ -259,6 +274,7 @@
         }
     }
 
+    LF_TICK(0);
     char* hn = smem + (cur ^ 1) * NS * HBUF_BYTES;
     Gates z[NC];
     float h[NC];
@@ -267,7 +283,7 @@
     for (int j = 0; j < NC; ++j) z[j] = lstm_gates<FAST>(acc[0][RSTEP * j], acc[1][RSTEP * j], acc[2][RSTEP * j], acc[3][RSTEP * j]);
 #pragma unroll
     for (int j = 0; j < NC; ++j) {
-        h[j] = lstm_cell<FAST>(z[j], c[j]);
+        h[j] = lstm_cell<FAST, NS == 1 && X_TYPE == AMTX_T_BF16 && OUT_TYPE == AMTX_T_BF16>(z[j], c[j]);
         low[j] = 0;
         if (NS == 2) split_bf16x2(h[j], 0.f, hiw[j], low[j]);
         else hiw[j] = pack_bf16x2(h[j], 0.f);
@@ -288,7 +304,12 @@
             else *reinterpret_cast<float*>(obase[j] + (int64_t)t * 256 * 4) = h[j];
         }
     }
+    LF_TICK(2);
     lds_barrier();
+    LF_TICK(3);
+#ifdef AMTX_LSTM_FWD_TIMING
+    lf_acc[4] += 1;
+#endif
 }
 
 template <int NS, int X_TYPE, int OUT_TYPE, int NC = 1>
@@ -342,15 +363,161 @@
     }
     __syncthreads();
 
+    LF_BEGIN;
     for (int s = 0; s < T; s += 4) {
         bool ok1[NC], ok2[NC], ok3[NC];
 #pragma unroll
         for (int j = 0; j < NC; ++j) { ok1[j] = clip_ok[j] && s + 1 < T; ok2[j] = clip_ok[j] && s + 2 < T; ok3[j] = clip_ok[j] && s + 3 < T; }
-        lstm4_step<NS, X_TYPE, OUT_TYPE, FAST, NC>(smem, 0, wf, x0, x3, c, xbase, obase, (int)tidx(s), (int)tidx(s + 3), lane, hwoff, clip_ok, save);
-        lstm4_step<NS, X_TYPE, OUT_TYPE, FAST, NC>(smem, 1, wf, x1, x0, c, xbase, obase, (int)tidx(s + 1), (int)tidx(s + 4), lane, hwoff, ok1, save);
-        lstm4_step<NS, X_TYPE, OUT_TYPE, FAST, NC>(smem, 0, wf, x2, x1, c, xbase, obase, (int)tidx(s + 2), (int)tidx(s + 5), lane, hwoff, ok2, save);
-        lstm4_step<NS, X_TYPE, OUT_TYPE, FAST, NC>(smem, 1, wf, x3, x2, c, xbase, obase, (int)tidx(s + 3), (int)tidx(s + 6), lane, hwoff, ok3, save);
-    }
+        lstm4_step<NS, X_TYPE, OUT_TYPE, FAST, NC>(smem, 0, wf, x0, x3, c, xbase, obase, (int)tidx(s), (int)tidx(s + 3), lane, hwoff, clip_ok, save LF_ARG);
+        lstm4_step<NS, X_TYPE, OUT_TYPE, FAST, NC>(smem, 1, wf, x1, x0, c, xbase, obase, (int)tidx(s + 1), (int)tidx(s + 4), lane, hwoff, ok1, save LF_ARG);
+        lstm4_step<NS, X_TYPE, OUT_TYPE, FAST, NC>(smem, 0, wf, x2, x1, c, xbase, obase, (int)tidx(s + 2), (int)tidx(s + 5), lane, hwoff, ok2, save LF_ARG);
+        lstm4_step<NS, X_TYPE, OUT_TYPE, FAST, NC>(smem, 1, wf, x3, x2, c, xbase, obase, (int)tidx(s + 3), (int)tidx(s + 6), lane, hwoff, ok3, save LF_ARG);
+    }
+    LF_END;
+}
+
+constexpr int XP = 64 * 4 + 8;
+constexpr int XBUF_BYTES = 16 * XP * 2;
+
+template <int KX>
+__device__ __forceinline__ void lstm4x_project(const char* xt, int lane, const uint4 (&wx)[4][KX], f32x4_t (&pacc)[4]) {
+#pragma unroll
+    for (int q = 0; q < 4; ++q) pacc[q] = (f32x4_t){0.f, 0.f, 0.f, 0.f};
+    static_for<0, KX>([&](auto kc) {
+        constexpr int ks = decltype(kc)::value;
+        const uint4 xf = *reinterpret_cast<const uint4*>(xt + ((lane & 15) * XP + 32 * ks + 8 * (lane >> 4)) * 2);
+        static_for<0, 4>([&](auto qc) { pacc[decltype(qc)::value] = mfma16(xf, wx[decltype(qc)::value][ks], pacc[decltype(qc)::value]); });
+    });
+}
+
+template <int KX>
+__device__ __forceinline__ void lstm4x_step(char* smem, int cur, const uint4 (&wf)[4][4], const uint4 (&wx)[4][KX], const float (&bias)[4], f32x4_t (&pacc)[4],
+                                            const uint2& xcur, uint2& xnext, const char* xsrc, int64_t xrow_bytes, int xwoff, float (&c)[2],
+                                            char* const (&obase)[2], int t, int tnext, int lane, const int (&hwoff)[2], const bool (&clip_ok)[2] LF_PARAM) {
+    const char* hb = smem + cur * HBUF_BYTES;
+    char* xtiles = smem + 2 * HBUF_BYTES;
+    uint4 hf[4];
+#pragma unroll
+    for (int ks = 0; ks < 4; ++ks) hf[ks] = *reinterpret_cast<const uint4*>(hb + ((lane & 15) * HP + 32 * ks + 8 * (lane >> 4)) * 2);
+
+    xnext = *reinterpret_cast<const uint2*>(xsrc + (int64_t)tnext * xrow_bytes);
+
+    auto r16 = [](float v) { return unpack16_lo(pack_bf16x2(v, 0.f)); };
+    f32x4_t acc[4];
+#pragma unroll
+    for (int q = 0; q < 4; ++q) acc[q] = (f32x4_t){r16(pacc[q][0] + bias[q]), 0.f, r16(pacc[q][2] + bias[q]), 0.f};
+#pragma unroll
+    for (int ks = 0; ks < 4; ++ks)
+#pragma unroll
+        for (int q = 0; q < 4; ++q) acc[q] = mfma16(hf[ks], wf[q][ks], acc[q]);
+    __builtin_amdgcn_sched_barrier(0);
+    LF_TICK(0);
+
+    *reinterpret_cast<uint2*>(xtiles + cur * XBUF_BYTES + xwoff) = xcur;
+    lstm4x_project<KX>(xtiles + (cur ^ 1) * XBUF_BYTES, lane, wx, pacc);
+#if defined(AMTX_LSTM_FWD_TIMING) && AMTX_LSTM_FWD_TIMING == 2
+    __builtin_amdgcn_sched_barrier(0);
+    LF_TICK(1);
+#endif
+
+    char* hn = smem + (cur ^ 1) * HBUF_BYTES;
+    Gates z[2];
+    uint32_t hiw[2];
+#pragma unroll
+    for (int j = 0; j < 2; ++j) z[j] = lstm_gates<true>(acc[0][2 * j], acc[1][2 * j], acc[2][2 * j], acc[3][2 * j]);
+#pragma unroll
+    for (int j = 0; j < 2; ++j) hiw[j] = pack_bf16x2(lstm_cell<true, true>(z[j], c[j]), 0.f);
+#pragma unroll
+    for (int j = 0; j < 2; ++j) *reinterpret_cast<unsigned short*>(hn + hwoff[j]) = (unsigned short)hiw[j];
+#pragma unroll
+    for (int j = 0; j < 2; ++j)
+        if (clip_ok[j]) *reinterpret_cast<unsigned short*>(obase[j] + (int64_t)t * 256 * 2) = (unsigned short)hiw[j];
+#if !defined(AMTX_LSTM_FWD_TIMING) || AMTX_LSTM_FWD_TIMING != 2
+    __builtin_amdgcn_sched_group_barrier(0x200, 1, 0);
+    __builtin_amdgcn_sched_group_barrier(0x100, KX, 0);
+    static_for<0, 4 * KX>([&](auto) {
+        __builtin_amdgcn_sched_group_barrier(0x008, 1, 0);
+        __builtin_amdgcn_sched_group_barrier(0x002, 2, 0);
+    });
+#endif
+    LF_TICK(2);
+    lds_barrier();
+    LF_TICK(3);
+#ifdef AMTX_LSTM_FWD_TIMING
+    lf_acc[4] += 1;
+#endif
+}
+
+template <int NC, int KX>
+__global__ __launch_bounds__(LTHREADS) void bilstm4x_kernel(LstmArgs a) {
+    extern __shared__ __attribute__((aligned(16))) char smem[];
+    constexpr int CPB = 4 * NC, RSTEP = 4 / NC;
+    static_assert(NC == 2 && CPB == LWAVES && KX >= 1 && 8 * KX <= 64, "eight clips per block: wave w stages clip w's row, 8 bytes per lane");
+    const int tid = threadIdx.x, lane = tid & 63, wave = tid >> 6;
+    const int unit = 16 * wave + (lane & 15), cg = lane >> 4;
+    const int dir = blockIdx.y;
+    const int T = a.T;
+
+    uint4 wf[4][4], wx[4][KX];
+    float bias[4];
+    {
+        const uint4* w = reinterpret_cast<const uint4*>(a.whh) + lane;
+#pragma unroll
+        for (int q = 0; q < 4; ++q)
+#pragma unroll
+            for (int ks = 0; ks < 4; ++ks) wf[q][ks] = w[((((dir * LWAVES + wave) * 4 + q) * 4 + ks)) * 64];
+        static_for<0, 4>([&](auto qc) {
+            constexpr int q = decltype(qc)::value;
+            const bf16_t* row = a.wih + (int64_t)(dir * 4 * H + q * H + unit) * a.ldw + 8 * cg;
+            static_for<0, KX>([&](auto kc) { wx[q][decltype(kc)::value] = *reinterpret_cast<const uint4*>(row + 32 * decltype(kc)::value); });
+            bias[q] = a.bias[dir * 4 * H + q * H + unit];
+        });
+    }
+    for (int i = tid; i < (2 * HBUF_BYTES + 2 * XBUF_BYTES) / 16; i += LTHREADS) reinterpret_cast<uint4*>(smem)[i] = make_uint4(0, 0, 0, 0);
+
+    float c[NC];
+    bool clip_ok[NC];
+    char* obase[NC];
+    int hwoff[NC];
+#pragma unroll
+    for (int j = 0; j < NC; ++j) {
+        const int b = (blockIdx.x * 4 + cg) * NC + j;
+        clip_ok[j] = b < a.B;
+        c[j] = 0.f;
+        obase[j] = reinterpret_cast<char*>(a.out) + ((int64_t)(clip_ok[j] ? b : 0) * T * 256 + dir * 128 + unit) * 2;
+        hwoff[j] = ((4 * cg + RSTEP * j) * HP + unit) * 2;
+    }
+    const int sclip = blockIdx.x * CPB + wave;
+    const int64_t xrow_bytes = a.ldx * 2;
+    const char* xsrc = reinterpret_cast<const char*>(a.x) + (int64_t)(sclip < a.B ? sclip : 0) * T * xrow_bytes + 8 * (lane < 8 * KX ? lane : 8 * KX - 1);
+    const int xwoff = RSTEP * wave * XP * 2 + 8 * lane;
+    char* xtiles = smem + 2 * HBUF_BYTES;
+    auto tidx = [&](int s) { return (int64_t)step_frame(s, T, dir); };
+    auto load_xr = [&](int s) { return *reinterpret_cast<const uint2*>(xsrc + tidx(s) * xrow_bytes); };
+
+    __syncthreads();
+    {
+        const uint2 r0 = load_xr(0), r1 = load_xr(1);
+        *reinterpret_cast<uint2*>(xtiles + xwoff) = r0;
+        *reinterpret_cast<uint2*>(xtiles + XBUF_BYTES + xwoff) = r1;
+    }
+    uint2 x0 = load_xr(2), x1 = load_xr(3), x2 = load_xr(4), x3;
+    __syncthreads();
+    f32x4_t pacc[4];
+    lstm4x_project<KX>(xtiles, lane, wx, pacc);
+    __syncthreads();
+
+    LF_BEGIN;
+    for (int s = 0; s < T; s += 4) {
+        bool ok1[NC], ok2[NC], ok3[NC];
+#pragma unroll
+        for (int j = 0; j < NC; ++j) { ok1[j] = clip_ok[j] && s + 1 < T; ok2[j] = clip_ok[j] && s + 2 < T; ok3[j] = clip_ok[j] && s + 3 < T; }
+        lstm4x_step<KX>(smem, 0, wf, wx, bias, pacc, x0, x3, xsrc, xrow_bytes, xwoff, c, obase, (int)tidx(s), (int)tidx(s + 5), lane, hwoff, clip_ok LF_ARG);
+        lstm4x_step<KX>(smem, 1, wf, wx, bias, pacc, x1, x0, xsrc, xrow_bytes, xwoff, c, obase, (int)tidx(s + 1), (int)tidx(s + 6), lane, hwoff, ok1 LF_ARG);
+        lstm4x_step<KX>(smem, 0, wf, wx, bias, pacc, x2, x1, xsrc, xrow_bytes, xwoff, c, obase, (int)tidx(s + 2), (int)tidx(s + 7), lane, hwoff, ok2 LF_ARG);
+        lstm4x_step<KX>(smem, 1, wf, wx, bias, pacc, x3, x2, xsrc, xrow_bytes, xwoff, c, obase, (int)tidx(s + 3), (int)tidx(s + 8), lane, hwoff, ok3 LF_ARG);
+    }
+    LF_END;
 }
 
 constexpr int GP = 4 * H + 8;
@@ -474,6 +641,16 @@
         for (int i = 0; i < 4; ++i) atomicAdd(&g_lstm_prof[i], lt_acc[i]);
 #endif
 }
+#if defined(AMTX_LSTM_FWD_TIMING) && !defined(AMTX_F16)
+extern "C" int amtxdbg_lstm_fwd_prof(unsigned long long* out5, int reset) {
+    if (hipMemcpyFromSymbol(out5, HIP_SYMBOL(g_lstm_fwd_prof), 5 * sizeof(unsigned long long)) != hipSuccess) return -1;
+    if (reset) {
+        unsigned long long z[5] = {0, 0, 0, 0, 0};
+        if (hipMemcpyToSymbol(HIP_SYMBOL(g_lstm_fwd_prof), z, sizeof(z)) != hipSuccess) return -1;
+    }
+    return 0;
+}
+#endif
 #if defined(AMTX_LSTM_TIMING) && !defined(AMTX_F16)
 extern "C" int amtxdbg_lstm_prof(unsigned long long* out4, int reset) {
     if (hipMemcpyFromSymbol(out4, HIP_SYMBOL(g_lstm_prof), 4 * sizeof(unsigned long long)) != hipSuccess) return -1;
@@ -811,9 +988,11 @@
     return sw;
 }
 
-enum LstmFamily { LSTM_CLIPS4, LSTM_CLIPS8, LSTM_CLIPS16, LSTM_STREAM, LSTM_ERROR };
+enum LstmFamily { LSTM_CLIPS4, LSTM_CLIPS8, LSTM_CLIPS8X, LSTM_CLIPS16, LSTM_STREAM, LSTM_ERROR };
 enum LstmInst { LSTM_BF16, LSTM_BF16_F32IO, LSTM_X3, LSTM_NO_INST };
 struct LstmRouted { LstmFamily family; LstmInst inst; dim3 grid; size_t lds; int code; const char* error; };
+
+constexpr int LSTM_KX_MAX = 6;
 
 LstmRouted lstm_route(const LstmArgs& a, const LstmSwitches& sw) {
     const bool io16 = a.x_type == AMTX_T_BF16 && a.out_type == AMTX_T_BF16, io32 = a.x_type == AMTX_T_F32 && a.out_type == AMTX_T_F32;
@@ -822,6 +1001,16 @@
     auto on = [&](LstmFamily family, int clips, size_t lds) {
         return LstmRouted{family, inst, dim3((unsigned)((a.B + clips - 1) / clips), 2, (unsigned)a.groups), lds, AMTX_OK, nullptr};
     };
+    if (a.x) {
+        if (a.hidden != H || inst != LSTM_BF16) return error(AMTX_ERR_UNSUPPORTED, "bilstm: the layer input is taken at hidden 128 in the one-plane 16-bit mode only");
+        if (a.kx < 1 || a.kx > LSTM_KX_MAX) return error(AMTX_ERR_UNSUPPORTED, "bilstm: the layer input is taken up to 192 columns (six 32-deep k-steps)");
+        if (!a.wih || !a.bias || a.ldx < 32 * a.kx || a.ldw < 32 * a.kx || (a.ldx % 8) != 0 || (a.ldw % 8) != 0)
+            return error(AMTX_ERR_ARG, "bilstm: the layer input needs its weights and bias, and rows of x and W_ih that hold 32 kx columns at 16-byte alignment");
+        if (a.save || a.groups != 1) return error(AMTX_ERR_UNSUPPORTED, "bilstm: the layer input is taken by one inference LSTM per launch (no save, one group)");
+        if (sw.no8 || (int64_t)((a.B + 3) / 4) * 2 <= 256 || (int64_t)((a.B + 3) / 4) * 2 > 1024)
+            return error(AMTX_ERR_UNSUPPORTED, "bilstm: the layer input is taken where eight-clip blocks run (513 .. 2048 clips)");
+        return on(LSTM_CLIPS8X, 8, 2 * (size_t)HBUF_BYTES + 2 * (size_t)XBUF_BYTES);
+    }
     if (a.hidden != H) {
         if (a.save && a.planes != 2) return error(AMTX_ERR_ARG, "bilstm: the training forward (save) is built for the two-plane precision");
         if (a.hidden != 256 && a.hidden != 384 && a.hidden != 512) return error(AMTX_ERR_UNSUPPORTED, "bilstm: unsupported hidden size (128, 256, 384 and 512 are built)");
@@ -861,6 +1050,18 @@
     switch (r.family) {
         case LSTM_CLIPS4: return launch_kernel(bilstm4_kernel<NS, XT, XT>, r.grid, r.lds, stream, a);
         case LSTM_CLIPS8: return launch_kernel(bilstm4_kernel<NS, XT, XT, 2>, r.grid, r.lds, stream, a);
+        case LSTM_CLIPS8X:
+            if constexpr (NS == 1 && XT == AMTX_T_BF16) {
+                switch (a.kx) {
+                    case 1: return launch_kernel(bilstm4x_kernel<2, 1>, r.grid, r.lds, stream, a);
+                    case 2: return launch_kernel(bilstm4x_kernel<2, 2>, r.grid, r.lds, stream, a);
+                    case 3: return launch_kernel(bilstm4x_kernel<2, 3>, r.grid, r.lds, stream, a);
+                    case 4: return launch_kernel(bilstm4x_kernel<2, 4>, r.grid, r.lds, stream, a);
+                    case 5: return launch_kernel(bilstm4x_kernel<2, 5>, r.grid, r.lds, stream, a);
+                    case 6: return launch_kernel(bilstm4x_kernel<2, 6>, r.grid, r.lds, stream, a);
+                }
+            }
+            break;
         case LSTM_CLIPS16: return launch_kernel(bilstm_kernel<NS, XT, XT>, r.grid, r.lds, stream, a);
         case LSTM_STREAM:
             if constexpr (NS == 2 || XT == AMTX_T_BF16)
@@ -886,7 +1087,7 @@
 }
 
 int amtx_launch_bilstm(const LstmArgs& a, hipStream_t stream) {
-    AMTX_REQUIRE(a.xproj && a.whh && a.out, "bilstm: null pointer");
+    AMTX_REQUIRE((a.xproj || a.x) && a.whh && a.out, "bilstm: null pointer");
     AMTX_REQUIRE(a.B > 0 && a.T > 0 && a.groups > 0, "bilstm: bad sizes");
     AMTX_REQUIRE(a.planes == 1 || a.planes == 2, "bilstm: planes must be 1 or 2");
     const LstmRouted r = lstm_route(a, lstm_switches());
@@ -898,6 +1099,14 @@
     }
     amtx_set_error("%s (hidden %d)", r.error, a.hidden);
     return r.code;
+}
+
+bool amtx_bilstm_takes_input(int hidden, int B, int kx, int64_t ldx, int64_t ldw) {
+    static const float given = 0.f;
+    LstmArgs a{};
+    a.x_type = a.out_type = AMTX_T_BF16; a.planes = 1; a.B = B; a.T = 1; a.groups = 1; a.hidden = hidden;
+    a.x = a.wih = reinterpret_cast<const bf16_t*>(&given); a.bias = &given; a.kx = kx; a.ldx = ldx; a.ldw = ldw;
+    return lstm_route(a, lstm_switches()).family == LSTM_CLIPS8X;
 }
 
 int amtx_launch_bilstm_pack_dev(const float* whh_fwd, const float* whh_bwd, int hidden, int planes, bf16_t* frag_fwd, bf16_t* frag_bwd, hipStream_t stream) {
diff --git a/amt_tools_amd/csrc/ofmodel.hip b/amt_tools_amd/csrc/ofmodel.hip
--- a/amt_tools_amd/csrc/ofmodel.hip
+++ b/amt_tools_amd/csrc/ofmodel.hip
@@ -15,7 +15,7 @@
     X(ns, pack_linear_host) X(ns, bilstm_pack_host) X(ns, conv1_pack_host) X(ns, conv1g_pack_host) X(ns, conv3x3_pack_host)     \
     X(ns, conv3x3_gen_pack_host) X(ns, pack_conv1_dev) X(ns, pack_conv1g_dev) X(ns, pack_conv3x3_dev) X(ns, pack_conv_gen_dev)    \
     X(ns, pack_linear_dev) X(ns, launch_bilstm_pack_dev) X(ns, launch_conv1) X(ns, launch_conv3x3) X(ns, launch_conv3x3_gen)    \
-    X(ns, launch_conv_stack) X(ns, launch_gemm) X(ns, launch_bilstm)
+    X(ns, launch_conv_stack) X(ns, launch_gemm) X(ns, launch_bilstm) X(ns, bilstm_takes_input)
 #define AMTX_KERNEL_FIELD(ns, name) decltype(&ns::amtx_##name) name;
 #define AMTX_KERNEL_ENTRY(ns, name) &ns::amtx_##name,
 struct KernelSet { AMTX_FMT_KERNELS(AMTX_KERNEL_FIELD, amtx_bf16) };
@@ -86,6 +86,8 @@
     std::vector<std::string> head_names;
     TensorStore store{"of_model", "was not provided"};
     DevBuf pack_scratch;
+    bool adj_in_recurrence = false;
+    bool adj_gemm = false;
     bool finalized = false;
     bool packed_once = false;
     DevBuf conv_w[3], conv_s[3];
@@ -122,6 +124,11 @@
                 PATH_CONV1 };
 struct ConvCall { ConvPath path; bool a2_in_hbm; int64_t a3_plane; };
 
+bool adj_fused(const amtx_of_model* m, int B) {
+    const int kp = (m->dim_aj + 63) / 64 * 64;
+    return m->adj_in_recurrence && !m->adj_gemm && m->precision == AMTX_PREC_BF16 && m->k->bilstm_takes_input(m->hid, B, (m->dim_aj + 31) / 32, kp, kp);
+}
+
 ConvCall resolve_conv(const amtx_of_model* m, int B, int T, bool feats16) {
     const ConvPlan& p = m->plan;
     if (p.stack && amtx_conv_stack_fused_ok(B, T, m->dim_in, m->n_heads))
@@ -143,7 +150,7 @@
     w.l1 = ws.take(BT * m->dim_lm * es * m->n_rec);
     w.joint = ws.take(BT * m->dim_aj * sizeof(float));
     w.joint16 = ws.take(BT * (size_t)((m->dim_aj + 63) / 64 * 64) * 2 * (m->plan.two_plane_acts ? 2 : 1));
-    w.xp2 = ws.take(BT * m->xw * es);
+    w.xp2 = adj_fused(m, B) ? nullptr : ws.take(BT * m->xw * es);
     w.l2 = ws.take(BT * m->dim_lm * es);
     w.mp = ws.take(BT * m->n_out * sizeof(float));
     w.total = ws.off;
@@ -161,9 +168,10 @@
 }
 
 extern "C" int amtx_of_model_create(amtx_of_model** out, int dim_in, int in_channels, int model_complexity, int n_out,
-                                    int has_offsets, int precision) {
+                                    int has_offsets, int precision_and_options) {
     AMTX_REQUIRE(out, "amtx_of_model_create: null model pointer");
     *out = nullptr;
+    const int precision = precision_and_options & ~AMTX_OF_PROJECT_IN_RECURRENCE;
     AMTX_REQUIRE(precision == AMTX_PREC_BF16 || precision == AMTX_PREC_X3 || precision == AMTX_PREC_F16, "amtx_of_model_create: bad precision");
     AMTX_REQUIRE(dim_in >= 4 && in_channels >= 1 && n_out > 0 && n_out % 4 == 0, "amtx_of_model_create: bad dims");
     if (precision == AMTX_PREC_F16 && !amtx_has_f16()) {
@@ -192,6 +200,8 @@
     m->hid = m->dim_lm / 2; m->xw = 8 * m->hid;
     m->hh_elems = amtx_bilstm_wfrag_elems(m->hid, m->planes);
     m->plan = make_conv_plan(in_channels, model_complexity, precision, switches_from_env());
+    m->adj_in_recurrence = (precision_and_options & AMTX_OF_PROJECT_IN_RECURRENCE) != 0;
+    m->adj_gemm = getenv("AMTX_OF_ADJ_GEMM") != nullptr;
     m->head_names = {"onset_head"};
     if (has_offsets) m->head_names.push_back("offset_head");
     m->n_rec = (int)m->head_names.size();
@@ -618,20 +628,26 @@
     if ((rc = k->launch_gemm(gp, s)) != AMTX_OK) return rc;
     mark();
 
-    if (pl == 1) {
-        if (!copy_on && (rc = amtx_launch_cvt_pad_bf16((const float*)w.joint, m->dim_aj, m->dim_aj, (bf16_t*)w.joint16, kp, BT, s, m->f16)) != AMTX_OK) return rc;
-        g = gemm_args(w.joint16, kp, AMTX_T_BF16, m->adj_ih, pl, w.xp2, m->xw, at, BT, 1, 0, 0);
-        g.K = kp;
-    } else if (sp) {
-        if ((rc = amtx_launch_cvt_split((const float*)w.joint, m->dim_aj, m->dim_aj, (bf16_t*)w.joint16, kp, BT * kp, BT, s)) != AMTX_OK) return rc;
-        g = gemm_args(w.joint16, kp, AMTX_T_SPLIT, m->adj_ih, pl, w.xp2, m->xw, at, BT, 1, 0, 0);
-        g.K = kp; g.a_split = BT * kp;
+    if (pl == 1 && !copy_on && (rc = amtx_launch_cvt_pad_bf16((const float*)w.joint, m->dim_aj, m->dim_aj, (bf16_t*)w.joint16, kp, BT, s, m->f16)) != AMTX_OK) return rc;
+    l.whh = (const bf16_t*)m->adj_hh.p; l.out = w.l2; l.groups = 1;
+    if (adj_fused(m, B)) {
+        l.xproj = nullptr; l.x = (const bf16_t*)w.joint16; l.ldx = kp; l.kx = (m->dim_aj + 31) / 32;
+        l.wih = (const bf16_t*)m->adj_ih.w.p; l.ldw = m->adj_ih.k_pad; l.bias = (const float*)m->adj_ih.b.p;
     } else {
-        g = gemm_args(w.joint, m->dim_aj, AMTX_T_F32, m->adj_ih, pl, w.xp2, m->xw, at, BT, 1, 0, 0);
-    }
-    if ((rc = k->launch_gemm(g, s)) != AMTX_OK) return rc;
-    mark();
-    l.xproj = w.xp2; l.whh = (const bf16_t*)m->adj_hh.p; l.out = w.l2; l.groups = 1;
+        if (pl == 1) {
+            g = gemm_args(w.joint16, kp, AMTX_T_BF16, m->adj_ih, pl, w.xp2, m->xw, at, BT, 1, 0, 0);
+            g.K = kp;
+        } else if (sp) {
+            if ((rc = amtx_launch_cvt_split((const float*)w.joint, m->dim_aj, m->dim_aj, (bf16_t*)w.joint16, kp, BT * kp, BT, s)) != AMTX_OK) return rc;
+            g = gemm_args(w.joint16, kp, AMTX_T_SPLIT, m->adj_ih, pl, w.xp2, m->xw, at, BT, 1, 0, 0);
+            g.K = kp; g.a_split = BT * kp;
+        } else {
+            g = gemm_args(w.joint, m->dim_aj, AMTX_T_F32, m->adj_ih, pl, w.xp2, m->xw, at, BT, 1, 0, 0);
+        }
+        if ((rc = k->launch_gemm(g, s)) != AMTX_OK) return rc;
+        l.xproj = w.xp2;
+    }
+    mark();
     if ((rc = k->launch_bilstm(l, s)) != AMTX_OK) return rc;
     mark();
     g = gemm_args(w.l2, m->dim_lm, at, m->adj_out, pl, w.mp, m->n_out, AMTX_T_F32, BT, 1, 0, 0);
diff --git a/amt_tools_amd/models.py b/amt_tools_amd/models.py
--- a/amt_tools_amd/models.py
+++ b/amt_tools_amd/models.py
@@ -357,7 +357,7 @@
     def __init__(self, model, device):
         self.n_out = model.profile.get_range_len()
         super().__init__(device, int(model.dim_in), int(model.in_channels), int(model.model_complexity), int(self.n_out),
-                         int(model.has_offsets), {'bf16': 0, 'x3': 1, 'f16': 2}[model.precision])
+                         int(model.has_offsets), {'bf16': 0, 'x3': 1, 'f16': 2}[model.precision] | 0x100)
         self.device_sync = os.environ.get('AMTX_HOST_WEIGHT_SYNC') is None
         self.device_syncs = 0
 
diff --git a/include/amtx.h b/include/amtx.h
--- a/include/amtx.h
+++ b/include/amtx.h
@@ -16,6 +16,8 @@
 #define AMTX_PREC_BF16 0
 #define AMTX_PREC_X3 1
 #define AMTX_PREC_F16 2
+
+#define AMTX_OF_PROJECT_IN_RECURRENCE 0x100
 
 const char* amtx_last_error(void);
 int amtx_version(void);
```

After: 42.21 million, median of 6. +1.8%, better.
